# awslabs/flowgger

Measured on AMD Instinct MI355X. Metric: log lines/sec (RFC5424, 256B avg) at 1/2/4/8 MI355X; achieved HBM GB/s, higher is better.
Workload: dtype u8; 1 GPU; BASELINE configs[1]: RFC5424 no structured data, 100000000 lines/GPU @ 254 B avg (1000000-line tile x100 resident in HBM), 1% invalid lines; lines_per_gpu=100000000, bytes_per_gpu=25376525600, parallelism=lines sharded 1-way, no data-path collective, ok_lines_per_tile=990000

## Files before the change

flowgger_amd/_lib.py:

```python
from __future__ import annotations

import ctypes as C
from pathlib import Path

import os

_HERE = Path(__file__).resolve().parent
_ALT = os.environ.get("FLOWGGER_AMD_LIB") or ""
if _ALT and (Path(_ALT).name != _ALT or not _ALT.startswith("libfg_hip") or not _ALT.endswith(".so")):
    raise RuntimeError(f"FLOWGGER_AMD_LIB={_ALT!r}: only a bare libfg_hip*.so file name beside flowgger_amd/_lib.py is accepted")
LIB_PATH = _HERE / (_ALT or ("libfg_hip_prof.so" if os.environ.get("FLOWGGER_AMD_PROF_LIB") else "libfg_hip.so"))

FG_ABI_VERSION = 4
FG_RFC5424, FG_LTSV, FG_GELF, FG_RFC3164, FG_CAPNP = 0, 1, 2, 3, 4
FG_EF_VAL_ESC, FG_EF_NAME_ESC, FG_EF_SUFFIX, FG_EF_NAME_VERBATIM = 1, 2, 4, 8
FG_FRAME_NONE, FG_FRAME_LINE, FG_FRAME_NUL, FG_FRAME_SYSLEN, FG_FRAME_CAPNP = 0, 1, 2, 3, 4
FG_CAPNP_CLEAN, FG_CAPNP_TAIL, FG_CAPNP_TOO_MANY_SEGMENTS, FG_CAPNP_TOO_LARGE = 0, 1, 2, 3
FG_CAPNP_FRAME_MAX_BYTES = 0xFFFF0000
FG_SYSLEN_CLEAN, FG_SYSLEN_TAIL, FG_SYSLEN_BAD_LEN, FG_SYSLEN_LONG_PREFIX = 0, 1, 2, 3
FG_SYSLEN_MAX_PREFIX = 24
FG_UDP_RAW, FG_UDP_ZLIB, FG_UDP_GZIP, FG_UDP_BAD_ZLIB, FG_UDP_BAD_GZIP, FG_UDP_BAD_UTF8, FG_UDP_TOO_LARGE = range(7)
FG_UDP_DEFAULT_MAX_INFLATED = 65_527 * 5
FG_ST_OVERFLOW, FG_ST_BAD_UTF8 = 0xFE, 0xFD
FG_F_LTSV_NOVALUE = 128
FG_OK, FG_ERR_ARG, FG_ERR_HIP, FG_ERR_NO_DEVICE, FG_ERR_ENT_OVERFLOW, FG_ERR_UNSUPPORTED, FG_ERR_NOMEM = 0, -1, -2, -3, -4, -5, -6
FG_YEAR_NOW = -2147483648
FG_NONE = 0xFFFFFFFF
FG_T_STRING, FG_T_BOOL, FG_T_F64, FG_T_I64, FG_T_U64, FG_T_NULL, FG_T_SDID = range(7)
FG_TABLE_ARRAYS = 15
_ERRNAMES = {-1: "FG_ERR_ARG", -2: "FG_ERR_HIP", -3: "FG_ERR_NO_DEVICE (no gfx950 GPU; there is no CPU fallback)",
             -4: "FG_ERR_ENT_OVERFLOW", -5: "FG_ERR_UNSUPPORTED", -6: "FG_ERR_NOMEM"}


class FgError(RuntimeError):
    def __init__(self, code: int, what: str = ""):
        self.code = code
        super().__init__(f"{what}: {_ERRNAMES.get(code, code)}")


class fg_span(C.Structure):
    _fields_ = [("off", C.c_uint32), ("len", C.c_uint32)]


class fg_tables(C.Structure):
    _fields_ = [
        ("n", C.c_uint64), ("ent_cap", C.c_uint64),
        ("meta", C.c_void_p), ("ts", C.c_void_p),
        ("hostname", C.c_void_p), ("appname", C.c_void_p), ("procid", C.c_void_p),
        ("msgid", C.c_void_p), ("msg", C.c_void_p), ("full_msg", C.c_void_p),
        ("ent_first", C.c_void_p), ("ent_count", C.c_void_p),
        ("ent_name", C.c_void_p), ("ent_val", C.c_void_p),
        ("ent_type", C.c_void_p), ("ent_flags", C.c_void_p), ("ent_used", C.c_void_p),
    ]


TABLE_FIELDS = ["meta", "ts", "hostname", "appname", "procid", "msgid", "msg", "full_msg", "ent_first",
                "ent_count", "ent_name", "ent_val", "ent_type", "ent_flags", "ent_used"]


class fg_gelf_extra(C.Structure):
    _fields_ = [("n", C.c_uint32), ("keys", C.POINTER(C.c_char_p)), ("values", C.POINTER(C.c_char_p))]


FG_ENC_GELF, FG_ENC_LTSV, FG_ENC_RFC5424, FG_ENC_RFC3164, FG_ENC_PASSTHROUGH, FG_ENC_CAPNP = range(6)
FG_MERGE_NONE, FG_MERGE_LINE, FG_MERGE_NUL, FG_MERGE_SYSLEN = range(4)


class fg_encode_cfg(C.Structure):
    _fields_ = [("encoder", C.c_int), ("merger", C.c_int), ("n_extra", C.c_uint32), ("extra_keys", C.POINTER(C.c_char_p)),
                ("extra_values", C.POINTER(C.c_char_p)), ("prepend", C.c_char_p), ("now_ts", C.c_double)]


class fg_launch_opts(C.Structure):
    _fields_ = [("lines_per_group", C.c_uint32), ("tile_cap", C.c_uint32), ("waves_per_cu", C.c_uint32),
                ("gelf_lds_budget", C.c_uint32), ("gelf_window_kib", C.c_uint32), ("flags", C.c_uint32), ("chunk_lines", C.c_uint32), ("ent_chunk", C.c_uint32), ("fused_look", C.c_uint32), ("fused_ext", C.c_uint32)]


FG_LO_GELF_GENERIC, FG_LO_TRANSCODE_ONE_PIECE, FG_LO_NO_HEAD, FG_LO_FORCE_HEAD, FG_LO_SD_WALK, FG_LO_SD_PAIRS, FG_LO_NO_ZERO_COPY, FG_LO_FRAME_KERNEL_UPLOAD = 1, 2, 4, 8, 16, 32, 64, 128
FG_LO_FRAME_CLASSIC = 256
FG_LO_STATIC_CHUNKS = 512
FG_LO_FRAME_SELFTEST_STALL = 1024
FG_LO_NO_TAPER = 2048
FG_LO_TAPER_1 = 4096
FG_LO_TAPER_2 = 8192
FG_LO_NO_FUSED_FRAMING = 16384
FG_LO_RFC3164_REGROUP, FG_LO_RFC3164_NO_REGROUP = 32768, 65536
FG_PATH_DECODE_ZERO_COPY, FG_PATH_DECODE_SLICED, FG_PATH_FRAME_FUSED, FG_PATH_FRAME_SLICED, FG_PATH_FRAME_ONE_PIECE = 1, 2, 3, 4, 5
FG_PATH_FRAME_SYSLEN_DEVICE, FG_PATH_FRAME_SYSLEN_HOST = 6, 7
FG_PATH_FRAME_CAPNP_DEVICE, FG_PATH_FRAME_CAPNP_HOST = 8, 9
FG_PATH_FRAME_MULTI = 10
FG_PATH_FRAME_SYSLEN_MULTI_DEVICE, FG_PATH_FRAME_SYSLEN_MULTI_HOST = 11, 12
FG_PATH_FRAME_CAPNP_MULTI_DEVICE, FG_PATH_FRAME_CAPNP_MULTI_HOST = 13, 14
FG_SLOT_FRAME, FG_SLOT_BAD_UTF8, FG_SLOT_CARRY = 0, 1, 2
FG_LO_RESERVED = 0x40000000


class fg_transcoded(C.Structure):
    _fields_ = [("out", C.c_void_p), ("out_bytes", C.c_uint64), ("out_offsets", C.c_void_p), ("meta", C.c_void_p),
                ("enc_status", C.c_void_p), ("frame_offsets", C.c_void_p), ("n", C.c_uint64), ("consumed", C.c_uint64)]


class fg_tz_table(C.Structure):
    _fields_ = [("n_zones", C.c_uint32), ("names", C.POINTER(C.c_char_p)), ("zone_first", C.c_void_p), ("utc_start", C.c_void_p),
                ("utc_offset", C.c_void_p)]


class fg_rfc3164_cfg(C.Structure):
    _fields_ = [("current_year", C.c_int32), ("tz", C.POINTER(fg_tz_table))]


class fg_cfg(C.Structure):
    _fields_ = [
        ("n_schema", C.c_uint32),
        ("schema_names", C.POINTER(C.c_char_p)),
        ("schema_types", C.POINTER(C.c_uint8)),
        ("suffix_bool", C.c_char_p), ("suffix_f64", C.c_char_p),
        ("suffix_i64", C.c_char_p), ("suffix_u64", C.c_char_p),
    ]


_lib = None


def lib() -> C.CDLL:
    global _lib
    if _lib is not None:
        return _lib
    if not LIB_PATH.exists():
        raise RuntimeError(
            f"{LIB_PATH} is missing: build it with `python -m flowgger_amd.build` "
            "(hipcc --offload-arch=gfx950). The decoders have no CPU fallback.")
    try:
        import torch
    except Exception:
        pass
    L = C.CDLL(str(LIB_PATH))
    vp, u64, u32 = C.c_void_p, C.c_uint64, C.c_uint32
    L.fg_abi_version.restype = C.c_int
    L.fg_create.argtypes = [C.c_int, C.POINTER(fg_cfg), C.POINTER(vp)]
    L.fg_clone.argtypes = [vp, C.POINTER(vp)]
    L.fg_destroy.argtypes = [vp]
    L.fg_destroy.restype = None
    L.fg_last_hip_error.argtypes = [vp]
    L.fg_set_launch_opts.argtypes = [vp, C.POINTER(fg_launch_opts)]
    L.fg_tables_layout.argtypes = [u64, u64, C.POINTER(u64)]
    L.fg_decode_batch_device.argtypes = [vp, C.c_int, vp, u64, vp, u64, C.POINTER(fg_tables), vp]
    L.fg_decode_batch.argtypes = [vp, C.c_int, vp, u64, vp, u64, C.POINTER(fg_tables)]
    L.fg_error_string.argtypes = [C.c_int, C.c_uint8]
    L.fg_error_string.restype = C.c_char_p
    L.fg_tables_serialize.argtypes = [C.c_int, C.POINTER(fg_cfg), vp, vp, C.POINTER(fg_tables), u64, u64, vp, u64, vp]
    L.fg_tables_serialize.restype = C.c_int64
    L.fg_tables_stdout.argtypes = [C.c_int, C.c_int, vp, vp, C.POINTER(fg_tables), u64, u64, vp, u64]
    L.fg_tables_stdout.restype = C.c_int64
    L.fg_shard_plan.argtypes = [vp, u64, u32, vp]
    L.fg_gather_size.argtypes = [C.POINTER(fg_tables), u32, C.POINTER(u64), C.POINTER(u64)]
    L.fg_gather_tables.argtypes = [C.POINTER(fg_tables), u32, C.POINTER(fg_tables)]
    L.fg_merge_tables.argtypes = [C.POINTER(fg_tables), u32, C.POINTER(vp), C.POINTER(fg_tables), vp]
    L.fg_merge_tables_device.argtypes = [vp, C.POINTER(fg_tables), u32, C.POINTER(vp), C.POINTER(fg_tables), vp, vp]
    L.fg_ordered_merge.argtypes = [u32, vp, C.POINTER(vp), C.POINTER(vp), C.POINTER(vp), vp, u64, vp]
    L.fg_ordered_merge.restype = C.c_int64
    L.fg_ticket_ring_check.argtypes = [vp]
    L.fg_set_pinned_limits.argtypes = [u64, u64]
    L.fg_pinned_stats.argtypes = [C.POINTER(u64), C.POINTER(u64), C.POINTER(u64)]
    L.fg_set_timing.argtypes = [vp, C.c_int]
    L.fg_last_kernel_ms.argtypes = [vp, C.POINTER(C.c_float)]
    L.fg_frame_decode_batch.argtypes = [vp, C.c_int, C.c_int, vp, u64, C.c_int, C.POINTER(fg_tables), C.POINTER(vp),
                                        C.POINTER(u64), C.POINTER(u64)]
    L.fg_encode_gelf_device.argtypes = [vp, C.c_int, vp, u64, vp, u64, C.POINTER(fg_tables), C.POINTER(fg_gelf_extra), vp, u64, vp,
                                        C.POINTER(u64), vp]
    L.fg_encode_device.argtypes = [vp, C.c_int, C.POINTER(fg_encode_cfg), vp, u64, vp, u64, C.POINTER(fg_tables), vp, u64, vp, vp,
                                   C.POINTER(u64), vp]
    L.fg_encode_device_async.argtypes = [vp, C.c_int, C.POINTER(fg_encode_cfg), vp, u64, vp, u64, C.POINTER(fg_tables), vp, u64, vp, vp,
                                         u64, vp]
    L.fg_transcode_batch.argtypes = [vp, C.c_int, C.c_int, C.POINTER(fg_encode_cfg), vp, u64, vp, u64, C.c_int, C.POINTER(fg_transcoded)]
    L.fg_encode_error_string.argtypes = [C.c_uint8]
    L.fg_encode_error_string.restype = C.c_char_p
    L.fg_set_rfc3164.argtypes = [vp, C.POINTER(fg_rfc3164_cfg)]
    L.fg_measure_link.argtypes = [vp, u64, C.POINTER(C.c_double)]
    L.fg_calibrate_device.argtypes = [vp, C.c_int, vp, vp, u64, vp]
    L.fg_alloc_pinned.argtypes = [u64, C.POINTER(vp)]
    L.fg_free_pinned.argtypes = [vp]
    L.fg_free_pinned.restype = None
    L.fg_frame_device.argtypes = [vp, C.c_int, vp, u64, vp, vp, u64, C.POINTER(u64), vp]
    L.fg_decode_frames_device.argtypes = [vp, C.c_int, C.c_int, vp, u64, vp, u64, vp, C.POINTER(fg_tables), vp]
    L.fg_last_host_path.argtypes = [vp]
    L.fg_last_syslen_stop.argtypes = [vp]
    L.fg_last_capnp_stop.argtypes = [vp]
    L.fg_frame_capnp_device.argtypes = [vp, vp, u64, C.c_int, vp, u64, C.POINTER(u64), C.POINTER(u64), C.POINTER(C.c_int), vp]
    L.fg_frame_syslen_device.argtypes = [vp, vp, u64, C.c_int, vp, vp, vp, vp, u64, C.POINTER(u64), C.POINTER(u64), C.POINTER(C.c_int), vp]
    L.fg_udp_error_string.argtypes = [C.c_uint8]
    L.fg_udp_error_string.restype = C.c_char_p
    L.fg_udp_unpack_device.argtypes = [vp, vp, u64, vp, u64, u64, vp, u64, vp, vp, vp, C.POINTER(u64), vp]
    L.fg_udp_decode_batch.argtypes = [vp, C.c_int, vp, u64, vp, u64, u64, C.POINTER(fg_tables), C.POINTER(vp), C.POINTER(vp), C.POINTER(vp)]
    L.fg_frame_decode_device.argtypes = [vp, C.c_int, C.c_int, vp, u64, C.c_int, vp, u64, C.POINTER(fg_tables), u64, vp, vp]
    L.fg_frame_multi_device.argtypes = [vp, C.c_int, vp, u64, vp, vp, u64, vp, vp, u64, vp, vp, C.POINTER(u64), vp]
    L.fg_frame_decode_multi_batch.argtypes = [vp, C.c_int, C.c_int, vp, u64, vp, vp, u64, C.POINTER(fg_tables), C.POINTER(vp), C.POINTER(vp),
                                              C.POINTER(vp), C.POINTER(vp), C.POINTER(u64)]
    L.fg_frame_syslen_multi_device.argtypes = [vp, vp, u64, vp, u64, vp, vp, vp, vp, u64, vp, vp, vp, C.POINTER(u64), C.POINTER(u64), vp]
    L.fg_frame_decode_syslen_multi_batch.argtypes = [vp, C.c_int, vp, u64, vp, u64, C.POINTER(fg_tables), C.POINTER(vp), C.POINTER(vp),
                                                     C.POINTER(vp), C.POINTER(vp), C.POINTER(u64)]
    L.fg_frame_capnp_multi_device.argtypes = [vp, vp, u64, vp, u64, vp, vp, u64, vp, vp, vp, C.POINTER(u64), vp]
    L.fg_frame_decode_capnp_multi_batch.argtypes = [vp, vp, u64, vp, u64, C.POINTER(fg_tables), C.POINTER(vp), C.POINTER(vp), C.POINTER(vp),
                                                    C.POINTER(vp), C.POINTER(vp), C.POINTER(u64)]
    if L.fg_abi_version() != FG_ABI_VERSION:
        raise RuntimeError("libfg_hip.so ABI version mismatch")
    _lib = L
    return L


def check(rc: int, what: str) -> None:
    if rc != 0:
        raise FgError(rc, what)
```

flowgger_amd/csrc/fg_pipeline.hpp:

```cpp
#pragma once
#include "fg_device.hpp"
#include "fg_plan_policy.hpp"
#include "fg_wave.hpp"

namespace fg {

using u32x4 = unsigned int __attribute__((ext_vector_type(4)));

__device__ __forceinline__ uint32_t eq_flags(uint32_t x, uint32_t pat) {
    uint32_t s = ((x & 0x7F7F7F7Fu) ^ pat) + 0x7F7F7F7Fu;
    return ~(s | x) & 0x80808080u;
}
__device__ __forceinline__ uint32_t range_flags(uint32_t x) {
    uint32_t l = x & 0x7F7F7F7Fu;
    uint32_t ge33 = l + 0x5F5F5F5Fu;
    uint32_t le126 = l + 0x01010101u;
    return ge33 & ~le126 & ~x & 0x80808080u;
}
__device__ __forceinline__ uint32_t ctrl_flags(uint32_t x) {
    uint32_t ge32 = (x & 0x7F7F7F7Fu) + 0x60606060u;
    return ~(ge32 | x) & 0x80808080u;
}
__device__ __forceinline__ uint32_t gather16(uint32_t f0, uint32_t f1, uint32_t f2, uint32_t f3) {
    uint32_t lo = __builtin_amdgcn_udot4(f1, 0x80402010u, __builtin_amdgcn_udot4(f0, 0x08040201u, 0u, false), false);
    uint32_t hi = __builtin_amdgcn_udot4(f3, 0x80402010u, __builtin_amdgcn_udot4(f2, 0x08040201u, 0u, false), false);
    return (lo >> 7) | (hi << 1);
}
__device__ __forceinline__ uint32_t mask16_eq(const uint4& v, uint32_t pat) {
    return gather16(eq_flags(v.x, pat), eq_flags(v.y, pat), eq_flags(v.z, pat), eq_flags(v.w, pat));
}

struct Tile {
    const uint32_t* w;
    const uint32_t* bm;
};
__device__ __forceinline__ void load8(const Tile& T, uint32_t a, uint32_t* lo, uint32_t* hi) {
    uint32_t d = a >> 2, s = a & 3u;
    uint32_t w0 = T.w[d], w1 = T.w[d + 1], w2 = T.w[d + 2];
    *lo = __builtin_amdgcn_alignbyte(w1, w0, s);
    *hi = __builtin_amdgcn_alignbyte(w2, w1, s);
}
__device__ __forceinline__ void load16(const Tile& T, uint32_t a, uint32_t w[4]) {
    const uint32_t d = a >> 2, s = a & 3u;
    uint32_t r0 = T.w[d], r1 = T.w[d + 1], r2 = T.w[d + 2], r3 = T.w[d + 3], r4 = T.w[d + 4];
    w[0] = __builtin_amdgcn_alignbyte(r1, r0, s);
    w[1] = __builtin_amdgcn_alignbyte(r2, r1, s);
    w[2] = __builtin_amdgcn_alignbyte(r3, r2, s);
    w[3] = __builtin_amdgcn_alignbyte(r4, r3, s);
}
struct WinReader {
    const Tile& T;
    uint32_t base;
    uint32_t w0 = 0x80000000u;
    uint64_t lo = 0, hi = 0;
    __device__ __forceinline__ WinReader(const Tile& t, uint32_t b) : T(t), base(b) {}
    __device__ __forceinline__ uint32_t byte(uint32_t i) {
        uint32_t off = i - w0;
        if (off >= 16u) {
            uint32_t w[4];
            load16(T, base + i, w);
            lo = (uint64_t)w[0] | ((uint64_t)w[1] << 32);
            hi = (uint64_t)w[2] | ((uint64_t)w[3] << 32);
            w0 = i;
            off = 0;
        }
        const uint64_t v = off < 8u ? lo : hi;
        return (uint32_t)(v >> (8u * (off & 7u))) & 0xFFu;
    }
};

__device__ __forceinline__ uint32_t find_bit(const uint32_t* bm, uint32_t base, uint32_t q, uint32_t len) {
    while (q < len) {
        uint32_t a = base + q;
        uint32_t w = bm[a >> 5] >> (a & 31u);
        if (w) {
            uint32_t r = q + (uint32_t)__builtin_ctz(w);
            return r < len ? r : len;
        }
        q += 32u - (a & 31u);
    }
    return len;
}
__device__ __forceinline__ uint32_t find_bit_long(const uint32_t* bm, uint32_t base, uint32_t q, uint32_t len) {
    if (q >= len) return len;
    {
        const uint32_t a = base + q;
        const uint32_t w = bm[a >> 5] >> (a & 31u);
        if (w) {
            const uint32_t r = q + (uint32_t)__builtin_ctz(w);
            return r < len ? r : len;
        }
        q += 32u - (a & 31u);
    }
    while (q + 256u <= len) {
        const uint32_t i = (base + q) >> 5;
        uint32_t w[8];
#pragma unroll
        for (int k = 0; k < 8; ++k) w[k] = bm[i + k];
        if ((w[0] | w[1] | w[2] | w[3] | w[4] | w[5] | w[6] | w[7]) != 0u) {
            uint32_t r = len;
#pragma unroll
            for (int k = 7; k >= 0; --k)
                if (w[k]) r = q + 32u * k + (uint32_t)__builtin_ctz(w[k]);
            return r < len ? r : len;
        }
        q += 256u;
    }
    while (q < len) {
        const uint32_t w = bm[(base + q) >> 5];
        if (w) {
            const uint32_t r = q + (uint32_t)__builtin_ctz(w);
            return r < len ? r : len;
        }
        q += 32u;
    }
    return len;
}
template <class M>
__device__ __forceinline__ void rebuild_bitmap(const uint8_t* smem, uint16_t* bm16, uint32_t nchunk) {
    const uint4* src = reinterpret_cast<const uint4*>(smem);
    for (uint32_t c = threadIdx.x; c < nchunk; c += kWave) bm16[c] = (uint16_t)M::mask16(src[c]);
}

struct RowOut {
    uint32_t meta;
    double ts;
    fg_span span[6];
    uint32_t first, count;
    bool skip = false;
};
__device__ __forceinline__ void store_row(const DevTables& t, uint64_t li, const RowOut& o) {
    if (o.skip) return;
    gstore(t.meta, li, o.meta);
    gstore(t.ts, li, o.ts);
#pragma unroll
    for (int k = 0; k < 6; ++k) gstore(t.span[k], li, o.span[k]);
    gstore(t.ent_first, li, o.first);
    gstore(t.ent_count, li, o.count);
}
constexpr uint32_t kStashEntries = 48;
constexpr uint32_t kStashWords = 2;

struct EntAlloc {
    uint32_t ex = 0;
    uint32_t total = 0;
    wv::Slots s{};
    bool overflow = false;
};
__device__ __forceinline__ EntAlloc alloc_entries_ex(const DevTables& t, uint32_t n_ent, uint32_t* ent_state) {
    EntAlloc a;
    if (!__any(n_ent != 0u)) return a;
    a.ex = wv::excl_sum(n_ent, &a.total);
    const uint32_t left = wv::wave_left(ent_state);
    const unsigned long long nofit = __ballot(n_ent != 0u && a.ex + n_ent > left);
    const uint32_t cut = nofit ? (uint32_t)__shfl((int)a.ex, (int)__builtin_ctzll(nofit), kWave) : a.total;
    a.s = wv::wave_alloc(t.ent_used, t.ent_cap, ent_state, a.total, cut, t.alloc_chunk);
    a.overflow = a.s.overflow && n_ent != 0u && a.ex >= a.s.cut;
    return a;
}
__device__ __forceinline__ uint32_t alloc_entries(const DevTables& t, uint32_t n_ent, bool* overflow, uint32_t* ent_state) {
    const EntAlloc a = alloc_entries_ex(t, n_ent, ent_state);
    *overflow = a.overflow;
    return (a.overflow || a.total == 0u) ? 0u : a.s.at(a.ex);
}

struct GroupCtx {
    const uint8_t* bytes;
    const uint8_t* smem;
    uint16_t* bm16;
    uint64_t o0, o1;
    uint64_t a0;
    uint32_t span;
    bool valid;
    uint64_t li;
    uint64_t* stash;
    uint32_t ablate;
    uint32_t* ent_state;
    unsigned long long* phase;
    uint32_t tbase = 0;
    uint32_t tlen = 0;
    uint32_t last2 = 0;
    uint32_t tile_cap = 0;
};

template <uint32_t WORDS, class Unpack>
__device__ __forceinline__ bool stash_to_table(const GroupCtx& c, const DevTables& t, const EntAlloc& a, uint32_t n_ent, bool mine,
                                               Unpack un) {
    const uint32_t lane = threadIdx.x;
    const uint32_t cap = (c.span / 18u) & ~3u;
    if (a.total == 0u || a.total > cap || a.s.overflow || c.stash == nullptr || __any(n_ent != 0u && !mine)) return false;
    uint64_t* s_name = reinterpret_cast<uint64_t*>(const_cast<uint8_t*>(c.smem));
    uint64_t* s_val = s_name + cap;
    uint16_t* s_tf = reinterpret_cast<uint16_t*>(s_val + cap);
    __syncthreads();
    for (uint32_t k0 = 0; k0 < n_ent; k0 += 4u) {
        uint64_t w0[4], w1[4];
#pragma unroll
        for (uint32_t j = 0; j < 4u; ++j) {
            const uint32_t k = k0 + j < n_ent ? k0 + j : n_ent - 1u;
            w0[j] = c.stash[(k * WORDS) * kWave + lane];
            w1[j] = WORDS > 1u ? c.stash[(k * WORDS + 1u) * kWave + lane] : 0ull;
        }
#pragma unroll
        for (uint32_t j = 0; j < 4u; ++j) {
            if (k0 + j < n_ent) {
                uint64_t name, val;
                uint32_t tf;
                un(w0[j], w1[j], &name, &val, &tf);
                const uint32_t idx = a.ex + k0 + j;
                s_name[idx] = name;
                s_val[idx] = val;
                s_tf[idx] = (uint16_t)tf;
            }
        }
    }
    __syncthreads();
    for (uint32_t idx = lane; idx < a.total; idx += kWave) {
        const uint32_t slot = a.s.at(idx);
        const uint64_t name = s_name[idx];
        const uint32_t tf = s_tf[idx];
        t.ent_name[slot] = fg_span{(uint32_t)name, (uint32_t)(name >> 32)};
        t.ent_val[slot] = s_val[idx];
        t.ent_type[slot] = (uint8_t)(tf & 0xFFu);
        t.ent_flags[slot] = (uint8_t)(tf >> 8);
    }
    return true;
}


struct FrameArgs {
    uint32_t strip;
    const uint8_t* line_bad;
    uint32_t* ticket = nullptr;
    uint32_t ticket_base = 0;
    uint32_t taper0 = kNoTaper, taper1 = kNoTaper, taper2 = kNoTaper;
};

#define FG_STREAM_AUX 2
__device__ __forceinline__ uint4 stream_load(const uint4* p) {
    typedef uint32_t nt4 __attribute__((ext_vector_type(4)));
    const nt4 v = __builtin_nontemporal_load(reinterpret_cast<const nt4*>(p));
    return make_uint4(v.x, v.y, v.z, v.w);
}

template <class F, class = void>
struct tail_batch { static constexpr int value = 4; };
template <class F>
struct tail_batch<F, decltype((void)F::kTailBatch)> { static constexpr int value = F::kTailBatch; };

template <class F, class = void>
struct defer_row_store { static constexpr bool value = true; };
template <class F>
struct defer_row_store<F, decltype((void)F::kDeferRowStore)> { static constexpr bool value = F::kDeferRowStore; };

constexpr uint32_t kHeadCap = 1024;
template <class F, class = void>
struct head_cap { static constexpr uint32_t value = kHeadCap; };
template <class F>
struct head_cap<F, decltype((void)F::kHeadBytes)> { static constexpr uint32_t value = F::kHeadBytes; };

template <int NB, bool PROF, class F, bool HEAD = false>
__device__ __forceinline__ void persistent_loop(const uint8_t* __restrict__ bytes, const uint64_t* __restrict__ offsets,
                                                uint64_t n, const DevTables& t, uint32_t tile_cap, uint32_t L, uint64_t chunk_lines,
                                                unsigned long long* prof, uint64_t* stash_base, F& fmt, FrameArgs fr) {
    static_assert(!HEAD || F::kClasses <= 1, "HEAD staging classifies one stage-A byte class at most");
    const uint64_t kChunkLines = chunk_lines;
    extern __shared__ __attribute__((aligned(16))) uint8_t smem[];
    uint16_t* bm16 = reinterpret_cast<uint16_t*>(smem + tile_cap + 64u);
    const uint32_t bm_stride = tile_cap / 16u + 16u;
    uint4* dst = reinterpret_cast<uint4*>(smem);
    const uint32_t lane = threadIdx.x;
    const uint64_t G = gridDim.x;
    uint64_t* stash = stash_base ? stash_base + (uint64_t)blockIdx.x * (kStashEntries * kStashWords * kWave) : nullptr;

    const bool dyn = fr.ticket != nullptr;
    uint32_t tk_raw = 0;
    bool tk_pending = false;
    auto draw_ticket = [&]() {
        if (lane == 0u) tk_raw = __hip_atomic_fetch_add(fr.ticket, 1u, __ATOMIC_RELAXED, __HIP_MEMORY_SCOPE_AGENT);
        tk_pending = true;
    };
    uint64_t chunk = blockIdx.x;
    uint64_t p, hi_line;
    chunk_range(chunk, kChunkLines, fr.taper0, fr.taper1, fr.taper2, n, &p, &hi_line);
    if (dyn && p < n) draw_ticket();

    auto load_offsets = [&](uint64_t q, uint64_t* o0, uint64_t* o1) {
        const uint64_t li = q + lane;
        const bool in = lane < L && li < hi_line;
        *o0 = offsets[in ? li : hi_line];
        *o1 = offsets[in ? li + 1 : hi_line];
    };
    auto geometry = [&](uint64_t q, uint64_t o0, uint64_t o1, uint32_t* nl, uint64_t* a0, uint32_t* span) {
        const uint64_t left = hi_line - q;
        const uint32_t avail = left < (uint64_t)L ? (uint32_t)left : L;
        const uint32_t lo_l = (uint32_t)__builtin_amdgcn_readfirstlane((int)(uint32_t)o0);
        const uint32_t lo_h = (uint32_t)__builtin_amdgcn_readfirstlane((int)(uint32_t)(o0 >> 32));
        const uint64_t lo = (uint64_t)lo_l | ((uint64_t)lo_h << 32);
        *a0 = lo & ~15ull;
        const unsigned long long fit = __ballot(lane < avail && (o1 - *a0) <= (uint64_t)tile_cap);
        uint32_t cnt = fit == ~0ull ? 64u : (uint32_t)__builtin_ctzll(~fit);
        if (cnt == 0u) cnt = 1u;
        *nl = cnt;
        const uint32_t last = cnt - 1u;
        const uint32_t hi_l = (uint32_t)__builtin_amdgcn_readlane((int)(uint32_t)o1, (int)last);
        const uint32_t hi_h = (uint32_t)__builtin_amdgcn_readlane((int)(uint32_t)(o1 >> 32), (int)last);
        const uint64_t hi = (uint64_t)hi_l | ((uint64_t)hi_h << 32);
        const uint64_t want = hi - *a0;
        *span = want > tile_cap ? tile_cap : (uint32_t)((want + 15ull) & ~15ull);
    };
    auto load_window = [&](uint64_t a0, uint32_t span, u32x4* v) {
        __amdgpu_buffer_rsrc_t rsrc =
            __builtin_amdgcn_make_buffer_rsrc(const_cast<uint8_t*>(bytes + a0), (short)0, (int)span, 0x00020000);
#pragma unroll
        for (int k = 0; k < NB; ++k) v[k] = __builtin_amdgcn_raw_buffer_load_b128(rsrc, (int)(lane * 16u + k * 1024u), 0, FG_STREAM_AUX);
    };
    auto geometry_head = [&](uint64_t q, uint64_t o0, uint64_t o1, uint32_t* nl, uint32_t* span, uint32_t* st_out, uint32_t* tb_out) {
        const uint64_t left = hi_line - q;
        const uint32_t avail = left < (uint64_t)L ? (uint32_t)left : L;
        const uint64_t want = (o1 - o0) + (o0 & 15ull);
        uint32_t st = want >= head_cap<F>::value ? head_cap<F>::value : (uint32_t)((want + 15ull) & ~15ull);
        if (lane >= avail) st = 0u;
        uint32_t total;
        const uint32_t tb = wv::excl_sum(st, &total);
        const unsigned long long fit = __ballot(lane < avail && tb + st <= tile_cap);
        uint32_t cnt = fit == ~0ull ? 64u : (uint32_t)__builtin_ctzll(~fit);
        if (cnt == 0u) cnt = 1u;
        *nl = cnt;
        const uint32_t last = cnt - 1u;
        *span = (uint32_t)__builtin_amdgcn_readlane((int)tb, (int)last) + (uint32_t)__builtin_amdgcn_readlane((int)st, (int)last);
        *st_out = lane < cnt ? st : 0u;
        *tb_out = tb;
    };
    auto load_window_head = [&](uint64_t o0, uint32_t st, u32x4* v) {
#pragma unroll
        for (int k = 0; k < NB; ++k) {
            const uint32_t lo = (uint32_t)__builtin_amdgcn_readlane((int)(uint32_t)o0, k);
            const uint32_t hi = (uint32_t)__builtin_amdgcn_readlane((int)(uint32_t)(o0 >> 32), k);
            const uint32_t sk = (uint32_t)__builtin_amdgcn_readlane((int)st, k);
            const uint64_t b = ((uint64_t)lo | ((uint64_t)hi << 32)) & ~15ull;
            __amdgpu_buffer_rsrc_t rsrc = __builtin_amdgcn_make_buffer_rsrc(const_cast<uint8_t*>(bytes + b), (short)0, (int)sk, 0x00020000);
            v[k] = __builtin_amdgcn_raw_buffer_load_b128(rsrc, (int)(lane * 16u), 0, FG_STREAM_AUX);
        }
    };
    auto load_last2 = [&](uint64_t o0, uint64_t o1) -> uint32_t {
        const uint64_t len = o1 - o0;
        uint32_t r = 0;
        if (len >= 1u) r = bytes[o1 - 1u];
        if (len >= 2u) r |= (uint32_t)bytes[o1 - 2u] << 8;
        return r;
    };

    uint32_t* ent_state = reinterpret_cast<uint32_t*>(smem + tile_cap + 56u);
    if (lane < 2u) ent_state[lane] = 0u;
    if (p >= hi_line) return;
    uint64_t o0, o1, a0 = 0;
    uint32_t span, nl, st = 0, tb = 0, last2 = 0;
    load_offsets(p, &o0, &o1);
    u32x4 v[NB];
    if constexpr (HEAD) {
        geometry_head(p, o0, o1, &nl, &span, &st, &tb);
        load_window_head(o0, st, v);
        last2 = load_last2(o0, o1);
    } else {
        geometry(p, o0, o1, &nl, &a0, &span);
        load_window(a0, span, v);
    }
    RowOut pend{};
    uint64_t pend_li = 0;
    bool pend_valid = false;
    uint64_t acc0 = 0, acc1 = 0, acc2 = 0, acc3 = 0, iters = 0, tm0 = 0, tm1 = 0, tm2 = 0, tm3 = 0;
    const uint32_t ablate = PROF ? (uint32_t)prof[5] : 0u;
    const uint32_t term4 = fr.strip == FG_FRAME_LINE ? 0x0A0A0A0Au : fr.strip == FG_FRAME_NUL ? 0u : wv::kNoTerm;

    for (;;) {
        uint64_t pn = p + nl;
        if (pn >= hi_line) {
            if (dyn) {
                if (!tk_pending) draw_ticket();
                const uint32_t tk = (uint32_t)__builtin_amdgcn_readfirstlane((int)tk_raw);
                chunk = (uint64_t)(uint32_t)(tk - fr.ticket_base) + G;
                tk_pending = false;
                chunk_range(chunk, kChunkLines, fr.taper0, fr.taper1, fr.taper2, n, &pn, &hi_line);
                if (pn < n) draw_ticket();
            } else {
                chunk += G;
                chunk_range(chunk, kChunkLines, kNoTaper, kNoTaper, kNoTaper, n, &pn, &hi_line);
            }
        }
        const bool more = pn < n;
        uint64_t no0 = 0, no1 = 0;
        if (more) load_offsets(pn, &no0, &no1);
        if (PROF) {
            tm0 = __builtin_amdgcn_s_memtime();
            __builtin_amdgcn_s_waitcnt(0x0F70);
            tm1 = __builtin_amdgcn_s_memtime();
        }
        FG_MARK(A);
        const uint32_t nchunk = span >> 4;
        const uint32_t nrow = HEAD ? nl : (nchunk + kWave - 1u) / kWave;
        if constexpr (HEAD) {
#pragma unroll
            for (int k = 0; k < NB; ++k) {
                if ((uint32_t)k < nl) {
                    const uint32_t tk = (uint32_t)__builtin_amdgcn_readlane((int)tb, k), sk = (uint32_t)__builtin_amdgcn_readlane((int)st, k);
                    if (lane * 16u < sk) {
                        const uint4 q = make_uint4(v[k][0], v[k][1], v[k][2], v[k][3]);
                        dst[(tk >> 4) + lane] = q;
                        if constexpr (F::kClasses != 0) F::classify_store(q, bm16, (tk >> 4) + lane, bm_stride, term4);
                    }
                }
            }
            constexpr uint32_t HB = tail_batch<F>::value >= 8 ? 8u : 4u;
            for (uint32_t r0 = NB; r0 < nl; r0 += HB) {
                uint4 w[HB];
                uint32_t tk[HB], sk[HB];
#pragma unroll
                for (uint32_t j = 0; j < HB; ++j) {
                    const uint32_t r = r0 + j < nl ? r0 + j : nl - 1u;
                    const uint32_t lo = (uint32_t)__builtin_amdgcn_readlane((int)(uint32_t)o0, (int)r);
                    const uint32_t hi = (uint32_t)__builtin_amdgcn_readlane((int)(uint32_t)(o0 >> 32), (int)r);
                    tk[j] = (uint32_t)__builtin_amdgcn_readlane((int)tb, (int)r);
                    sk[j] = (uint32_t)__builtin_amdgcn_readlane((int)st, (int)r);
                    const uint64_t b = ((uint64_t)lo | ((uint64_t)hi << 32)) & ~15ull;
                    __amdgpu_buffer_rsrc_t rsrc = __builtin_amdgcn_make_buffer_rsrc(const_cast<uint8_t*>(bytes + b), (short)0, (int)sk[j], 0x00020000);
                    const u32x4 x = __builtin_amdgcn_raw_buffer_load_b128(rsrc, (int)(lane * 16u), 0, FG_STREAM_AUX);
                    w[j] = make_uint4(x[0], x[1], x[2], x[3]);
                }
#pragma unroll
                for (uint32_t j = 0; j < HB; ++j)
                    if (lane * 16u < sk[j]) {
                        dst[(tk[j] >> 4) + lane] = w[j];
                        if constexpr (F::kClasses != 0) F::classify_store(w[j], bm16, (tk[j] >> 4) + lane, bm_stride, term4);
                    }
            }
        } else {
#pragma unroll
        for (int k = 0; k < NB; ++k) {
            if ((uint32_t)k < nrow) {
                uint32_t idx = k * kWave + lane;
                uint4 q = make_uint4(v[k][0], v[k][1], v[k][2], v[k][3]);
                dst[idx] = q;
                F::classify_store(q, bm16, idx, bm_stride, idx < nchunk ? term4 : wv::kPastSpan);
            }
        }
        }
        if (!HEAD && nrow > (uint32_t)NB) {
            const uint4* __restrict__ src = reinterpret_cast<const uint4*>(bytes + a0);
            const uint32_t last = nchunk - 1u;
            constexpr int TB = tail_batch<F>::value;
            for (uint32_t c0 = NB * kWave; c0 < nchunk; c0 += kWave * TB) {
                uint4 w[TB];
#pragma unroll
                for (int k = 0; k < TB; ++k) {
                    const uint32_t idx = c0 + k * kWave + lane;
                    w[k] = stream_load(src + (idx < last ? idx : last));
                }
#pragma unroll
                for (int k = 0; k < TB; ++k) {
                    if (k == 0 || c0 + k * kWave < nchunk) {
                        const uint32_t idx = c0 + k * kWave + lane, ci = idx < last ? idx : last;
                        dst[ci] = w[k];
                        F::classify_store(w[k], bm16, ci, bm_stride, term4);
                    }
                }
            }
        }
        __builtin_amdgcn_sched_barrier(0);
        FG_MARK(S);
        if (PROF) {
            __builtin_amdgcn_s_waitcnt(0xC07F);
            tm2 = __builtin_amdgcn_s_memtime();
        }
        uint64_t pa0 = 0;
        uint32_t pspan = 0, pnl = 0, pst = 0, ptb = 0, plast2 = 0;
        if (more) {
            if constexpr (HEAD) geometry_head(pn, no0, no1, &pnl, &pspan, &pst, &ptb);
            else geometry(pn, no0, no1, &pnl, &pa0, &pspan);
        }
        FG_MARK(ST);
        if (pend_valid && !(ablate & 1u)) store_row(t, pend_li, pend);
        FG_MARK(W0);
        if (more) {
            if constexpr (HEAD) {
                load_window_head(no0, pst, v);
                plast2 = load_last2(no0, no1);
            } else {
                load_window(pa0, pspan, v);
            }
        }
        __builtin_amdgcn_sched_barrier(0);
        FG_MARK(W1);
        FG_MARK(B);
        if (PROF) tm3 = __builtin_amdgcn_s_memtime();
        __syncthreads();
        if (!(ablate & 2u)) {
            const uint64_t li = p + lane;
            const bool valid = lane < nl;
            uint64_t e1 = o1;
            uint32_t l2 = last2;
            if (fr.strip != FG_FRAME_NONE) {
                uint32_t b1 = last2 & 0xFFu, b2 = (last2 >> 8) & 0xFFu;
                if constexpr (!HEAD) {
                    const uint64_t len = o1 - o0;
                    const bool over = nl == 1u && __builtin_amdgcn_readfirstlane((int)((o1 - a0) > (uint64_t)span)) != 0;
                    if (over) {
                        FG_RARE_BEGIN();
                        if (valid && len >= 1u) b1 = bytes[o1 - 1u];
                        if (valid && len >= 2u) b2 = bytes[o1 - 2u];
                        FG_RARE_END();
                    } else if (valid) {
                        const uint32_t q = (uint32_t)(o1 - a0);
                        if (len >= 1u) b1 = smem[q - 1u];
                        if (len >= 2u) b2 = smem[q - 2u];
                    }
                }
                if (valid && e1 > o0) {
                    if (fr.strip == FG_FRAME_LINE) {
                        if (b1 == '\n') {
                            --e1;
                            if (e1 > o0 && b2 == '\r') --e1;
                        }
                    } else if (b1 == 0u) {
                        --e1;
                    }
                    if (HEAD && e1 != o1) {
                        l2 = 0u;
                        if (e1 - o0 >= 1u) l2 = bytes[e1 - 1];
                        if (e1 - o0 >= 2u) l2 |= (uint32_t)bytes[e1 - 2] << 8;
                    }
                }
            }
            GroupCtx c{bytes, smem, bm16, o0, e1, a0, span, valid, li, (ablate & 8u) ? nullptr : stash, ablate, ent_state, PROF ? prof + 6 : nullptr};
            c.tile_cap = tile_cap;
            if constexpr (HEAD) {
                const uint32_t al = (uint32_t)(o0 & 15ull), len = (uint32_t)(e1 - o0);
                c.tbase = tb + al;
                c.tlen = st == 0u ? 0u : (st - al < len ? st - al : len);
                c.last2 = l2;
            }
            pend = fmt.decode(c, t);
            if (fr.line_bad && valid && fr.line_bad[li]) {
                pend.meta = FG_ST_BAD_UTF8 | (0xFFu << 8) | (0xFFu << 16);
                pend.ts = 0.0;
#pragma unroll
                for (int k = 0; k < 6; ++k) pend.span[k] = fg_span{0, FG_NONE};
                pend.count = 0;
            }
            pend_li = li;
            pend_valid = valid;
            if (!defer_row_store<F>::value) {
                if (pend_valid && !(ablate & 1u)) store_row(t, pend_li, pend);
                pend_valid = false;
            }
        }
        if (PROF) {
            __builtin_amdgcn_sched_barrier(0);
            __builtin_amdgcn_s_waitcnt(0xC07F);
            uint64_t tm4 = __builtin_amdgcn_s_memtime();
            acc0 += tm1 - tm0;
            acc1 += tm2 - tm1;
            acc2 += tm3 - tm2;
            acc3 += tm4 - tm3;
            iters += 1;
        }
        FG_MARK(Z);
        if (!more) break;
        __syncthreads();
        p = pn;
        nl = pnl;
        o0 = no0;
        o1 = no1;
        a0 = pa0;
        span = pspan;
        if constexpr (HEAD) {
            st = pst;
            tb = ptb;
            last2 = plast2;
        }
    }
    if (pend_valid && !(ablate & 1u)) store_row(t, pend_li, pend);
    if (PROF && lane == 0) {
        atomicAdd(&prof[0], (unsigned long long)acc0);
        atomicAdd(&prof[1], (unsigned long long)acc1);
        atomicAdd(&prof[2], (unsigned long long)acc2);
        atomicAdd(&prof[3], (unsigned long long)acc3);
        atomicAdd(&prof[4], (unsigned long long)iters);
    }
}

}

#include <cstdio>
#include <cstdlib>

#include "fg_cus.hpp"

namespace fg {
constexpr int kComputeBoundWindow = 2;

inline void take_tickets(FrameArgs* fr, TicketSlot* tk, const LaunchPlan& p) {
    if (!tk || !tk->d_word || !tk->h_val || p.chunks + p.blocks >= 0xFFFFFFFFull || p.blocks > p.chunks) return;
    if (!p.tickets) return;
    fr->ticket = tk->d_word;
    fr->ticket_base = *tk->h_val;
    fr->taper0 = p.taper[0], fr->taper1 = p.taper[1], fr->taper2 = p.taper[2];
    *tk->h_val += (uint32_t)p.chunks;
}

template <class K>
inline int plan_launch(K kernel, uint64_t n, uint64_t avg_len, uint32_t extra_lds, uint32_t max_tile, uint32_t stash_blocks, LaunchPlan* p,
                       const fg_launch_opts& lo, const PlanFormat& pf = PlanFormat()) {
    static_cast<LaunchGeometry&>(*p) = launch_geometry(n, avg_len, extra_lds, max_tile, lo, pf);
    const int cus = device_cus();
    if (cus < 1) return -1;
    int per_cu = 0;
    if (hipOccupancyMaxActiveBlocksPerMultiprocessor(&per_cu, kernel, kWave, p->lds) != hipSuccess || per_cu < 1) per_cu = 1;
    if (lo.waves_per_cu > 0 && per_cu > (int)lo.waves_per_cu) per_cu = (int)lo.waves_per_cu;
    uint64_t blocks = (uint64_t)per_cu * (uint64_t)cus;
    if (blocks > p->groups) blocks = p->groups;
    if (stash_blocks && blocks > stash_blocks) blocks = stash_blocks;
    const ChunkPlan cp = plan_chunks(n, blocks, p->L, p->g, p->full, pf.ticket_from, lo, pf.taper);
    p->chunk = cp.chunk;
    p->chunks = cp.chunks;
    p->tickets = cp.tickets;
    for (int j = 0; j < 3; ++j) p->taper[j] = cp.taper[j];
    p->blocks = cp.blocks;
    return 0;
}

#if defined(FG_PROF_BUILD)
inline bool prof_requested() { return getenv("FG_PROF") != nullptr; }
#define FG_PROF_TWIN(...) (__VA_ARGS__)
#else
constexpr bool prof_requested() { return false; }
#define FG_PROF_TWIN(...) nullptr
#endif
struct ProfRun {
    unsigned long long* d = nullptr;
    unsigned long long h[16] = {0, 0, 0, 0, 0, 0, 0, 0, 0, 0, 0, 0, 0, 0, 0, 0};
    bool begin(hipStream_t stream) {
#if defined(FG_PROF_BUILD)
        if (const char* e = getenv("FG_ABLATE")) h[5] = (unsigned long long)atoi(e);
#endif
        if (hipMalloc((void**)&d, sizeof(h)) != hipSuccess) return false;
        (void)hipMemcpyAsync(d, h, sizeof(h), hipMemcpyHostToDevice, stream);
        return true;
    }
    void end(hipStream_t stream, const char* name, const LaunchPlan& p) {
        (void)hipStreamSynchronize(stream);
        (void)hipMemcpy(h, d, sizeof(h), hipMemcpyDeviceToHost);
        (void)hipFree(d);
        const double it = h[4] ? (double)h[4] : 1.0;
        fprintf(stderr,
                "[fg prof] %s: grid %u x64, L %u, tile %u, iters/wave %.1f | cycles per iteration: wait %.0f, stageA %.0f, "
                "stores+prefetch-issue %.0f, stageB %.0f\n",
                name, p.blocks, p.L, p.tile, it / (double)(p.blocks ? p.blocks : 1), h[0] / it, h[1] / it, h[2] / it, h[3] / it);
        bool any_phase = false;
        for (int k = 6; k < 16; ++k) any_phase = any_phase || h[k] != 0;
        if (any_phase) {
            fprintf(stderr, "[fg prof] %s stage-B phases (cycles per iteration):", name);
            for (int k = 6; k < 16; ++k) fprintf(stderr, " %.0f", h[k] / it);
            fprintf(stderr, "\n");
        }
    }
};

template <class K>
struct Kernels {
    K run, prof;
    const char* name;
};
template <class K>
inline Kernels<K> kernels(K run, typename SameAs<K>::type prof, const char* name) { return Kernels<K>{run, prof, name}; }

struct DecodeCall {
    uint64_t n;
    const DevTables* t;
    hipStream_t stream;
    FrameArgs fr;
    const fg_launch_opts* lo;
    TicketSlot* tk;
};
template <class K, class Go>
inline int launch_planned(const Kernels<K>& k, const LaunchPlan& p, const DecodeCall& c, Go go, bool prof_tickets = true) {
    const bool prof = k.prof != nullptr && prof_requested();
    FrameArgs fr = c.fr;
    if (!prof || prof_tickets) take_tickets(&fr, c.tk, p);
    DevTables tt = *c.t;
    tt.alloc_chunk = entry_chunk(tt.ent_cap, p.blocks, c.n, *c.lo, tt.shares);
    if (prof) {
        ProfRun pr;
        if (!pr.begin(c.stream)) return -1;
        go(k.prof, p, tt, fr, pr.d);
        pr.end(c.stream, k.name, p);
    } else {
        go(k.run, p, tt, fr, (unsigned long long*)nullptr);
    }
    return (int)hipGetLastError();
}
template <class K, class Go>
inline int plan_and_launch(const Kernels<K>& k, const DecodeCall& c, uint64_t avg_len, uint32_t extra_lds, uint32_t max_tile, uint32_t stash_blocks,
                           const PlanFormat& pf, Go go) {
    LaunchPlan p;
    if (plan_launch(k.run, c.n, avg_len, extra_lds, max_tile, stash_blocks, &p, *c.lo, pf)) return -1;
    return launch_planned(k, p, c, go);
}
}
```

flowgger_amd/csrc/fg_plan_policy.hpp:

```cpp
#pragma once
#include <stdint.h>

#include "../../include/fg_hip.h"

#if defined(__HIPCC__)
#define FG_POLICY_HD __host__ __device__
#else
#define FG_POLICY_HD
#endif

namespace fg {

constexpr uint32_t kNoTaper = 0xFFFFFFFFu;

FG_POLICY_HD inline void chunk_range(uint64_t c, uint64_t chunk, uint32_t t0, uint32_t t1, uint32_t t2, uint64_t n, uint64_t* lo,
                                     uint64_t* hi) {
    uint64_t base = 0, first = 0, sz = chunk;
    if (c >= t0) {
        base = (uint64_t)t0 * sz, first = t0, sz >>= 1;
        if (c >= t1) {
            base += (uint64_t)(t1 - t0) * sz, first = t1, sz >>= 1;
            if (c >= t2) base += (uint64_t)(t2 - t1) * sz, first = t2, sz >>= 1;
        }
    }
    const uint64_t l = base + (c - first) * sz;
    *lo = l < n ? l : n;
    *hi = l + sz < n ? l + sz : n;
}

inline uint64_t count_chunks(uint64_t chunk, const uint32_t t[3], uint64_t n) {
    uint64_t base = 0, first = 0, sz = chunk;
    for (int j = 0; j < 3; ++j) {
        if (t[j] == kNoTaper) break;
        const uint64_t upto = base + (uint64_t)(t[j] - first) * sz;
        if (upto >= n) break;
        base = upto, first = t[j], sz >>= 1;
    }
    return first + (n - base + sz - 1) / sz;
}

struct ChunkPlan {
    uint64_t chunk = 1;
    uint64_t chunks = 0;
    uint32_t blocks = 0;
    bool tickets = false;
    uint32_t taper[3] = {kNoTaper, kNoTaper, kNoTaper};
};

inline ChunkPlan plan_chunks(uint64_t n, uint64_t blocks, uint32_t L, uint64_t g, uint64_t full, uint32_t ticket_from, const fg_launch_opts& lo,
                             uint32_t taper = 1) {
    ChunkPlan p;
    if (blocks < 1u) blocks = 1u;
    if (g < 1u) g = 1u;
    if (g > L) g = L;
    if (full < 1u) full = 1u;
    const bool dynamic = !(lo.flags & FG_LO_STATIC_CHUNKS);
    const bool named = lo.chunk_lines >= (dynamic ? 1u : L) && lo.chunk_lines <= 65536u;
    const uint64_t per_wave = (n + blocks - 1) / blocks;
    uint64_t chunk;
    bool tickets = false;
    if (named) {
        chunk = lo.chunk_lines;
        if (n < blocks * 2u * chunk) {
            chunk = per_wave;
            if (chunk < (dynamic ? g : (uint64_t)L)) chunk = dynamic ? g : (uint64_t)L;
        }
        tickets = dynamic;
    } else if (dynamic && per_wave >= (uint64_t)ticket_from * full) {
        chunk = full;
        tickets = true;
    } else if (dynamic) {
        chunk = per_wave;
        const uint64_t unit = g >= L ? g : (g * 15u / 16u ? g * 15u / 16u : 1u);
        if (chunk < unit) chunk = unit;
    } else {
        const uint64_t k = (per_wave + full - 1) / full;
        chunk = (per_wave + (k ? k : 1) - 1) / (k ? k : 1);
        if (chunk < L) chunk = L;
    }
    if (chunk < 1u) chunk = 1u;
    p.chunk = chunk;
    p.chunks = (n + chunk - 1) / chunk;
    if (lo.flags & (FG_LO_TAPER_1 | FG_LO_TAPER_2)) taper = ((lo.flags & FG_LO_TAPER_1) ? 1u : 0u) + ((lo.flags & FG_LO_TAPER_2) ? 2u : 0u);
    if (taper > 3u) taper = 3u;
    if (tickets && taper && !(lo.flags & FG_LO_NO_TAPER)) {
        uint64_t m = n / (2u * chunk);
        if (m > blocks) m = blocks;
        uint32_t levels = 0;
        while (levels < taper && (chunk >> (levels + 1u)) >= g) ++levels;
        if (m >= 1u && levels >= 1u && p.chunks + 4u * m < 0xFFFFFFF0ull) {
            const uint64_t t0 = (n - m * chunk) / chunk;
            p.taper[0] = (uint32_t)t0;
            if (levels >= 2u) p.taper[1] = (uint32_t)(t0 + m);
            if (levels >= 3u) p.taper[2] = (uint32_t)(t0 + 2u * m);
            p.chunks = count_chunks(chunk, p.taper, n);
        }
    }
    p.blocks = (uint32_t)(blocks > p.chunks ? p.chunks : blocks);
    p.tickets = tickets;
    return p;
}

constexpr int kWindowKiB = 20;
constexpr uint32_t kMaxTile = 57344;

constexpr uint32_t tile_lds(uint32_t tile, uint32_t classes = 1) { return tile + 64u + (tile / 16u + 16u) * 2u * classes; }

constexpr uint32_t kShortLineTile = 17408;
static_assert(tile_lds(kShortLineTile) <= 160u * 1024u / 8u, "eight waves per CU");
static_assert(tile_lds(kShortLineTile + 1024u) > 160u * 1024u / 8u, "the largest such tile");

constexpr uint64_t kHeadFromLen = 768, kPairsFromLen = 320;
struct Variant { bool head, pairs; };
inline Variant pick_variant(uint64_t avg_len, uint32_t flags) {
    return Variant{(flags & FG_LO_FORCE_HEAD) || (avg_len >= kHeadFromLen && !(flags & FG_LO_NO_HEAD)),
                   (flags & FG_LO_SD_PAIRS) || (avg_len >= kPairsFromLen && !(flags & FG_LO_SD_WALK))};
}
inline bool gelf_group_fits_3k(uint64_t avg_len) { return 8u * avg_len * 17u / 16u + 256u <= 3072u; }
inline bool gelf_const_3k(uint64_t avg_len, const fg_launch_opts& lo) {
    return gelf_group_fits_3k(avg_len) && !lo.tile_cap && !(lo.flags & FG_LO_GELF_GENERIC);
}

struct PlanFormat {
    uint32_t max_lines = 64;
    uint32_t n_classes = 1;
    uint32_t (*extra_for)(uint32_t tile, uint32_t lines) = nullptr;
    uint32_t (*extra_tile)(uint32_t tile) = nullptr;
    uint32_t default_tile = 0;
    uint32_t default_chunk = 0;
    uint32_t ticket_from = 2;
    uint32_t taper = 1;
    PlanFormat& lines(uint32_t v) { max_lines = v; return *this; }
    PlanFormat& classes(uint32_t v) { n_classes = v; return *this; }
    PlanFormat& lds_for(uint32_t (*f)(uint32_t, uint32_t)) { extra_for = f; return *this; }
    PlanFormat& lds_tile(uint32_t (*f)(uint32_t)) { extra_tile = f; return *this; }
    PlanFormat& tile(uint32_t v) { default_tile = v; return *this; }
    PlanFormat& chunk(uint32_t v) { default_chunk = v; return *this; }
    PlanFormat& tickets_from(uint32_t v) { ticket_from = v; return *this; }
    PlanFormat& taper_levels(uint32_t v) { taper = v; return *this; }
};
inline PlanFormat rfc5424_walk_format(uint64_t avg_len) {
    return PlanFormat().tickets_from(20u).taper_levels(0u).tile(avg_len < kPairsFromLen ? kShortLineTile : 0u);
}

struct LaunchGeometry {
    uint32_t L = 64;
    uint32_t tile = 0;
    uint32_t lds = 0;
    uint64_t groups = 0;
    uint64_t full = 256;
    uint64_t g = 64;
};
struct LaunchPlan : LaunchGeometry {
    uint64_t chunk = 256;
    uint64_t chunks = 0;
    bool tickets = false;
    uint32_t taper[3] = {kNoTaper, kNoTaper, kNoTaper};
    uint32_t blocks = 0;
};

inline LaunchGeometry launch_geometry(uint64_t n, uint64_t avg_len, uint32_t extra_lds, uint32_t max_tile, const fg_launch_opts& lo,
                                      const PlanFormat& pf = PlanFormat()) {
    const uint64_t window = (uint64_t)kWindowKiB * 1024u;
    auto tile_for = [&](uint32_t l) { return (((uint64_t)l * avg_len * 17u / 16u + 256u) + 1023u) / 1024u * 1024u; };
    auto clamp = [&](uint64_t v) { return (uint32_t)(v < 4096u ? 4096u : v > max_tile ? max_tile : v); };
    const bool named_lines = lo.lines_per_group >= 1 && lo.lines_per_group <= pf.max_lines;
    const bool named_tile = lo.tile_cap >= 1024 && lo.tile_cap <= max_tile;
    LaunchGeometry p;
    uint32_t L = pf.max_lines;
    while (L > 1 && tile_for(L) > window + 2048u) L >>= 1;
    if (named_lines) L = lo.lines_per_group;
    uint32_t tile = clamp(tile_for(L));
    if (pf.default_tile && tile > pf.default_tile && !named_lines) tile = pf.default_tile;
    if (named_tile) tile = (lo.tile_cap + 1023u) / 1024u * 1024u;
    if (!pf.extra_for && !named_lines) {
        if (L <= 16u && !named_tile && tile < 18432u && max_tile >= 18432u && !pf.default_tile) tile = 18432u;
        L = pf.max_lines;
    }
    p.L = L;
    p.tile = tile;
    p.lds = tile_lds(tile, pf.n_classes ? pf.n_classes : 1u) + extra_lds + (pf.extra_for ? pf.extra_for(tile, L) : 0u) +
            (pf.extra_tile ? pf.extra_tile(tile) : 0u);
    {
        const uint64_t by_lines = (n + L - 1) / L, by_bytes = (n * avg_len + tile - 1) / tile;
        p.groups = by_lines > by_bytes ? by_lines : by_bytes;
    }
    p.full = pf.default_chunk ? pf.default_chunk : (avg_len ? (uint64_t)tile / avg_len : L) >= L ? 256u : 512u;
    p.g = avg_len ? ((uint64_t)tile * 16u) / (avg_len * 17u) : L;
    return p;
}

inline uint32_t entry_chunk(uint64_t ent_cap, uint32_t blocks, uint64_t n, const fg_launch_opts& lo, uint32_t shares = 1) {
    if (lo.ent_chunk == 1u) return 0u;
    if (lo.ent_chunk >= 2u) return lo.ent_chunk;
    const uint64_t waves = blocks ? blocks : 1u;
    const uint64_t budget = ent_cap / (shares ? shares : 1u);
    uint64_t c = budget / (16ull * waves);
    if (c > 4096u) c = 4096u;
    if (budget / (4ull * waves) < 256u) return 0u;
    if (c < 256u) c = 256u;
    const uint64_t per_wave = (n + waves - 1u) / waves * 8ull;
    if (c > per_wave) c = per_wave;
    if (c < 256u) c = 256u;
    return (uint32_t)c;
}

}
```

flowgger_amd/csrc/fg_rfc5424.hip:

```cpp
#include <cstdio>
#include <cstdlib>

#include "fg_fused.hpp"
#include "fg_sd2.hpp"
#include "fg_tsfast.hpp"

namespace fg {

enum : uint32_t {
    E_OK = 0,
    E_BOM = 1,
    E_BRACKETS = 2,
    E_INVPRI = 3,
    E_NOVER = 4,
    E_BADVER = 5,
    E_NOTS = 6,
    E_BADTS = 7,
    E_NOHOST = 8,
    E_NOAPP = 9,
    E_NOPROC = 10,
    E_NOMSGID = 11,
    E_NODATA = 12,
    E_NOMSG = 13,
    E_MALFORMED = 14,
    E_NOSD = 15,
    E_SDFMT = 16,
    E_NOBRACKET = 17
};

struct Row {
    uint32_t status = E_OK;
    uint32_t facility = 0xFF, severity = 0xFF, flags = 0;
    double ts = 0.0;
    uint32_t off[6];
    uint32_t len[6];
    uint32_t data0 = 0;
    uint32_t n_ent = 0;
};


template <class R>
__device__ __forceinline__ uint32_t find_space(R& rd, uint32_t q, uint32_t len) {
    while (q < len && rd.byte(q) != ' ') ++q;
    return q;
}

template <bool EMIT, class R>
__device__ __forceinline__ uint32_t sd_walk(R& rd, uint32_t pos, uint32_t len, uint32_t* msg_at, uint32_t* n_ent,
                            const DevTables& t, uint32_t slot) {
    uint32_t cnt = 0;
    for (;;) {
        uint32_t s = pos + 1;
        uint32_t sp = find_space(rd, s, len);
        if (sp >= len) return E_NOSD;
        if (EMIT) {
            t.ent_name[slot + cnt] = fg_span{s, sp - s};
            t.ent_val[slot + cnt] = 0;
            t.ent_type[slot + cnt] = FG_T_SDID;
            t.ent_flags[slot + cnt] = 0;
        }
        ++cnt;
        uint32_t st = 0, name_s = 0, name_e = 0, val_s = 0, esc_seen = 0;
        uint32_t i = sp + 1;
        uint32_t after = 0;
        for (; i < len; ++i) {
            uint32_t c = rd.byte(i);
            if (st == 3) {
                if (c == '\\') {
                    st = 4;
                    esc_seen = 1;
                } else if (c == '"') {
                    if (EMIT) {
                        t.ent_name[slot + cnt] = fg_span{name_s, name_e - name_s};
                        t.ent_val[slot + cnt] = (uint64_t)val_s | ((uint64_t)(i - val_s) << 32);
                        t.ent_type[slot + cnt] = FG_T_STRING;
                        t.ent_flags[slot + cnt] = esc_seen ? FG_EF_VAL_ESC : 0;
                    }
                    ++cnt;
                    st = 0;
                }
            } else if (st == 4) {
                st = 3;
            } else {
                bool is_name = (c - 33u) <= 93u && c != '"' && c != '=' && c != ']';
                if (st == 0) {
                    if (c == ' ' || c == '"') {
                    } else if (c == ']') {
                        after = i + 1;
                        break;
                    } else if (is_name) {
                        st = 1;
                        name_s = i;
                    } else {
                        return E_SDFMT;
                    }
                } else if (st == 1) {
                    if (is_name) {
                    } else if (c == '=') {
                        name_e = i;
                        st = 2;
                    } else {
                        return E_SDFMT;
                    }
                } else {
                    if (c != '"') return E_SDFMT;
                    st = 3;
                    val_s = i + 1;
                    esc_seen = 0;
                }
            }
        }
        if (after == 0) return E_NOBRACKET;
        if (after >= len) return E_NOMSG;
        uint32_t c = rd.byte(after);
        if (c == '[') {
            pos = after;
            continue;
        }
        if (c != ' ') return E_MALFORMED;
        *msg_at = after;
        *n_ent = cnt;
        return E_OK;
    }
}

template <class R>
__device__ __forceinline__ void parse_tail(R& rd, uint32_t q, uint32_t line0, uint32_t len, Row& r, const DevTables& t) {
    if (q >= len) {
        r.status = E_NOMSG;
        return;
    }
    r.data0 = q;
    uint32_t c = rd.byte(q);
    uint32_t msg_at;
    if (c == '-') {
        msg_at = q + 1;
    } else if (c == '[') {
        uint32_t st = sd_walk<false>(rd, q, len, &msg_at, &r.n_ent, t, 0);
        if (st != E_OK) {
            r.status = st;
            r.n_ent = 0;
            return;
        }
    } else {
        r.status = E_MALFORMED;
        return;
    }
    uint32_t e = trim_end(rd, line0, len);
    r.off[S_FULL] = line0;
    r.len[S_FULL] = e - line0;
    uint32_t s = trim_start(rd, msg_at, len);
    if (e > s) {
        r.off[S_MSG] = s;
        r.len[S_MSG] = e - s;
    }
}

template <class R>
__device__ __forceinline__ void parse_line_generic(R& rd, uint32_t len, Row& r, const DevTables& t) {
    uint32_t p = 0;
    if (len >= 3 && rd.byte(0) == 0xEFu && rd.byte(1) == 0xBBu && rd.byte(2) == 0xBFu) {
        p = 3;
        r.flags |= FG_F_BOM;
    } else if (len == 0 || rd.byte(0) != '<') {
        r.status = E_BOM;
        return;
    }
    const uint32_t line0 = p;
    if (p >= len || rd.byte(p) != '<') {
        r.status = E_BRACKETS;
        return;
    }
    uint32_t q = p + 1;
    {
        uint32_t v = 0, nd = 0;
        bool ok = true;
        if (q < len && rd.byte(q) == '+') ++q;
        while (q < len) {
            uint32_t c = rd.byte(q);
            if (c == '>' || c == ' ') break;
            uint32_t d = c - '0';
            if (d <= 9u) {
                v = v * 10u + d;
                if (v > 255u) {
                    v = 256u;
                    ok = false;
                }
                ++nd;
            } else {
                ok = false;
            }
            ++q;
        }
        if (!ok || nd == 0) {
            r.status = E_INVPRI;
            return;
        }
        if (q >= len || rd.byte(q) != '>') {
            r.status = E_NOVER;
            return;
        }
        ++q;
        if (!(q < len && rd.byte(q) == '1' && (q + 1 == len || rd.byte(q + 1) == ' '))) {
            r.status = E_BADVER;
            return;
        }
        ++q;
        r.facility = v >> 3;
        r.severity = v & 7u;
    }
    if (q >= len) {
        r.status = E_NOTS;
        return;
    }
    ++q;
    {
        uint32_t e = find_space(rd, q, len);
        if (!parse_rfc3339(rd, q, e, &r.ts)) {
            r.status = E_BADTS;
            return;
        }
        q = e;
    }
#pragma unroll
    for (int k = 0; k < 4; ++k) {
        if (q >= len) {
            r.status = E_NOHOST + k;
            return;
        }
        ++q;
        uint32_t e = find_space(rd, q, len);
        r.off[k] = q;
        r.len[k] = e - q;
        q = e;
    }
    if (q >= len) {
        r.status = E_NODATA;
        return;
    }
    ++q;
    parse_tail(rd, q, line0, len, r, t);
}


enum : uint32_t {
    R_GENERIC = 1,
    R_TS_SLOW = 2,
    R_TAIL = 4,
    R_TRIM = 8
};

struct Fast {
    uint32_t route;
    uint32_t no_ts;
    uint32_t ts_ok;
    uint32_t rest;
    uint32_t t0, te;
    uint32_t d0;
    uint32_t c7;
    uint32_t e, s;
};

__device__ __forceinline__ uint32_t fast_rfc3339(const Tile& T, uint32_t base, const uint32_t* hdr, uint32_t t0, uint32_t L,
                                                 double* out) {
    const uint32_t a = base + t0;
    const uint32_t s = t0 - 4u;
    uint32_t r[9];
#pragma unroll
    for (int k = 0; k < 9; ++k) r[k] = __builtin_amdgcn_alignbyte(hdr[k + 2], hdr[k + 1], s);
    return fast_rfc3339_core(r, L, [&](uint32_t pos, uint32_t* z0, uint32_t* z1) { load8(T, a + pos, z0, z1); }, out);
}

__device__ __forceinline__ uint32_t take_space(uint64_t& lo, uint64_t& hi, uint32_t none, uint32_t& found) {
    const bool in_lo = lo != 0, in_hi = hi != 0;
    const uint32_t p = in_lo ? (uint32_t)__builtin_ctzll(lo) : in_hi ? 64u + (uint32_t)__builtin_ctzll(hi) : none;
    const uint64_t lo2 = lo & (lo - 1ull), hi2 = hi & (hi - 1ull);
    hi = in_lo ? hi : hi2;
    lo = lo2;
    found += (in_lo || in_hi) ? 1u : 0u;
    return p;
}

constexpr uint32_t kNoLastByte = 0xFFFFFFFFu;
__device__ __forceinline__ Fast parse_line_fast(const Tile& T, uint32_t base, uint32_t len, Row& r, uint32_t last_byte = kNoLastByte) {
    Fast f;
    uint32_t l0 = last_byte, l1;
    if (last_byte == kNoLastByte) load8(T, base + (len ? len - 1u : 0u), &l0, &l1);
    uint32_t hdr[33];
    {
        const uint32_t d = base >> 2, sft = base & 3u;
        uint32_t raw[34];
#pragma unroll
        for (int k = 0; k < 34; ++k) raw[k] = T.w[d + k];
#pragma unroll
        for (int k = 0; k < 33; ++k) hdr[k] = __builtin_amdgcn_alignbyte(raw[k + 1], raw[k], sft);
    }
    const uint32_t h0 = hdr[0], h1 = hdr[1];

    const uint32_t c1 = ((h0 >> 8) & 0xFFu) - '0', c2 = ((h0 >> 16) & 0xFFu) - '0', c3 = (h0 >> 24) - '0';
    const bool d2 = c2 <= 9u, d3 = d2 && c3 <= 9u;
    const uint32_t nd = 1u + (d2 ? 1u : 0u) + (d3 ? 1u : 0u);
    uint32_t pri = c1;
    pri = d2 ? pri * 10u + c2 : pri;
    pri = d3 ? pri * 10u + c3 : pri;
    const uint64_t hh = (((uint64_t)h1 << 32) | h0) >> (8u * (1u + nd));
    const uint32_t sp0 = 3u + nd;
    const bool shape = (h0 & 0xFFu) == '<' && c1 <= 9u && pri <= 255u && (uint32_t)(hh & 0xFFFFu) == (('1' << 8) | '>') &&
                       sp0 <= len;
    f.no_ts = sp0 == len ? 1u : 0u;
    f.route = (!shape || (sp0 < len && (uint32_t)((hh >> 16) & 0xFFu) != ' ')) ? R_GENERIC : 0u;
    r.facility = pri >> 3;
    r.severity = pri & 7u;

    uint64_t lo, hi;
    {
        uint32_t m[8];
#pragma unroll
        for (int k = 0; k < 8; ++k)
            m[k] = gather16(eq_flags(hdr[4 * k], 0x20202020u), eq_flags(hdr[4 * k + 1], 0x20202020u),
                            eq_flags(hdr[4 * k + 2], 0x20202020u), eq_flags(hdr[4 * k + 3], 0x20202020u));
        lo = (uint64_t)(m[0] | (m[1] << 16)) | ((uint64_t)(m[2] | (m[3] << 16)) << 32);
        hi = (uint64_t)(m[4] | (m[5] << 16)) | ((uint64_t)(m[6] | (m[7] << 16)) << 32);
    }
    {
        const uint64_t lo_keep = len < 64u ? (1ull << (len & 63u)) - 1ull : ~0ull;
        const uint64_t hi_keep = len < 64u ? 0ull : len < 128u ? (1ull << ((len - 64u) & 63u)) - 1ull : ~0ull;
        lo &= lo_keep & ~((2ull << sp0) - 1ull);
        hi &= hi_keep;
    }
    uint32_t found = 0;
    const uint32_t s1 = take_space(lo, hi, len, found);
    const uint32_t s2 = take_space(lo, hi, len, found);
    const uint32_t s3 = take_space(lo, hi, len, found);
    const uint32_t s4 = take_space(lo, hi, len, found);
    const uint32_t s5 = take_space(lo, hi, len, found);
    f.route |= (found < 5u && len > 128u) ? R_GENERIC : 0u;

    f.t0 = sp0 + 1u;
    f.te = s1;
    {
        const uint32_t ok = fast_rfc3339(T, base, hdr, f.t0, s1 - f.t0, &r.ts);
        f.ts_ok = ok == 1u ? 1u : 0u;
        f.route |= ok == 2u ? R_TS_SLOW : 0u;
    }
    r.off[S_HOST] = s1 + 1u;
    r.len[S_HOST] = s2 - s1 - 1u;
    r.off[S_APP] = s2 + 1u;
    r.len[S_APP] = s3 - s2 - 1u;
    r.off[S_PROC] = s3 + 1u;
    r.len[S_PROC] = s4 - s3 - 1u;
    r.off[S_MSGID] = s4 + 1u;
    r.len[S_MSGID] = s5 - s4 - 1u;
    const uint32_t d0 = s5 + 1u;
    f.d0 = d0;
    f.rest = found < 5u ? E_NOHOST + found : d0 >= len ? E_NOMSG : E_OK;

    uint32_t m0, m1;
    load8(T, base + (d0 < len ? d0 : 0u), &m0, &m1);
    const uint32_t c = m0 & 0xFFu;
    f.c7 = c;
    const bool live = !f.no_ts && f.rest == E_OK;
    f.route |= (live && c != '-') ? R_TAIL : 0u;
    const uint32_t last = l0 & 0xFFu;
    const bool end_plain = last > 0x20u && last < 0x80u;
    f.e = len;
    const uint32_t cA = (m0 >> 8) & 0xFFu, cB = (m0 >> 16) & 0xFFu;
    const uint32_t s = d0 + 1u;
    const bool one_sp = s + 1u < len && cA == ' ' && cB > 0x20u && cB < 0x80u;
    const bool no_sp = s < len && cA > 0x20u && cA < 0x80u;
    f.s = one_sp ? s + 1u : s;
    f.route |= (live && c == '-' && !(end_plain && (one_sp || no_sp))) ? R_TRIM : 0u;
    return f;
}

struct QuoteClass {
    static __device__ __forceinline__ uint32_t mask16(const uint4& v) {
        const uint32_t Q = 0x22222222u, B = 0x5C5C5C5Cu;
        return gather16(eq_flags(v.x, Q) | eq_flags(v.x, B), eq_flags(v.y, Q) | eq_flags(v.y, B),
                        eq_flags(v.z, Q) | eq_flags(v.z, B), eq_flags(v.w, Q) | eq_flags(v.w, B));
    }
};
__device__ __forceinline__ bool is_sd_name_char(uint32_t c) {
    return (c - 33u) <= 93u && c != '"' && c != '=' && c != ']';
}
struct WinMasks {
    uint32_t space;
    uint32_t skip;
    uint32_t name;
    uint32_t eq, quote, rb;
};
__device__ __forceinline__ WinMasks window_masks(const uint32_t w[4]) {
    uint32_t sp[4], qu[4], eq[4], rb[4], rg[4];
#pragma unroll
    for (int k = 0; k < 4; ++k) {
        sp[k] = eq_flags(w[k], 0x20202020u);
        qu[k] = eq_flags(w[k], 0x22222222u);
        eq[k] = eq_flags(w[k], 0x3D3D3D3Du);
        rb[k] = eq_flags(w[k], 0x5D5D5D5Du);
        rg[k] = range_flags(w[k]);
    }
    WinMasks m;
    m.quote = gather16(qu[0], qu[1], qu[2], qu[3]);
    m.eq = gather16(eq[0], eq[1], eq[2], eq[3]);
    m.rb = gather16(rb[0], rb[1], rb[2], rb[3]);
    m.space = gather16(sp[0], sp[1], sp[2], sp[3]);
    m.skip = m.space | m.quote;
    m.name = gather16(rg[0], rg[1], rg[2], rg[3]) & ~(m.quote | m.eq | m.rb);
    return m;
}

enum { SD_COUNT = 0, SD_EMIT = 1, SD_STASH = 2 };
__device__ __forceinline__ uint64_t stash_pack(uint32_t name_s, uint32_t name_len, uint32_t val_len, uint32_t esc, uint32_t sdid) {
    return (uint64_t)name_s | ((uint64_t)name_len << 16) | ((uint64_t)val_len << 32) | ((uint64_t)esc << 48) | ((uint64_t)sdid << 49);
}
template <int MODE>
__device__ __forceinline__ uint32_t sd_walk_tile(const Tile& T, uint32_t base, uint32_t pos, uint32_t len, uint32_t* msg_at,
                                                 uint32_t* n_ent, const DevTables& t, uint32_t slot, uint32_t* tile_w = nullptr,
                                                 bool* rec_ok_out = nullptr) {
    constexpr bool EMIT = MODE == SD_EMIT;
    LdsReader rd(T.w, base);
    uint32_t cnt = 0;
    uint32_t wpos = (base + 3u) & ~3u;
    bool rec_ok = true;
    auto record = [&](uint64_t rec, uint32_t consumed) {
        if (rec_ok) {
            if (wpos + 8u <= base + consumed) {
                tile_w[wpos >> 2] = (uint32_t)rec;
                tile_w[(wpos >> 2) + 1u] = (uint32_t)(rec >> 32);
                wpos += 8u;
            } else {
                rec_ok = false;
            }
        }
    };
    for (;;) {
        const uint32_t s = pos + 1;
        uint32_t sp = s;
        for (;;) {
            if (sp >= len) return E_NOSD;
            uint32_t w[4];
            load16(T, base + sp, w);
            const uint32_t avail = len - sp < 16u ? len - sp : 16u;
            const uint32_t hit = gather16(eq_flags(w[0], 0x20202020u), eq_flags(w[1], 0x20202020u), eq_flags(w[2], 0x20202020u),
                                          eq_flags(w[3], 0x20202020u)) & ((1u << avail) - 1u);
            if (hit) {
                sp += (uint32_t)__builtin_ctz(hit);
                break;
            }
            sp += avail;
        }
        if (EMIT) {
            t.ent_name[slot + cnt] = fg_span{s, sp - s};
            t.ent_val[slot + cnt] = 0;
            t.ent_type[slot + cnt] = FG_T_SDID;
            t.ent_flags[slot + cnt] = 0;
        }
        if (MODE == SD_STASH) record(stash_pack(s, sp - s, 0, 0, 1), sp + 1u);
        ++cnt;
        uint32_t status = E_OK;
        uint32_t i = sp + 1;
        bool in_value = false;
        uint32_t name_s = 0, name_e = 0, val_s = 0, cur = 0, esc_seen = 0;
        uint32_t close_at = 0;
        for (;;) {
            uint32_t w0 = i, start = 0;
            if (in_value) {
                const uint32_t p = find_bit(T.bm, base, cur, len);
                if (p >= len) {
                    status = E_NOBRACKET;
                    break;
                }
                w0 = p;
                start = 1;
            } else if (i >= len) {
                status = E_NOBRACKET;
                break;
            }
            uint32_t w[4];
            load16(T, base + w0, w);
            if (in_value) {
                if ((w[0] & 0xFFu) == '\\') {
                    esc_seen = 1;
                    cur = w0 + 2;
                    continue;
                }
                if (EMIT) {
                    t.ent_name[slot + cnt] = fg_span{name_s, name_e - name_s};
                    t.ent_val[slot + cnt] = (uint64_t)val_s | ((uint64_t)(w0 - val_s) << 32);
                    t.ent_type[slot + cnt] = FG_T_STRING;
                    t.ent_flags[slot + cnt] = esc_seen ? FG_EF_VAL_ESC : 0;
                }
                if (MODE == SD_STASH) record(stash_pack(name_s, name_e - name_s, w0 - val_s, esc_seen, 0), w0 + 1u);
                ++cnt;
                in_value = false;
            }
            const uint32_t avail = len - w0 < 16u ? len - w0 : 16u;
            const uint32_t inside = (1u << avail) - 1u;
            const WinMasks m = window_masks(w);
            const uint32_t from = ~((1u << start) - 1u);
            const uint32_t stop = ~m.skip & from & inside;
            if (stop == 0) {
                i = w0 + avail;
                continue;
            }
            const uint32_t i0 = (uint32_t)__builtin_ctz(stop);
            if ((m.rb >> i0) & 1u) {
                close_at = w0 + i0;
                break;
            }
            if (!((m.name >> i0) & 1u)) {
                status = E_SDFMT;
                break;
            }
            const uint32_t after_name = ~m.name & ~((1u << i0) - 1u) & 0xFFFFu;
            const uint32_t e0 = after_name ? (uint32_t)__builtin_ctz(after_name) : 16u;
            if (e0 + 1u < avail) {
                if (!((m.eq >> e0) & 1u) || !((m.quote >> (e0 + 1u)) & 1u)) {
                    status = E_SDFMT;
                    break;
                }
                name_s = w0 + i0;
                name_e = w0 + e0;
                val_s = name_e + 2u;
            } else if (i0 != 0) {
                i = w0 + i0;
                continue;
            } else {
                uint32_t q = w0, c = 0;
                do {
                    ++q;
                    c = q < len ? rd.byte(q) : 0x100u;
                } while (is_sd_name_char(c));
                if (q >= len || q + 1u >= len) {
                    status = (q < len && c != '=') ? E_SDFMT : E_NOBRACKET;
                    break;
                }
                if (c != '=' || rd.byte(q + 1u) != '"') {
                    status = E_SDFMT;
                    break;
                }
                name_s = w0;
                name_e = q;
                val_s = q + 2u;
            }
            in_value = true;
            esc_seen = 0;
            cur = val_s;
        }
        if (status != E_OK) return status;
        const uint32_t after = close_at + 1;
        if (after >= len) return E_NOMSG;
        const uint32_t c = rd.byte(after);
        if (c == '[') {
            pos = after;
            continue;
        }
        if (c != ' ') return E_MALFORMED;
        *msg_at = after;
        *n_ent = cnt;
        if (rec_ok_out) *rec_ok_out = rec_ok;
        return E_OK;
    }
}
__device__ __forceinline__ bool finish_sd_tail(const Tile& T, uint32_t base, uint32_t len, uint32_t walk_len, uint32_t last2, uint32_t msg_at, Row& r,
                                               const uint8_t* gbytes, uint64_t o0) {
    LdsReader rd(T.w, base);
    if (walk_len < len) {
        const uint32_t s = trim_start(rd, msg_at, walk_len - 8u);
        if (s + 8u >= walk_len) return false;
        const uint32_t last = last2 & 0xFFu;
        uint32_t e = len;
        if (!(last > 0x20u && last < 0x80u)) {
            GlobalReader grd(reinterpret_cast<const uint32_t*>(gbytes), o0);
            e = trim_end(grd, 0u, len);
        }
        r.off[S_FULL] = 0;
        r.len[S_FULL] = e;
        if (e > s) {
            r.off[S_MSG] = s;
            r.len[S_MSG] = e - s;
        }
        return true;
    }
    uint32_t e = trim_end(rd, 0u, len);
    r.off[S_FULL] = 0;
    r.len[S_FULL] = e;
    uint32_t s = trim_start(rd, msg_at, len);
    if (e > s) {
        r.off[S_MSG] = s;
        r.len[S_MSG] = e - s;
    }
    return true;
}
__device__ __forceinline__ bool parse_tail_sd_tile(const Tile& T, uint32_t base, uint32_t q, uint32_t len, uint32_t walk_len, uint32_t last2, Row& r,
                                                   const DevTables& t, uint32_t* tile_w, bool* rec_ok, const uint8_t* gbytes, uint64_t o0) {
    r.data0 = q;
    uint32_t msg_at = 0;
    uint32_t st = tile_w ? sd_walk_tile<SD_STASH>(T, base, q, walk_len, &msg_at, &r.n_ent, t, 0, tile_w, rec_ok)
                         : sd_walk_tile<SD_COUNT>(T, base, q, walk_len, &msg_at, &r.n_ent, t, 0);
    if (st != E_OK) {
        r.n_ent = 0;
        if (walk_len < len) return false;
        r.status = st;
        return true;
    }
    if (!finish_sd_tail(T, base, len, walk_len, last2, msg_at, r, gbytes, o0)) {
        r.n_ent = 0;
        return false;
    }
    return true;
}

constexpr uint32_t kShortSdTail = 64;

template <bool HEAD, bool SDX = false, bool PROF = false>
struct Rfc5424FormatT {
    static constexpr uint32_t kClasses = 0;
    static __device__ __forceinline__ void classify_store(const uint4&, uint16_t*, uint32_t, uint32_t, uint32_t) {}
    unsigned long long* pacc = nullptr;

    __device__ __forceinline__ RowOut decode(const GroupCtx& c, const DevTables& t) const {
    const uint8_t* __restrict__ bytes = c.bytes;
    const uint8_t* smem = c.smem;
    uint16_t* bm16 = c.bm16;
    const uint64_t o0 = c.o0, o1 = c.o1, a0 = c.a0;
    const uint32_t span = c.span, ablate = c.ablate;
    const bool valid = c.valid;
    uint64_t* stash = c.stash;
    const uint32_t lane = threadIdx.x;
    Row r;
#pragma unroll
    for (int k = 0; k < 6; ++k) {
        r.off[k] = 0;
        r.len[k] = FG_NONE;
    }
    const uint32_t len = (uint32_t)(o1 - o0);
    const bool in_tile = HEAD ? c.tlen == len : (o1 - a0) <= (uint64_t)span;
    const bool head_only = HEAD && !in_tile && c.tlen >= 512u;
    const uint32_t walk_len = HEAD ? c.tlen : len;
    const uint32_t base = HEAD ? c.tbase : (uint32_t)(o0 - a0);
    bool from_global = false;
    uint32_t* tile_w = reinterpret_cast<uint32_t*>(const_cast<uint8_t*>(smem));
    bool rec_ok = false;
    Tile T{reinterpret_cast<const uint32_t*>(smem), reinterpret_cast<const uint32_t*>(bm16)};
    uint64_t pc[10] = {0, 0, 0, 0, 0, 0, 0, 0, 0, 0}, tk = PROF ? wv::clock() : 0;
    auto tick = [&](int k) {
        if (PROF) {
            const uint64_t now = wv::clock();
            pc[k] += now - tk;
            tk = now;
        }
    };
    uint32_t route = 0;
    Fast f{};
    if (valid) {
        route = R_GENERIC;
        if (in_tile || head_only) {
            f = parse_line_fast(T, base, len, r, HEAD ? (len ? (c.last2 & 0xFFu) : 0u) : kNoLastByte);
            route = f.route;
            if (!(route & R_GENERIC)) {
                if (route & R_TS_SLOW) {
                    LdsReader rd(T.w, base);
                    bool ok = parse_rfc3339(rd, f.t0, f.te, &r.ts);
                    r.status = f.no_ts ? E_NOTS : ok ? f.rest : E_BADTS;
                } else {
                    r.status = f.no_ts ? E_NOTS : f.ts_ok ? f.rest : E_BADTS;
                }
            }
        }
    }
    const bool sd_any = valid && !(route & R_GENERIC) && (route & R_TAIL) && r.status == E_OK && f.c7 == '[';
    const uint64_t sd_ballot = __ballot(sd_any);
    const bool group_has_sd = __any(sd_any && len - f.d0 > kShortSdTail) || __popcll(sd_ballot) > 4;
    const bool sd_lane = sd_any && group_has_sd;
    FG_MARK(F);
    tick(0);
    sd2::Lds SL{};
    sd2::LineIn sin{false, 0u, 0u, 0u, false};
    sd2::LineOut slo{false, 0u, false, E_OK, 0u, 0u, 0u};
    bool sd2_ran = false;
    if constexpr (SDX) {
        if (group_has_sd) {
            const uint32_t stride16 = c.tile_cap / 16u + 16u;
            SL = sd2::carve(smem, bm16, c.tile_cap, reinterpret_cast<uint8_t*>(bm16 + 2u * stride16));
            __syncthreads();
            const bool chain = sd2::classify_tile(SL, span);
            __syncthreads();
            tick(1);
            sin = sd2::LineIn{sd_lane && (in_tile || head_only), base, f.d0, walk_len, in_tile};
            if (!chain) {
                slo = sd2::group_walk<PROF>(SL, span, sin, pc);
                sd2_ran = true;
            }
            tk = PROF ? wv::clock() : 0;
        }
    } else if (group_has_sd) {
        __syncthreads();
        rebuild_bitmap<QuoteClass>(smem, bm16, span >> 4);
        __syncthreads();
    }
    bool redo = false;
    bool coop = false;
    if (valid) {
        if (!(route & R_GENERIC)) {
            if (r.status == E_OK) {
                if (SDX && sd_lane) {
                    redo = !slo.handled;
                    if (slo.handled) {
                        r.data0 = f.d0;
                        if (slo.status != E_OK) {
                            r.status = slo.status;
                        } else {
                            r.n_ent = slo.n_ent;
                            redo = !finish_sd_tail(T, base, len, walk_len, c.last2, slo.msg_at, r, bytes, o0);
                        }
                    }
                } else if (sd_lane) {
                    redo = !parse_tail_sd_tile(T, base, f.d0, len, walk_len, c.last2, r, t, stash ? tile_w : nullptr, &rec_ok, bytes, o0);
                } else if (head_only && (route & R_TAIL)) {
                    redo = true;
                } else if (route & R_TAIL) {
                    LdsReader rd(T.w, base);
                    parse_tail(rd, f.d0, 0u, len, r, t);
                } else {
                    uint32_t e = f.e, s0 = f.s;
                    if (route & R_TRIM) {
                        LdsReader rd(T.w, base);
                        if (head_only) {
                            s0 = trim_start(rd, f.d0 + 1u, walk_len - 8u);
                            GlobalReader grd(reinterpret_cast<const uint32_t*>(bytes), o0);
                            e = trim_end(grd, 0u, len);
                            redo = s0 + 8u >= walk_len;
                        } else {
                            e = trim_end(rd, 0u, len);
                            s0 = trim_start(rd, f.d0 + 1u, len);
                        }
                    }
                    r.data0 = f.d0;
                    r.off[S_FULL] = 0;
                    r.len[S_FULL] = e;
                    r.off[S_MSG] = e > s0 ? s0 : 0u;
                    r.len[S_MSG] = e > s0 ? e - s0 : FG_NONE;
                }
            }
        } else {
            redo = !in_tile;
            if (in_tile) {
                r = Row();
#pragma unroll
                for (int k = 0; k < 6; ++k) {
                    r.off[k] = 0;
                    r.len[k] = FG_NONE;
                }
                LdsReader rd(T.w, base);
                parse_line_generic(rd, len, r, t);
            }
        }
        if (HEAD && redo && (o1 - (o0 & ~15ull)) <= (uint64_t)c.tile_cap) {
            coop = true;
            redo = false;
            slo.handled = false;
            r = Row();
#pragma unroll
            for (int k = 0; k < 6; ++k) {
                r.off[k] = 0;
                r.len[k] = FG_NONE;
            }
        }
        if (redo) {
            slo.handled = false;
            from_global = true;
            r = Row();
#pragma unroll
            for (int k = 0; k < 6; ++k) {
                r.off[k] = 0;
                r.len[k] = FG_NONE;
            }
            FG_RARE_BEGIN();
            GlobalReader rd(reinterpret_cast<const uint32_t*>(bytes), o0);
            parse_line_generic(rd, len, r, t);
            FG_RARE_END();
        }
    }

    tick(6);
    uint32_t first = 0;
    {
        const EntAlloc ea = alloc_entries_ex(t, r.n_ent, c.ent_state);
        tick(7);
        const uint32_t mine = (ea.overflow || ea.total == 0u) ? 0u : ea.s.at(ea.ex);
        if (ea.overflow) {
            r.status = FG_ST_OVERFLOW;
            r.n_ent = 0;
        }
        first = r.n_ent != 0 ? mine : 0u;
        const bool by_pairs = SDX && sd_lane && slo.handled && !from_global;
        if constexpr (SDX) {
            if (sd2_ran) sd2::group_emit(SL, t, sin, slo, by_pairs && !ea.overflow && !(ablate & 4u), first);
        }
        if (r.n_ent != 0 && !(ablate & 4u) && !by_pairs) {
            uint32_t msg_at, cnt;
            if (sd_lane && !from_global && stash && rec_ok) {
                const uint32_t* rec32 = tile_w + (((base + 3u) & ~3u) >> 2);
                for (uint32_t k0 = 0; k0 < r.n_ent; k0 += 4u) {
                    uint32_t lo[4], hi[4];
#pragma unroll
                    for (uint32_t j = 0; j < 4u; ++j) {
                        const uint32_t k = k0 + j < r.n_ent ? k0 + j : r.n_ent - 1u;
                        lo[j] = rec32[k * 2u];
                        hi[j] = rec32[k * 2u + 1u];
                    }
#pragma unroll
                    for (uint32_t j = 0; j < 4u; ++j) {
                        const uint32_t k = k0 + j;
                        if (k < r.n_ent) {
                            const uint32_t name_s = lo[j] & 0xFFFFu, name_len = lo[j] >> 16, val_len = hi[j] & 0xFFFFu;
                            const bool sdid = (hi[j] >> 17) & 1u;
                            t.ent_name[first + k] = fg_span{name_s, name_len};
                            t.ent_val[first + k] = sdid ? 0ull : ((uint64_t)(name_s + name_len + 2u) | ((uint64_t)val_len << 32));
                            t.ent_type[first + k] = sdid ? FG_T_SDID : FG_T_STRING;
                            t.ent_flags[first + k] = ((hi[j] >> 16) & 1u) ? FG_EF_VAL_ESC : 0;
                        }
                    }
                }
            } else if (from_global || (sd_lane && stash)) {
                FG_RARE_BEGIN();
                GlobalReader rd(reinterpret_cast<const uint32_t*>(bytes), o0);
                sd_walk<true>(rd, r.data0, len, &msg_at, &cnt, t, first);
                FG_RARE_END();
            } else if (sd_lane) {
                sd_walk_tile<SD_EMIT>(T, base, r.data0, walk_len, &msg_at, &cnt, t, first);
            } else if (in_tile) {
                LdsReader rd(T.w, base);
                sd_walk<true>(rd, r.data0, len, &msg_at, &cnt, t, first);
            } else {
                FG_RARE_BEGIN();
                GlobalReader rd(reinterpret_cast<const uint32_t*>(bytes), o0);
                sd_walk<true>(rd, r.data0, len, &msg_at, &cnt, t, first);
                FG_RARE_END();
            }
        }
    }

    tick(8);
    RowOut o;
    const bool ok = r.status == E_OK;
    o.meta = r.status | (r.facility << 8) | (r.severity << 16) | (r.flags << 24);
    o.ts = ok ? r.ts : 0.0;
#pragma unroll
    for (int k = 0; k < 6; ++k) o.span[k] = ok ? fg_span{r.off[k], r.len[k]} : fg_span{0, FG_NONE};
    o.first = first;
    o.count = r.n_ent;
    if constexpr (HEAD) {
        unsigned long long todo = __ballot(coop);
        while (todo) {
            const int src = (int)__builtin_ctzll(todo);
            todo &= todo - 1ull;
            auto rl64 = [&](uint64_t x) -> uint64_t {
                return (uint64_t)(uint32_t)__builtin_amdgcn_readlane((int)(uint32_t)x, src) |
                       ((uint64_t)(uint32_t)__builtin_amdgcn_readlane((int)(uint32_t)(x >> 32), src) << 32);
            };
            const uint64_t ro0 = rl64(o0), ro1 = rl64(o1), rli = rl64(c.li);
            const uint64_t ra0 = ro0 & ~15ull;
            const uint32_t rspan = (uint32_t)((ro1 - ra0 + 15ull) & ~15ull);
            __syncthreads();
            {
                __amdgpu_buffer_rsrc_t rsrc = __builtin_amdgcn_make_buffer_rsrc(const_cast<uint8_t*>(bytes + ra0), (short)0, (int)rspan, 0x00020000);
                uint4* dst = reinterpret_cast<uint4*>(const_cast<uint8_t*>(smem));
                const uint32_t nrow = (rspan + 1023u) >> 10;
                for (uint32_t r0 = 0; r0 < nrow; r0 += 4u) {
                    u32x4 w[4];
#pragma unroll
                    for (uint32_t j = 0; j < 4u; ++j) w[j] = __builtin_amdgcn_raw_buffer_load_b128(rsrc, (int)(lane * 16u + (r0 + j) * 1024u), 0, FG_STREAM_AUX);
#pragma unroll
                    for (uint32_t j = 0; j < 4u; ++j)
                        if (r0 + j < nrow) dst[(r0 + j) * kWave + lane] = make_uint4(w[j][0], w[j][1], w[j][2], w[j][3]);
                }
            }
            __syncthreads();
            GroupCtx c2{bytes, smem, bm16, ro0, ro1, ra0, rspan, lane == 0u, rli, c.stash, ablate, c.ent_state, nullptr};
            c2.tile_cap = c.tile_cap;
            Rfc5424FormatT<false, SDX, false> whole;
            const RowOut w = whole.decode(c2, t);
            auto b32 = [&](uint32_t x) -> uint32_t { return (uint32_t)__builtin_amdgcn_readfirstlane((int)x); };
            const uint32_t g_meta = b32(w.meta), g_first = b32(w.first), g_count = b32(w.count);
            const uint64_t tsb = (uint64_t)__builtin_bit_cast(unsigned long long, w.ts);
            const uint32_t g_ts0 = b32((uint32_t)tsb), g_ts1 = b32((uint32_t)(tsb >> 32));
            uint32_t g_off[6], g_len[6];
#pragma unroll
            for (int k = 0; k < 6; ++k) {
                g_off[k] = b32(w.span[k].off);
                g_len[k] = b32(w.span[k].len);
            }
            if ((int)lane == src) {
                o.meta = g_meta;
                o.ts = __builtin_bit_cast(double, (unsigned long long)((uint64_t)g_ts0 | ((uint64_t)g_ts1 << 32)));
#pragma unroll
                for (int k = 0; k < 6; ++k) o.span[k] = fg_span{g_off[k], g_len[k]};
                o.first = g_first;
                o.count = g_count;
            }
        }
    }
    tick(9);
    if (PROF && pacc && lane == 0)
        for (int k = 0; k < 10; ++k) pacc[k] += (unsigned long long)pc[k];
    return o;
    }
};

using Rfc5424Format = Rfc5424FormatT<false>;

template <int NB, bool PROF, bool HEAD = false, bool SDX = false>
__global__ __launch_bounds__(kWave, 2) void k_rfc5424(const uint8_t* __restrict__ bytes,
                                                     const uint64_t* __restrict__ offsets, uint64_t n, DevTables t,
                                                     uint32_t tile_cap, uint32_t L, uint64_t groups,
                                                     unsigned long long* prof, uint64_t* stash_base, FrameArgs fr) {
    Rfc5424FormatT<HEAD, SDX, PROF> fmt;
    if constexpr (PROF) {
        __shared__ unsigned long long pacc[10];
        if (threadIdx.x < 10) pacc[threadIdx.x] = 0ull;
        fmt.pacc = pacc;
        __syncthreads();
        persistent_loop<NB, PROF, Rfc5424FormatT<HEAD, SDX, PROF>, HEAD>(bytes, offsets, n, t, tile_cap, L, groups, prof, stash_base, fmt, fr);
        __syncthreads();
        if (prof && threadIdx.x < 10) atomicAdd(&prof[6 + threadIdx.x], pacc[threadIdx.x]);
    } else if constexpr (SDX) {
        __shared__ DevTables t_lds;
        if (threadIdx.x == 0) t_lds = t;
        __syncthreads();
        persistent_loop<NB, PROF, Rfc5424FormatT<HEAD, SDX, PROF>, HEAD>(bytes, offsets, n, t_lds, tile_cap, L, groups, prof, stash_base, fmt, fr);
    } else {
        persistent_loop<NB, PROF, Rfc5424FormatT<HEAD, SDX, PROF>, HEAD>(bytes, offsets, n, t, tile_cap, L, groups, prof, stash_base, fmt, fr);
    }
}

template <int NB, bool SDX>
__global__ __launch_bounds__(kWave, 2) void k_rfc5424_fused(const uint8_t* __restrict__ bytes, DevTables t, uint32_t tile_cap, uint32_t L,
                                                           uint64_t* stash_base, FusedArgs fa, uint32_t strip) {
    Rfc5424FormatT<false, SDX, false> fmt;
    __shared__ DevTables t_lds;
    __shared__ FusedArgs fa_lds;
    if (threadIdx.x == 0) {
        t_lds = t;
        fa_lds = fa;
    }
    __syncthreads();
    fused_loop<NB>(bytes, t_lds, tile_cap, L, fmt, fa_lds, strip, stash_base);
}

}

extern "C" uint64_t fg_stash_bytes(uint32_t blocks) {
    return (uint64_t)blocks * fg::kStashEntries * fg::kStashWords * fg::kWave * sizeof(uint64_t);
}

namespace {
template <bool HEAD, bool SDX>
auto rfc5424_kernels(const char* name) {
    return fg::kernels(fg::k_rfc5424<fg::kWindowKiB, false, HEAD, SDX>, FG_PROF_TWIN(fg::k_rfc5424<fg::kWindowKiB, true, HEAD, SDX>), name);
}
}

extern "C" int fg_launch_rfc5424(const uint8_t* d_bytes, const uint64_t* d_offsets, uint64_t n, const fg::DevTables* t,
                                 uint64_t avg_len, hipStream_t stream, uint64_t* stash, uint32_t stash_blocks, uint32_t strip,
                                 const uint8_t* line_bad, const fg_launch_opts* lo, fg::TicketSlot* tk) {
    if (n == 0) return 0;
    const fg::Variant v = fg::pick_variant(avg_len, lo->flags);
    const auto ks = v.pairs ? (v.head ? rfc5424_kernels<true, true>("rfc5424 (head, pairs)") : rfc5424_kernels<false, true>("rfc5424 (pairs)"))
                            : (v.head ? rfc5424_kernels<true, false>("rfc5424 (head)") : rfc5424_kernels<false, false>("rfc5424"));
    const fg::PlanFormat pf = v.pairs ? fg::PlanFormat().classes(2u).lds_tile(fg::sd2::extra_bytes).tile(12288u).chunk(128u).tickets_from(4u)
                              : v.head ? fg::PlanFormat()
                                       : fg::rfc5424_walk_format(avg_len);
    const uint32_t max_tile = v.pairs ? 36864u : fg::kMaxTile;
    const uint64_t plan_len = v.head ? (avg_len < fg::kHeadCap ? avg_len : fg::kHeadCap) : avg_len;
    const uint32_t sb = stash ? stash_blocks : 0u;
    if (stash_blocks == 0) stash = nullptr;
    return fg::plan_and_launch(ks, fg::DecodeCall{n, t, stream, fg::FrameArgs{strip, line_bad}, lo, tk}, plan_len, 0u, max_tile, sb, pf,
                               [&](auto k, const fg::LaunchPlan& p, const fg::DevTables& tt, const fg::FrameArgs& fr, unsigned long long* prof) {
                                   hipLaunchKernelGGL(k, dim3(p.blocks), dim3(fg::kWave), p.lds, stream, d_bytes, d_offsets, n, tt, p.tile, p.L, p.chunk,
                                                      prof, stash, fr);
                               });
}

extern "C" int fg_launch_rfc5424_fused(const uint8_t* d_bytes, uint64_t nbytes, const fg::DevTables* t, const fg::FusedGeom* g, hipStream_t stream,
                                       uint64_t* stash, uint32_t stash_blocks, uint32_t strip, int final_, uint64_t* d_offsets, uint64_t cap,
                                       uint8_t* scratch, const fg_launch_opts* lo, unsigned long long** d_total) {
    const bool sdx = g->variant == 1u;
    const auto kernel = sdx ? fg::k_rfc5424_fused<12, true> : fg::k_rfc5424_fused<16, false>;
    const uint32_t base_lds = fg::tile_lds(g->tile, sdx ? 2u : 1u) + (sdx ? fg::sd2::extra_bytes(g->tile) : 0u);
    if (stash_blocks == 0) stash = nullptr;
    return fg::launch_fused(kernel, fg::FusedCall{nbytes, t, g, stream, strip, final_, d_offsets, cap, scratch, lo, d_total}, base_lds, stash ? stash_blocks : 0u,
                            [&](auto k, uint32_t blocks, uint32_t lds, const fg::DevTables& tt, const fg::FusedArgs& fa) {
                                hipLaunchKernelGGL(k, dim3(blocks), dim3(fg::kWave), lds, stream, d_bytes, tt, g->tile, g->L, stash, fa, strip);
                            });
}
```

flowgger_amd/decoder.py:

```python
from __future__ import annotations

import ctypes as C
from typing import Iterable, List, Optional, Sequence, Tuple, Union

import numpy as np

from . import _lib as L
from .record import DecodeError, Record, parse_canonical
from .tables import DeviceTables, HostTables

_TYPE_IDS = {"string": L.FG_T_STRING, "bool": L.FG_T_BOOL, "f64": L.FG_T_F64, "i64": L.FG_T_I64, "u64": L.FG_T_U64}


def pack_lines(lines: Iterable[Union[str, bytes]]) -> Tuple[np.ndarray, np.ndarray]:
    bl = [ln.encode("utf-8", "surrogateescape") if isinstance(ln, str) else bytes(ln) for ln in lines]
    offsets = np.zeros(len(bl) + 1, np.uint64)
    if bl:
        offsets[1:] = np.cumsum([len(b) for b in bl], dtype=np.uint64)
    data = np.frombuffer(b"".join(bl), np.uint8).copy() if bl else np.zeros(0, np.uint8)
    return data, offsets


class Decoder:

    fmt: int = -1

    def __init__(self, config: Optional[dict] = None, device: int = 0):
        self._cfg = self._make_cfg(config)
        self._ctx = C.c_void_p()
        self.device = device
        L.check(L.lib().fg_create(device, C.byref(self._cfg) if self._cfg is not None else None,
                                  C.byref(self._ctx)), "fg_create")

    def _make_cfg(self, config: Optional[dict]):
        return None

    def clone_boxed(self) -> "Decoder":
        other = object.__new__(type(self))
        other._cfg = self._cfg
        other._keep = getattr(self, "_keep", None)
        other.device = self.device
        other._ctx = C.c_void_p()
        L.check(L.lib().fg_clone(self._ctx, C.byref(other._ctx)), "fg_clone")
        return other

    def set_launch_opts(self, lines_per_group: int = 0, tile_cap: int = 0, waves_per_cu: int = 0, gelf_lds_budget: int = 0,
                        gelf_window_kib: int = 0, gelf_generic: bool = False, transcode_one_piece: bool = False, chunk_lines: int = 0,
                        no_head: bool = False, force_head: bool = False, sd_walk: bool = False, sd_pairs: bool = False, no_zero_copy: bool = False, frame_kernel_upload: bool = False, frame_classic: bool = False, static_chunks: bool = False, frame_selftest_stall: bool = False, ent_chunk: int = 0, no_taper: bool = False, taper_levels: int = 0, no_fused_framing: bool = False, fused_look: int = 0, fused_ext: int = 0, rfc3164_regroup: int = 0) -> None:
        lo = L.fg_launch_opts(lines_per_group, tile_cap, waves_per_cu, gelf_lds_budget, gelf_window_kib,
                              (L.FG_LO_GELF_GENERIC if gelf_generic else 0) | (L.FG_LO_TRANSCODE_ONE_PIECE if transcode_one_piece else 0) |
                              (L.FG_LO_NO_HEAD if no_head else 0) | (L.FG_LO_FORCE_HEAD if force_head else 0) |
                              (L.FG_LO_SD_WALK if sd_walk else 0) | (L.FG_LO_SD_PAIRS if sd_pairs else 0) | (L.FG_LO_NO_ZERO_COPY if no_zero_copy else 0) | (L.FG_LO_FRAME_KERNEL_UPLOAD if frame_kernel_upload else 0) | (L.FG_LO_FRAME_CLASSIC if frame_classic else 0) | (L.FG_LO_STATIC_CHUNKS if static_chunks else 0) | (L.FG_LO_FRAME_SELFTEST_STALL if frame_selftest_stall else 0) | (L.FG_LO_NO_TAPER if no_taper else 0) | (L.FG_LO_TAPER_1 if taper_levels & 1 else 0) | (L.FG_LO_TAPER_2 if taper_levels & 2 else 0) | (L.FG_LO_NO_FUSED_FRAMING if no_fused_framing else 0) | (L.FG_LO_RFC3164_REGROUP if rfc3164_regroup == 1 else L.FG_LO_RFC3164_NO_REGROUP if rfc3164_regroup == 2 else 0),
                              chunk_lines, ent_chunk, fused_look, fused_ext)
        L.check(L.lib().fg_set_launch_opts(self._ctx, C.byref(lo)), "fg_set_launch_opts")

    def close(self) -> None:
        if getattr(self, "_ctx", None) is not None and self._ctx.value:
            L.lib().fg_destroy(self._ctx)
            self._ctx = C.c_void_p()

    def __del__(self):
        try:
            self.close()
        except Exception:
            pass

    def decode(self, line: Union[str, bytes]) -> Record:
        res = self.decode_batch([line])[0]
        if isinstance(res, DecodeError):
            raise res
        return res

    def decode_packed(self, data: np.ndarray, offsets: np.ndarray) -> HostTables:
        data = np.ascontiguousarray(data, np.uint8)
        offsets = np.ascontiguousarray(offsets, np.uint64)
        n = len(offsets) - 1
        st = L.fg_tables()
        L.check(L.lib().fg_decode_batch(self._ctx, self.fmt, data.ctypes.data, data.size,
                                        offsets.ctypes.data, n, C.byref(st)), "fg_decode_batch")
        return HostTables.from_struct(st)

    def decode_batch(self, lines: Sequence[Union[str, bytes]]) -> List[Union[Record, DecodeError]]:
        data, offsets = pack_lines(lines)
        tab = self.decode_packed(data, offsets)
        n_rows = len(offsets) - 1
        if self.fmt == L.FG_LTSV:
            import sys

            from .tables import tables_stdout

            if n_rows and bool(((tab.a["meta"][:n_rows] >> 24) & L.FG_F_LTSV_NOVALUE).any()):
                text = tables_stdout(tab, self.fmt, data, offsets)
                if text:
                    sys.stdout.write(text.decode("utf-8", "replace"))
        blob, offs = tab.serialize(self.fmt, data, offsets, cfg=self._cfg)
        raw = blob.tobytes()
        return [parse_canonical(raw[int(offs[i]):int(offs[i + 1])]) for i in range(len(lines))]

    def decode_device(self, d_bytes, d_offsets, tables: DeviceTables, stream=None) -> None:
        import torch

        if stream is None:
            stream = torch.cuda.current_stream(d_bytes.device)
        n = d_offsets.numel() - 1
        L.check(L.lib().fg_decode_batch_device(self._ctx, self.fmt, d_bytes.data_ptr(), d_bytes.numel(),
                                               d_offsets.data_ptr(), n, C.byref(tables.struct),
                                               C.c_void_p(stream.cuda_stream)), "fg_decode_batch_device")

    def frame_device(self, d_bytes, framing: int, cap_frames: Optional[int] = None, stream=None):
        import torch

        if stream is None:
            stream = torch.cuda.current_stream(d_bytes.device)
        nbytes = d_bytes.numel()
        cap = cap_frames if cap_frames is not None else nbytes // 16 + 16
        while True:
            d_offsets = torch.empty(cap + 2, dtype=torch.int64, device=d_bytes.device)
            d_bad = torch.empty(cap + 1, dtype=torch.uint8, device=d_bytes.device)
            n = C.c_uint64()
            rc = L.lib().fg_frame_device(self._ctx, framing, d_bytes.data_ptr(), nbytes, d_offsets.data_ptr(),
                                         d_bad.data_ptr(), cap, C.byref(n), C.c_void_p(stream.cuda_stream))
            if rc == L.FG_ERR_ENT_OVERFLOW:
                cap = int(n.value) + 16
                continue
            L.check(rc, "fg_frame_device")
            return d_offsets, d_bad, int(n.value)

    def frame_syslen_device(self, d_bytes, final: bool = True, cap_frames: Optional[int] = None, stream=None):
        import torch

        if stream is None:
            stream = torch.cuda.current_stream(d_bytes.device)
        nbytes = d_bytes.numel()
        cap = cap_frames if cap_frames is not None else nbytes // 32 + 16
        d_packed = torch.empty((nbytes + 15) // 16 * 16 + 16, dtype=torch.uint8, device=d_bytes.device)
        while True:
            d_offsets = torch.empty(cap + 1, dtype=torch.int64, device=d_bytes.device)
            d_starts = torch.empty(cap + 1, dtype=torch.int64, device=d_bytes.device)
            d_bad = torch.empty(max(cap, 1), dtype=torch.uint8, device=d_bytes.device)
            n, consumed, stop = C.c_uint64(), C.c_uint64(), C.c_int()
            rc = L.lib().fg_frame_syslen_device(self._ctx, d_bytes.data_ptr(), nbytes, int(final), d_packed.data_ptr(), d_offsets.data_ptr(),
                                                d_starts.data_ptr(), d_bad.data_ptr(), cap, C.byref(n), C.byref(consumed), C.byref(stop),
                                                C.c_void_p(stream.cuda_stream))
            if rc == L.FG_ERR_ENT_OVERFLOW:
                cap = int(n.value) + 16
                continue
            L.check(rc, "fg_frame_syslen_device")
            k = int(n.value)
            return d_packed, d_offsets[:k + 1], d_starts[:k + 1], d_bad[:k], k, int(consumed.value), int(stop.value)

    def frame_capnp_device(self, d_bytes, final: bool = True, cap_frames: Optional[int] = None, stream=None):
        import torch

        if stream is None:
            stream = torch.cuda.current_stream(d_bytes.device)
        nbytes = d_bytes.numel()
        cap = cap_frames if cap_frames is not None else nbytes // 64 + 16
        while True:
            d_offsets = torch.empty(cap + 1, dtype=torch.int64, device=d_bytes.device)
            n, consumed, stop = C.c_uint64(), C.c_uint64(), C.c_int()
            rc = L.lib().fg_frame_capnp_device(self._ctx, d_bytes.data_ptr(), nbytes, int(final), d_offsets.data_ptr(), cap, C.byref(n),
                                               C.byref(consumed), C.byref(stop), C.c_void_p(stream.cuda_stream))
            if rc == L.FG_ERR_ENT_OVERFLOW and cap_frames is None:
                cap = int(n.value) + 16
                continue
            L.check(rc, "fg_frame_capnp_device")
            k = int(n.value)
            return d_offsets[:k + 1], k, int(consumed.value), int(stop.value)

    def last_capnp_stop(self) -> int:
        return int(L.lib().fg_last_capnp_stop(self._ctx))

    def last_host_path(self) -> int:
        return int(L.lib().fg_last_host_path(self._ctx))

    def last_syslen_stop(self) -> int:
        return int(L.lib().fg_last_syslen_stop(self._ctx))

    def decode_frames_device(self, d_bytes, d_offsets, n: int, tables: DeviceTables, framing: int, d_bad=None,
                             stream=None) -> None:
        import torch

        if stream is None:
            stream = torch.cuda.current_stream(d_bytes.device)
        L.check(L.lib().fg_decode_frames_device(self._ctx, self.fmt, framing, d_bytes.data_ptr(), d_bytes.numel(),
                                                d_offsets.data_ptr(), n, d_bad.data_ptr() if d_bad is not None else None,
                                                C.byref(tables.struct), C.c_void_p(stream.cuda_stream)),
                "fg_decode_frames_device")

    def frame_decode_device(self, d_bytes, framing: int, tables: DeviceTables, cap_frames: int, final: bool = True, avg_line: int = 0,
                            stream=None):
        import torch

        if stream is None:
            stream = torch.cuda.current_stream(d_bytes.device)
        d_offsets = torch.empty(cap_frames + 2, dtype=torch.int64, device=d_bytes.device)
        d_result = torch.zeros(2, dtype=torch.int64, device=d_bytes.device)
        L.check(L.lib().fg_frame_decode_device(self._ctx, self.fmt, framing, d_bytes.data_ptr(), d_bytes.numel(), int(final),
                                               d_offsets.data_ptr(), cap_frames, C.byref(tables.struct), avg_line, d_result.data_ptr(),
                                               C.c_void_p(stream.cuda_stream)), "fg_frame_decode_device")
        return d_offsets, d_result

    def frame_decode_batch(self, raw: Union[bytes, np.ndarray], framing: int, final: bool = True):
        buf = np.frombuffer(raw, np.uint8) if not isinstance(raw, np.ndarray) else np.ascontiguousarray(raw, np.uint8)
        padded = np.zeros(buf.size + 16, np.uint8)
        padded[:buf.size] = buf
        st = L.fg_tables()
        off = C.c_void_p()
        n, used = C.c_uint64(), C.c_uint64()
        L.check(L.lib().fg_frame_decode_batch(self._ctx, self.fmt, framing, padded.ctypes.data, buf.size, int(final),
                                              C.byref(st), C.byref(off), C.byref(n), C.byref(used)), "fg_frame_decode_batch")
        nf = int(n.value)
        if nf == 0:
            return None, np.zeros(1, np.uint64), int(used.value)
        offsets = np.ctypeslib.as_array(C.cast(off, C.POINTER(C.c_uint64)), (nf + 1,)).copy()
        return HostTables.from_struct(st), offsets, int(used.value)

    def frame_multi_device(self, d_bytes, d_seg_starts, d_seg_final, framing: int, cap_slots: Optional[int] = None, stream=None):
        import torch

        if stream is None:
            stream = torch.cuda.current_stream(d_bytes.device)
        nbytes, K = d_bytes.numel(), d_seg_starts.numel() - 1
        cap = cap_slots if cap_slots is not None else nbytes // 16 + K + 16
        d_first = torch.empty(K + 1, dtype=torch.int64, device=d_bytes.device)
        d_cons = torch.empty(max(K, 1), dtype=torch.int64, device=d_bytes.device)
        while True:
            d_offsets = torch.empty(cap + 1, dtype=torch.int64, device=d_bytes.device)
            d_kind = torch.empty(max(cap, 1), dtype=torch.uint8, device=d_bytes.device)
            n = C.c_uint64()
            rc = L.lib().fg_frame_multi_device(self._ctx, framing, d_bytes.data_ptr(), nbytes, d_seg_starts.data_ptr(),
                                               d_seg_final.data_ptr() if d_seg_final is not None else None, K, d_offsets.data_ptr(),
                                               d_kind.data_ptr(), cap, d_first.data_ptr(), d_cons.data_ptr(), C.byref(n),
                                               C.c_void_p(stream.cuda_stream))
            if rc == L.FG_ERR_ENT_OVERFLOW and cap_slots is None:
                cap = int(n.value)
                continue
            L.check(rc, "fg_frame_multi_device")
            return d_offsets, d_kind, int(n.value), d_first, d_cons[:K]

    def frame_decode_multi(self, raw: Union[bytes, np.ndarray], seg_starts, seg_final, framing: int):
        buf = np.frombuffer(raw, np.uint8) if not isinstance(raw, np.ndarray) else np.ascontiguousarray(raw, np.uint8)
        starts = np.ascontiguousarray(seg_starts, np.uint64)
        K = len(starts) - 1
        final = None if seg_final is None else np.ascontiguousarray(seg_final, np.uint8)
        st = L.fg_tables()
        off, kind, first, cons = C.c_void_p(), C.c_void_p(), C.c_void_p(), C.c_void_p()
        n = C.c_uint64()
        L.check(L.lib().fg_frame_decode_multi_batch(self._ctx, self.fmt, framing, buf.ctypes.data if buf.size else None, buf.size,
                                                    starts.ctypes.data, final.ctypes.data if final is not None and K else None, K,
                                                    C.byref(st), C.byref(off), C.byref(kind), C.byref(first), C.byref(cons), C.byref(n)),
                "fg_frame_decode_multi_batch")
        ns = int(n.value)
        u64p, u8p = C.POINTER(C.c_uint64), C.POINTER(C.c_uint8)
        offsets = np.ctypeslib.as_array(C.cast(off, u64p), (ns + 1,)).copy()
        kinds = np.ctypeslib.as_array(C.cast(kind, u8p), (ns,)).copy() if ns else np.zeros(0, np.uint8)
        seg_first = np.ctypeslib.as_array(C.cast(first, u64p), (K + 1,)).copy()
        seg_cons = np.ctypeslib.as_array(C.cast(cons, u64p), (K,)).copy() if K else np.zeros(0, np.uint64)
        return (HostTables.from_struct(st) if ns else None), offsets, kinds, seg_first, seg_cons

    def frame_syslen_multi_device(self, d_bytes, d_seg_starts, cap_frames: Optional[int] = None, stream=None):
        import torch

        if stream is None:
            stream = torch.cuda.current_stream(d_bytes.device)
        dev = d_bytes.device
        nbytes, K = d_bytes.numel(), d_seg_starts.numel() - 1
        cap = cap_frames if cap_frames is not None else nbytes // 32 + 16
        d_packed = torch.empty((nbytes + 15) // 16 * 16 + 16, dtype=torch.uint8, device=dev)
        d_first = torch.empty(K + 1, dtype=torch.int64, device=dev)
        d_cons = torch.empty(max(K, 1), dtype=torch.int64, device=dev)
        d_stop = torch.empty(max(K, 1), dtype=torch.uint8, device=dev)
        while True:
            d_offsets = torch.empty(cap + 1, dtype=torch.int64, device=dev)
            d_starts = torch.empty(max(cap, 1), dtype=torch.int64, device=dev)
            d_bad = torch.empty(max(cap, 1), dtype=torch.uint8, device=dev)
            n, payload = C.c_uint64(), C.c_uint64()
            rc = L.lib().fg_frame_syslen_multi_device(self._ctx, d_bytes.data_ptr(), nbytes, d_seg_starts.data_ptr(), K, d_packed.data_ptr(),
                                                      d_offsets.data_ptr(), d_starts.data_ptr(), d_bad.data_ptr(), cap, d_first.data_ptr(),
                                                      d_cons.data_ptr(), d_stop.data_ptr(), C.byref(n), C.byref(payload),
                                                      C.c_void_p(stream.cuda_stream))
            if rc == L.FG_ERR_ENT_OVERFLOW and cap_frames is None:
                cap = int(n.value) + 16
                continue
            L.check(rc, "fg_frame_syslen_multi_device")
            k = int(n.value)
            return d_packed, d_offsets[:k + 1], d_starts[:k], d_bad[:k], k, d_first, d_cons[:K], d_stop[:K], int(payload.value)

    def frame_decode_syslen_multi(self, raw: Union[bytes, np.ndarray], seg_starts):
        buf = np.frombuffer(raw, np.uint8) if not isinstance(raw, np.ndarray) else np.ascontiguousarray(raw, np.uint8)
        starts = np.ascontiguousarray(seg_starts, np.uint64)
        K = len(starts) - 1
        st = L.fg_tables()
        fs, first, cons, stop = C.c_void_p(), C.c_void_p(), C.c_void_p(), C.c_void_p()
        n = C.c_uint64()
        L.check(L.lib().fg_frame_decode_syslen_multi_batch(self._ctx, self.fmt, buf.ctypes.data if buf.size else None, buf.size,
                                                           starts.ctypes.data, K, C.byref(st), C.byref(fs), C.byref(first), C.byref(cons),
                                                           C.byref(stop), C.byref(n)), "fg_frame_decode_syslen_multi_batch")
        nf = int(n.value)
        u64p, u8p = C.POINTER(C.c_uint64), C.POINTER(C.c_uint8)
        frame_starts = np.ctypeslib.as_array(C.cast(fs, u64p), (nf,)).copy() if nf else np.zeros(0, np.uint64)
        seg_first = np.ctypeslib.as_array(C.cast(first, u64p), (K + 1,)).copy()
        seg_cons = np.ctypeslib.as_array(C.cast(cons, u64p), (K,)).copy() if K else np.zeros(0, np.uint64)
        seg_stop = np.ctypeslib.as_array(C.cast(stop, u8p), (K,)).copy() if K else np.zeros(0, np.uint8)
        return (HostTables.from_struct(st) if nf else None), frame_starts, seg_first, seg_cons, seg_stop

    def frame_capnp_multi_device(self, d_bytes, d_seg_starts, cap_slots: Optional[int] = None, stream=None):
        import torch

        if stream is None:
            stream = torch.cuda.current_stream(d_bytes.device)
        dev = d_bytes.device
        nbytes, K = d_bytes.numel(), d_seg_starts.numel() - 1
        cap = cap_slots if cap_slots is not None else nbytes // 64 + K + 16
        d_first = torch.empty(K + 1, dtype=torch.int64, device=dev)
        d_cons = torch.empty(max(K, 1), dtype=torch.int64, device=dev)
        d_stop = torch.empty(max(K, 1), dtype=torch.uint8, device=dev)
        while True:
            d_offsets = torch.empty(cap + 1, dtype=torch.int64, device=dev)
            d_kind = torch.empty(max(cap, 1), dtype=torch.uint8, device=dev)
            n = C.c_uint64()
            rc = L.lib().fg_frame_capnp_multi_device(self._ctx, d_bytes.data_ptr(), nbytes, d_seg_starts.data_ptr(), K, d_offsets.data_ptr(),
                                                     d_kind.data_ptr(), cap, d_first.data_ptr(), d_cons.data_ptr(), d_stop.data_ptr(),
                                                     C.byref(n), C.c_void_p(stream.cuda_stream))
            if rc == L.FG_ERR_ENT_OVERFLOW and cap_slots is None:
                cap = int(n.value) + 16
                continue
            L.check(rc, "fg_frame_capnp_multi_device")
            k = int(n.value)
            return d_offsets[:k + 1], d_kind[:k], k, d_first, d_cons[:K], d_stop[:K]

    def frame_decode_capnp_multi(self, raw: Union[bytes, np.ndarray], seg_starts):
        buf = np.frombuffer(raw, np.uint8) if not isinstance(raw, np.ndarray) else np.ascontiguousarray(raw, np.uint8)
        starts = np.ascontiguousarray(seg_starts, np.uint64)
        K = len(starts) - 1
        st = L.fg_tables()
        off, kind, first, cons, stop = C.c_void_p(), C.c_void_p(), C.c_void_p(), C.c_void_p(), C.c_void_p()
        n = C.c_uint64()
        L.check(L.lib().fg_frame_decode_capnp_multi_batch(self._ctx, buf.ctypes.data if buf.size else None, buf.size, starts.ctypes.data, K,
                                                          C.byref(st), C.byref(off), C.byref(kind), C.byref(first), C.byref(cons),
                                                          C.byref(stop), C.byref(n)), "fg_frame_decode_capnp_multi_batch")
        ns = int(n.value)
        u64p, u8p = C.POINTER(C.c_uint64), C.POINTER(C.c_uint8)
        offsets = np.ctypeslib.as_array(C.cast(off, u64p), (ns + 1,)).copy()
        kinds = np.ctypeslib.as_array(C.cast(kind, u8p), (ns,)).copy() if ns else np.zeros(0, np.uint8)
        seg_first = np.ctypeslib.as_array(C.cast(first, u64p), (K + 1,)).copy()
        seg_cons = np.ctypeslib.as_array(C.cast(cons, u64p), (K,)).copy() if K else np.zeros(0, np.uint64)
        seg_stop = np.ctypeslib.as_array(C.cast(stop, u8p), (K,)).copy() if K else np.zeros(0, np.uint8)
        return (HostTables.from_struct(st) if ns else None), offsets, kinds, seg_first, seg_cons, seg_stop

    def udp_decode_packed(self, data: np.ndarray, offsets: np.ndarray, max_inflated: Optional[int] = None):
        data = np.ascontiguousarray(data, np.uint8)
        offsets = np.ascontiguousarray(offsets, np.uint64)
        n = len(offsets) - 1
        st = L.fg_tables()
        lines, offs, ust = C.c_void_p(), C.c_void_p(), C.c_void_p()
        L.check(L.lib().fg_udp_decode_batch(self._ctx, self.fmt, data.ctypes.data, data.size, offsets.ctypes.data, n, int(max_inflated or 0),
                                            C.byref(st), C.byref(lines), C.byref(offs), C.byref(ust)), "fg_udp_decode_batch")
        if n == 0:
            return None, np.zeros(0, np.uint8), np.zeros(1, np.uint64), np.zeros(0, np.uint8)
        line_offsets = np.ctypeslib.as_array(C.cast(offs, C.POINTER(C.c_uint64)), (n + 1,)).copy()
        total = int(line_offsets[n])
        out = np.zeros(total + 16, np.uint8)
        if total:
            out[:total] = np.ctypeslib.as_array(C.cast(lines, C.POINTER(C.c_uint8)), (total,))
        status = np.ctypeslib.as_array(C.cast(ust, C.POINTER(C.c_uint8)), (n,)).copy()
        return HostTables.from_struct(st), out[:total], line_offsets, status

    def decode_datagrams(self, datagrams: Sequence[bytes], max_inflated: Optional[int] = None) -> List[Union[Record, DecodeError]]:
        data, offsets = pack_lines(datagrams)
        if len(datagrams) == 0:
            return []
        tab, lines, line_offsets, ust = self.udp_decode_packed(data, offsets, max_inflated)
        blob, offs = tab.serialize(self.fmt, lines, line_offsets, cfg=self._cfg)
        raw = blob.tobytes()
        out: List[Union[Record, DecodeError]] = []
        for i in range(len(datagrams)):
            if ust[i] > L.FG_UDP_GZIP:
                out.append(DecodeError(L.lib().fg_udp_error_string(int(ust[i])).decode()))
            else:
                out.append(parse_canonical(raw[int(offs[i]):int(offs[i + 1])]))
        return out

    def encode_gelf_device(self, d_bytes, d_offsets, n: int, tables: DeviceTables, extra: Optional[dict] = None, stream=None):
        import torch

        if stream is None:
            stream = torch.cuda.current_stream(d_bytes.device)
        items = list((extra or {}).items())
        ks = (C.c_char_p * max(len(items), 1))(*[k.encode() for k, _ in items])
        vs = (C.c_char_p * max(len(items), 1))(*[v.encode() for _, v in items])
        ex = L.fg_gelf_extra(len(items), C.cast(ks, C.POINTER(C.c_char_p)), C.cast(vs, C.POINTER(C.c_char_p)))
        d_off = torch.empty(n + 1, dtype=torch.int64, device=d_bytes.device)
        total = C.c_uint64()
        args = (self._ctx, self.fmt, d_bytes.data_ptr(), d_bytes.numel(), d_offsets.data_ptr(), n, C.byref(tables.struct), C.byref(ex))
        L.check(L.lib().fg_encode_gelf_device(*args, None, 0, d_off.data_ptr(), C.byref(total), C.c_void_p(stream.cuda_stream)),
                "fg_encode_gelf_device (size)")
        d_out = torch.empty(max(int(total.value), 1), dtype=torch.uint8, device=d_bytes.device)
        L.check(L.lib().fg_encode_gelf_device(*args, d_out.data_ptr(), d_out.numel(), d_off.data_ptr(), C.byref(total),
                                              C.c_void_p(stream.cuda_stream)), "fg_encode_gelf_device")
        return d_out[:int(total.value)], d_off

    def set_timing(self, enabled: bool = True) -> None:
        L.check(L.lib().fg_set_timing(self._ctx, int(enabled)), "fg_set_timing")

    def last_kernel_ms(self) -> float:
        ms = C.c_float()
        L.check(L.lib().fg_last_kernel_ms(self._ctx, C.byref(ms)), "fg_last_kernel_ms")
        return float(ms.value)

    def error_string(self, status: int) -> Optional[str]:
        s = L.lib().fg_error_string(self.fmt, status)
        return None if s is None else s.decode()


class UdpUnpacker:

    def __init__(self, decoder: Decoder, max_inflated: Optional[int] = None):
        self.decoder = decoder
        self.max_inflated = int(max_inflated or 0)

    def unpack(self, d_bytes, d_offsets, stream=None):
        import torch

        if stream is None:
            stream = torch.cuda.current_stream(d_bytes.device)
        n = d_offsets.numel() - 1
        dev = d_bytes.device
        d_off = torch.zeros(n + 1, dtype=torch.int64, device=dev)
        d_drop = torch.zeros(max(n, 1), dtype=torch.uint8, device=dev)
        d_st = torch.zeros(max(n, 1), dtype=torch.uint8, device=dev)
        total = C.c_uint64()
        args = (self.decoder._ctx, d_bytes.data_ptr(), d_bytes.numel(), d_offsets.data_ptr(), n, self.max_inflated)
        tail = (d_off.data_ptr(), d_drop.data_ptr(), d_st.data_ptr(), C.byref(total), C.c_void_p(stream.cuda_stream))
        L.check(L.lib().fg_udp_unpack_device(*args, None, 0, *tail), "fg_udp_unpack_device (size)")
        cap = int(total.value)
        d_out = torch.zeros((cap + 15) // 16 * 16 + 16, dtype=torch.uint8, device=dev)
        L.check(L.lib().fg_udp_unpack_device(*args, d_out.data_ptr(), cap, *tail), "fg_udp_unpack_device")
        return d_out[:cap], d_off, d_drop[:n], d_st[:n]


class FlushPolicy:

    def __init__(self, max_bytes: int = 8 << 20, max_latency_ms: float = 5.0):
        self.max_bytes, self.max_latency_ms = max_bytes, max_latency_ms


_RUST_WS = "\t\n\x0b\x0c\r \x85\xa0\u1680\u2000\u2001\u2002\u2003\u2004\u2005\u2006\u2007\u2008\u2009\u200a\u2028\u2029\u202f\u205f\u3000"


class MultiStreamSplitter:

    def __init__(self, decoder: Decoder, framing: int, policy: Optional[FlushPolicy] = None):
        if framing not in (L.FG_FRAME_LINE, L.FG_FRAME_NUL):
            raise ValueError("MultiStreamSplitter frames FG_FRAME_LINE or FG_FRAME_NUL streams")
        self.decoder, self.framing, self.policy = decoder, framing, policy or FlushPolicy()
        self._carry: dict = {}
        self._pending: dict = {}
        self._closed: set = set()
        self._bytes = 0
        self._first_at: Optional[float] = None

    def push(self, conn_id, chunk: bytes) -> list:
        import time

        if conn_id in self._closed:
            raise ValueError("push after close")
        if chunk:
            self._pending.setdefault(conn_id, []).append(bytes(chunk))
            self._bytes += len(chunk)
            if self._first_at is None:
                self._first_at = time.monotonic()
        due = self._bytes >= self.policy.max_bytes or (
            self._first_at is not None and (time.monotonic() - self._first_at) * 1e3 >= self.policy.max_latency_ms)
        return self.flush() if due else []

    def close(self, conn_id) -> None:
        self._closed.add(conn_id)
        self._pending.setdefault(conn_id, [])

    def pending_bytes(self) -> int:
        return self._bytes

    def flush(self) -> list:
        conns = list(self._pending)
        segs = [self._carry.pop(c, b"") + b"".join(self._pending[c]) for c in conns]
        final = [1 if c in self._closed else 0 for c in conns]
        self._pending, self._bytes, self._first_at = {}, 0, None
        for c in conns:
            self._closed.discard(c)
        if not conns:
            return []
        raw = b"".join(segs)
        starts = np.zeros(len(segs) + 1, np.uint64)
        starts[1:] = np.cumsum([len(s) for s in segs], dtype=np.uint64)
        tab, offsets, kind, first, _ = self.decoder.frame_decode_multi(raw, starts, final, self.framing)
        fmt, out = self.decoder.fmt, []
        can, coffs = b"", None
        if tab is not None:
            data = np.frombuffer(raw + b"\0" * 32, np.uint8)
            if fmt == L.FG_LTSV and bool(((tab.a["meta"][:tab.n] >> 24) & L.FG_F_LTSV_NOVALUE).any()):
                import sys

                from .tables import tables_stdout

                text = tables_stdout(tab, fmt, data, offsets, self.framing)
                if text:
                    sys.stdout.write(text.decode("utf-8", "replace"))
            blob, coffs = tab.serialize(fmt, data, offsets, cfg=self.decoder._cfg)
            can = blob.tobytes()
        for k, c in enumerate(conns):
            res: list = []
            for i in range(int(first[k]), int(first[k + 1])):
                a, b = int(offsets[i]), int(offsets[i + 1])
                if kind[i] == L.FG_SLOT_CARRY:
                    self._carry[c] = raw[a:b]
                elif kind[i] == L.FG_SLOT_BAD_UTF8:
                    res.append(DecodeError("Invalid UTF-8 input"))
                else:
                    r = parse_canonical(can[int(coffs[i]):int(coffs[i + 1])])
                    if isinstance(r, DecodeError):
                        line = raw[a:b]
                        if self.framing == L.FG_FRAME_LINE:
                            line = line[:-2] if line.endswith(b"\r\n") else line[:-1] if line.endswith(b"\n") else line
                        elif line.endswith(b"\0"):
                            line = line[:-1]
                        text = line.decode("utf-8").strip(_RUST_WS)
                        if self.framing == L.FG_FRAME_NUL and not text:
                            continue
                        r = DecodeError(f"{r}: [{text}]")
                    res.append(r)
            out.append((c, res))
        return out


SYSLEN_BAD_LENGTH = "Can't read message's length"
SYSLEN_SHORT_READ = "failed to fill whole buffer"
SYSLEN_PANIC = "thread panicked: called `Result::unwrap()` on an `Err` value: FromUtf8Error (syslen_splitter.rs:32)"


class MultiSyslenSplitter:

    def __init__(self, decoder: Decoder, policy: Optional[FlushPolicy] = None):
        self.decoder, self.policy = decoder, policy or FlushPolicy()
        self._carry: dict = {}
        self._pending: dict = {}
        self._closed: set = set()
        self._over: set = set()
        self._bytes = 0
        self._first_at: Optional[float] = None

    def push(self, conn_id, chunk: bytes) -> list:
        import time

        if conn_id in self._closed or conn_id in self._over:
            raise ValueError("push after the connection ended")
        if chunk:
            self._pending.setdefault(conn_id, []).append(bytes(chunk))
            self._bytes += len(chunk)
            if self._first_at is None:
                self._first_at = time.monotonic()
        due = self._bytes >= self.policy.max_bytes or (
            self._first_at is not None and (time.monotonic() - self._first_at) * 1e3 >= self.policy.max_latency_ms)
        return self.flush() if due else []

    def close(self, conn_id) -> None:
        if conn_id not in self._over:
            self._closed.add(conn_id)
            self._pending.setdefault(conn_id, [])

    def pending_bytes(self) -> int:
        return self._bytes

    def _decode_error(self, r: DecodeError, payload: bytes) -> DecodeError:
        return DecodeError(f"{r}: [{payload.decode('utf-8').strip(_RUST_WS)}]")

    def _eof(self, tail: bytes) -> list:
        sp = tail.find(b" ")
        if sp >= 0:
            return [DecodeError(SYSLEN_SHORT_READ)]
        num = tail[:-1]
        body = num[1:] if num[:1] == b"+" else num
        if len(tail) <= 1 or not body or not body.isdigit() or int(body) >= 1 << 64:
            return [DecodeError(SYSLEN_BAD_LENGTH)]
        if int(body) != 0:
            return [DecodeError(SYSLEN_SHORT_READ)]
        r = self.decoder.decode_batch([b""])[0]
        return [self._decode_error(r, b"") if isinstance(r, DecodeError) else r, DecodeError(SYSLEN_BAD_LENGTH)]

    def flush(self) -> list:
        conns = list(self._pending)
        segs = [self._carry.pop(c, b"") + b"".join(self._pending[c]) for c in conns]
        self._pending, self._bytes, self._first_at = {}, 0, None
        if not conns:
            return []
        raw = b"".join(segs)
        starts = np.zeros(len(segs) + 1, np.uint64)
        starts[1:] = np.cumsum([len(s) for s in segs], dtype=np.uint64)
        tab, fstart, first, cons, stop = self.decoder.frame_decode_syslen_multi(raw, starts)
        fmt = self.decoder.fmt
        payloads = []
        for a in fstart:
            sp = raw.index(b" ", int(a))
            payloads.append(raw[sp + 1:sp + 1 + int(raw[int(a):sp])])
        can, coffs = b"", None
        if tab is not None:
            data, offsets = pack_lines(payloads)
            data = np.concatenate([data, np.zeros(32, np.uint8)])
            if fmt == L.FG_LTSV and bool(((tab.a["meta"][:tab.n] >> 24) & L.FG_F_LTSV_NOVALUE).any()):
                import sys

                from .tables import tables_stdout

                text = tables_stdout(tab, fmt, data, offsets)
                if text:
                    sys.stdout.write(text.decode("utf-8", "replace"))
            blob, coffs = tab.serialize(fmt, data, offsets, cfg=self.decoder._cfg)
            can = blob.tobytes()
            status = tab.a["meta"][:tab.n] & 0xFF
        out = []
        for k, c in enumerate(conns):
            res: list = []
            over = False
            for i in range(int(first[k]), int(first[k + 1])):
                if status[i] == L.FG_ST_BAD_UTF8:
                    res.append(DecodeError(SYSLEN_PANIC))
                    over = True
                    break
                r = parse_canonical(can[int(coffs[i]):int(coffs[i + 1])])
                res.append(self._decode_error(r, payloads[i]) if isinstance(r, DecodeError) else r)
            if not over and stop[k] == L.FG_SYSLEN_BAD_LEN:
                res.append(DecodeError(SYSLEN_BAD_LENGTH))
                over = True
            tail = segs[k][int(cons[k]):]
            if not over and c in self._closed:
                res += self._eof(tail) if tail else [DecodeError(SYSLEN_BAD_LENGTH)]
                over = True
            self._closed.discard(c)
            if over:
                self._over.add(c)
            elif tail:
                self._carry[c] = tail
            out.append((c, res))
        return out


class RFC5424Decoder(Decoder):
    fmt = L.FG_RFC5424


class GelfDecoder(Decoder):
    fmt = L.FG_GELF


def pack_messages(messages: Iterable[bytes]) -> Tuple[np.ndarray, np.ndarray]:
    bl = [bytes(m) for m in messages]
    for i, b in enumerate(bl):
        if len(b) & 7:
            raise ValueError(f"message {i}: {len(b)} bytes is not a whole number of 8-byte words")
    offsets = np.zeros(len(bl) + 1, np.uint64)
    if bl:
        offsets[1:] = np.cumsum([len(b) for b in bl], dtype=np.uint64)
    data = np.frombuffer(b"".join(bl), np.uint8).copy() if bl else np.zeros(0, np.uint8)
    return data, offsets


class CapnpStreamError(Exception):

    def __init__(self, text: str, offsets=None, consumed: int = 0):
        super().__init__(text)
        self.offsets = np.zeros(1, np.uint64) if offsets is None else offsets
        self.consumed = consumed


class CapnpFramer:

    MAX_SEGMENTS = 512
    MAX_WORDS = 8 << 20

    def __init__(self):
        self._carry = b""
        self._ended = None

    @classmethod
    def frame(cls, buf: Union[bytes, memoryview]) -> Tuple[np.ndarray, int]:
        import struct

        mv = memoryview(buf)
        offs, p, n_buf = [0], 0, len(mv)
        while n_buf - p >= 8:
            n = struct.unpack_from("<I", mv, p)[0] + 1
            if n >= cls.MAX_SEGMENTS:
                raise CapnpStreamError(f"Too many segments: {n}", np.array(offs, np.uint64), p)
            table = (4 + 4 * n + 7) // 8 * 8
            if n_buf - p < table:
                break
            words = sum(struct.unpack_from(f"<{n}I", mv, p + 4))
            if words > cls.MAX_WORDS:
                raise CapnpStreamError(f"Message has {words} words, which is too large", np.array(offs, np.uint64), p)
            if n_buf - p < table + 8 * words:
                break
            p += table + 8 * words
            offs.append(p)
        return np.array(offs, np.uint64), p

    def feed(self, chunk: bytes) -> Tuple[np.ndarray, np.ndarray]:
        if self._ended is not None:
            raise self._ended
        buf = self._carry + bytes(chunk)
        try:
            offsets, consumed = self.frame(buf)
        except CapnpStreamError as e:
            self._ended = e
            if len(e.offsets) < 2:
                raise
            offsets, consumed = e.offsets, e.consumed
        self._carry = buf[consumed:]
        return np.frombuffer(buf[:consumed], np.uint8).copy(), offsets

    @property
    def pending(self) -> int:
        return len(self._carry)


class _GpuCapnpCarry:

    def __init__(self):
        self._carry = b""
        self._ended = None

    def begin(self, chunk: bytes) -> bytes:
        if self._ended is not None:
            raise self._ended
        return self._carry + bytes(chunk)

    def end(self, buf: bytes, n: int, consumed: int, stop: int) -> None:
        self._carry = buf[consumed:]
        if stop in (L.FG_CAPNP_TOO_MANY_SEGMENTS, L.FG_CAPNP_TOO_LARGE):
            try:
                CapnpFramer.frame(self._carry)
                raise AssertionError("the device framer stopped at a table the host walk accepts")
            except CapnpStreamError as e:
                self._ended = e
            if n == 0:
                raise self._ended

    @property
    def pending(self) -> int:
        return len(self._carry)


class CapnpDecoder(Decoder):
    fmt = L.FG_CAPNP

    def decode_batch(self, lines: Sequence[bytes]) -> List[Union[Record, DecodeError]]:
        data, offsets = pack_messages(lines)
        tab = self.decode_packed(data, offsets)
        blob, offs = tab.serialize(self.fmt, data, offsets)
        raw = blob.tobytes()
        return [parse_canonical(raw[int(offs[i]):int(offs[i + 1])]) for i in range(len(lines))]


class CapnpSplitter:

    def __init__(self, decoder: Optional[CapnpDecoder] = None, device: int = 0, gpu_framing: bool = False):
        self.decoder = decoder or CapnpDecoder(device=device)
        self.framer = _GpuCapnpCarry() if gpu_framing else CapnpFramer()
        self.gpu_framing = gpu_framing

    def feed(self, chunk: bytes) -> List[Union[Record, DecodeError]]:
        if self.gpu_framing:
            buf = self.framer.begin(chunk)
            tab, offsets, consumed = self.decoder.frame_decode_batch(buf, L.FG_FRAME_CAPNP, final=False)
            n = len(offsets) - 1
            self.framer.end(buf, n, consumed, self.decoder.last_capnp_stop())
            data = np.frombuffer(buf[:consumed], np.uint8)
        else:
            data, offsets = self.framer.feed(chunk)
            n = len(offsets) - 1
            tab = self.decoder.decode_packed(data, offsets) if n else None
        if n == 0:
            return []
        blob, offs = tab.serialize(L.FG_CAPNP, data, offsets)
        raw = blob.tobytes()
        return [parse_canonical(raw[int(offs[i]):int(offs[i + 1])]) for i in range(n)]


class MultiCapnpSplitter:

    def __init__(self, decoder: Optional[CapnpDecoder] = None, policy: Optional[FlushPolicy] = None):
        self.decoder, self.policy = decoder or CapnpDecoder(), policy or FlushPolicy()
        self._carry: dict = {}
        self._pending: dict = {}
        self._closed: set = set()
        self._over: set = set()
        self._bytes = 0
        self._first_at: Optional[float] = None

    def push(self, conn_id, chunk: bytes) -> list:
        import time

        if conn_id in self._closed or conn_id in self._over:
            raise ValueError("push after the connection ended")
        if chunk:
            self._pending.setdefault(conn_id, []).append(bytes(chunk))
            self._bytes += len(chunk)
            if self._first_at is None:
                self._first_at = time.monotonic()
        due = self._bytes >= self.policy.max_bytes or (
            self._first_at is not None and (time.monotonic() - self._first_at) * 1e3 >= self.policy.max_latency_ms)
        return self.flush() if due else []

    def close(self, conn_id) -> None:
        if conn_id not in self._over:
            self._closed.add(conn_id)
            self._pending.setdefault(conn_id, [])

    def pending_bytes(self) -> int:
        return self._bytes

    def flush(self) -> list:
        conns = list(self._pending)
        whole = [self._carry.pop(c, b"") + b"".join(self._pending[c]) for c in conns]
        self._pending, self._bytes, self._first_at = {}, 0, None
        if not conns:
            return []
        segs = [w[:len(w) & ~7] for w in whole]
        raw = b"".join(segs)
        starts = np.zeros(len(segs) + 1, np.uint64)
        starts[1:] = np.cumsum([len(s) for s in segs], dtype=np.uint64)
        tab, offsets, kind, first, cons, stop = self.decoder.frame_decode_capnp_multi(raw, starts)
        can, coffs = b"", None
        if tab is not None:
            blob, coffs = tab.serialize(L.FG_CAPNP, np.frombuffer(raw + b"\0" * 32, np.uint8), offsets)
            can = blob.tobytes()
        out = []
        for k, c in enumerate(conns):
            res: list = [parse_canonical(can[int(coffs[i]):int(coffs[i + 1])]) for i in range(int(first[k]), int(first[k + 1]))
                         if kind[i] == L.FG_SLOT_FRAME]
            tail = whole[k][int(cons[k]):]
            over = c in self._closed
            if stop[k] in (L.FG_CAPNP_TOO_MANY_SEGMENTS, L.FG_CAPNP_TOO_LARGE):
                try:
                    CapnpFramer.frame(tail)
                    raise AssertionError("the framer stopped at a table the host walk accepts")
                except CapnpStreamError as e:
                    res.append(e)
                over = True
            self._closed.discard(c)
            if over:
                self._over.add(c)
            elif tail:
                self._carry[c] = tail
            out.append((c, res))
        return out


class CapnpTranscodingSplitter:

    def __init__(self, encoder, decoder: Optional[CapnpDecoder] = None, device: int = 0, now_ts: float = 0.0, gpu_framing: bool = False):
        from .encoder import Pipeline

        self.decoder = decoder or CapnpDecoder(device=device)
        self.pipeline = Pipeline(self.decoder, encoder)
        self.framer = _GpuCapnpCarry() if gpu_framing else CapnpFramer()
        self.gpu_framing = gpu_framing
        self.now_ts = now_ts

    def feed(self, chunk: bytes):
        from .encoder import Transcoded

        if self.gpu_framing:
            buf = self.framer.begin(chunk)
            res = self.pipeline.run_stream(buf, L.FG_FRAME_CAPNP, final=False, now_ts=self.now_ts)
            self.framer.end(buf, len(res.out_offsets) - 1, res.consumed, self.decoder.last_capnp_stop())
            return res
        data, offsets = self.framer.feed(chunk)
        if len(offsets) < 2:
            return Transcoded(np.zeros(0, np.uint8), np.zeros(1, np.uint64), np.zeros(0, np.uint32), np.zeros(0, np.uint8), None, 0)
        return self.pipeline.run_packed(data, offsets, now_ts=self.now_ts)


class RFC3164Decoder(Decoder):
    fmt = L.FG_RFC3164

    def __init__(self, config: Optional[dict] = None, device: int = 0):
        super().__init__(config, device)
        from . import tzdb

        opt = (config or {}).get("rfc3164", {})
        self.current_year = int(opt.get("current_year", L.FG_YEAR_NOW))
        zones = opt.get("zones", "all")
        self.tz_table = tzdb.default_table() if zones == "all" else (tzdb.build_table(zones) if zones else None)
        self._apply()

    def _apply(self):
        cfg = L.fg_rfc3164_cfg(self.current_year, None)
        t = self.tz_table
        if t is not None and len(t.names):
            names = (C.c_char_p * len(t.names))(*[n.encode() for n in t.names])
            zf = np.ascontiguousarray(t.zone_first, np.uint32)
            us = np.ascontiguousarray(t.utc_start, np.int64)
            uo = np.ascontiguousarray(t.utc_offset, np.int32)
            tab = L.fg_tz_table(len(t.names), C.cast(names, C.POINTER(C.c_char_p)), zf.ctypes.data, us.ctypes.data, uo.ctypes.data)
            cfg.tz = C.pointer(tab)
            self._keep3164 = (names, zf, us, uo, tab)
        L.check(L.lib().fg_set_rfc3164(self._ctx, C.byref(cfg)), "fg_set_rfc3164")

    def clone_boxed(self) -> "Decoder":
        other = super().clone_boxed()
        other.current_year, other.tz_table = self.current_year, self.tz_table
        return other


class LTSVDecoder(Decoder):
    fmt = L.FG_LTSV

    def _make_cfg(self, config: Optional[dict]):
        inp = (config or {}).get("input", {})
        schema = inp.get("ltsv_schema")
        suffixes = inp.get("ltsv_suffixes")
        cfg = L.fg_cfg()
        keep = []
        names, types = [], []
        if schema is not None:
            if not isinstance(schema, dict):
                raise ValueError("input.ltsv_schema must be a list of key/type pairs")
            for name, sdtype in schema.items():
                if not isinstance(sdtype, str):
                    raise ValueError("input.ltsv_schema types must be strings")
                t = _TYPE_IDS.get(sdtype.lower())
                if t is None:
                    raise ValueError(f"Unsupported type in input.ltsv_schema for name [{name}]")
                names.append(name.encode())
                types.append(t)
        cfg.n_schema = len(names)
        arr_n = (C.c_char_p * max(len(names), 1))(*names)
        arr_t = (C.c_uint8 * max(len(types), 1))(*types)
        cfg.schema_names = C.cast(arr_n, C.POINTER(C.c_char_p))
        cfg.schema_types = C.cast(arr_t, C.POINTER(C.c_uint8))
        keep += [arr_n, arr_t, names]
        if suffixes is not None:
            if not isinstance(suffixes, dict):
                raise ValueError("input.ltsv_suffixes must be a list of type/suffixes pairs")
            for sdtype, suffix in suffixes.items():
                if not isinstance(suffix, str):
                    raise ValueError("input.ltsv_suffixes suffixes must be strings")
                t = sdtype.lower()
                if t == "string":
                    raise ValueError("Strings cannot be suffixed")
                if t not in ("bool", "f64", "i64", "u64"):
                    raise ValueError(f"Unsupported type in input.ltsv_suffixes for type [{sdtype}]")
                setattr(cfg, "suffix_" + t, suffix.encode())
        self._keep = keep
        return cfg
```

include/fg_hip.h:

```cpp
#ifndef FG_HIP_H
#define FG_HIP_H
#include <stdint.h>

#ifdef __cplusplus
extern "C" {
#endif

#define FG_ABI_VERSION 4

typedef enum fg_format { FG_RFC5424 = 0, FG_LTSV = 1, FG_GELF = 2, FG_RFC3164 = 3, FG_CAPNP = 4 } fg_format;

enum {
    FG_OK = 0,
    FG_ERR_ARG = -1,
    FG_ERR_HIP = -2,
    FG_ERR_NO_DEVICE = -3,
    FG_ERR_ENT_OVERFLOW = -4,
    FG_ERR_UNSUPPORTED = -5,
    FG_ERR_NOMEM = -6
};

enum {
    FG_T_STRING = 0, FG_T_BOOL = 1, FG_T_F64 = 2, FG_T_I64 = 3, FG_T_U64 = 4, FG_T_NULL = 5,
    FG_T_SDID = 6
};

#define FG_NONE 0xFFFFFFFFu
typedef struct fg_span { uint32_t off; uint32_t len; } fg_span;

#define FG_META_STATUS(m)   ((uint8_t)((m) & 0xFF))
#define FG_META_FACILITY(m) ((uint8_t)(((m) >> 8) & 0xFF))
#define FG_META_SEVERITY(m) ((uint8_t)(((m) >> 16) & 0xFF))
#define FG_META_FLAGS(m)    ((uint8_t)(((m) >> 24) & 0xFF))
enum {
    FG_F_TS_NOW = 1,
    FG_F_HOST_ESC = 2,
    FG_F_MSG_ESC = 4,
    FG_F_FULLMSG_ESC = 8,
    FG_F_BOM = 16,
    FG_F_GELF_RETRY = 32,
    FG_F_MSG_JOIN = 64,
    FG_F_LTSV_NOVALUE = 128
};
#define FG_ST_OVERFLOW 0xFE
#define FG_ST_BAD_UTF8 0xFD

typedef enum fg_framing {
    FG_FRAME_NONE = 0,
    FG_FRAME_LINE = 1,
    FG_FRAME_NUL = 2,
    FG_FRAME_SYSLEN = 3,
    FG_FRAME_CAPNP = 4
} fg_framing;

typedef enum fg_capnp_stop {
    FG_CAPNP_CLEAN = 0,
    FG_CAPNP_TAIL = 1,
    FG_CAPNP_TOO_MANY_SEGMENTS = 2,
    FG_CAPNP_TOO_LARGE = 3
} fg_capnp_stop;

typedef enum fg_syslen_stop {
    FG_SYSLEN_CLEAN = 0,
    FG_SYSLEN_TAIL = 1,
    FG_SYSLEN_BAD_LEN = 2,
    FG_SYSLEN_LONG_PREFIX = 3
} fg_syslen_stop;
#define FG_SYSLEN_MAX_PREFIX 24u

static inline uint32_t FG_SYSLEN_PREFIX_LEN(const uint8_t* frame, uint64_t frame_len) {
    uint32_t k = 0;
    while (k < frame_len && frame[k] != (uint8_t)' ') ++k;
    return k < frame_len ? k + 1u : (uint32_t)frame_len;
}

enum {
    FG_EF_VAL_ESC = 1,
    FG_EF_NAME_ESC = 2,
    FG_EF_SUFFIX = 4,
    FG_EF_NAME_VERBATIM = 8
};

typedef struct fg_tables {
    uint64_t n;
    uint64_t ent_cap;
    uint32_t* meta;
    double*   ts;
    fg_span*  hostname;
    fg_span*  appname;
    fg_span*  procid;
    fg_span*  msgid;
    fg_span*  msg;
    fg_span*  full_msg;
    uint32_t* ent_first;
    uint32_t* ent_count;
    fg_span*  ent_name;
    uint64_t* ent_val;
    uint8_t*  ent_type;
    uint8_t*  ent_flags;
    uint64_t* ent_used;
} fg_tables;

#define FG_ROW_BYTES 68u
#define FG_ENT_BYTES 18u

typedef struct fg_cfg {
    uint32_t n_schema;
    const char* const* schema_names;
    const uint8_t* schema_types;
    const char* suffix_bool;
    const char* suffix_f64;
    const char* suffix_i64;
    const char* suffix_u64;
} fg_cfg;

typedef struct fg_tz_table {
    uint32_t n_zones;
    const char* const* names;
    const uint32_t* zone_first;
    const int64_t* utc_start;
    const int32_t* utc_offset;
} fg_tz_table;
#define FG_YEAR_NOW (-2147483647 - 1)
typedef struct fg_rfc3164_cfg {
    int32_t current_year;
    const fg_tz_table* tz;
} fg_rfc3164_cfg;

typedef struct fg_ctx fg_ctx;
#define FG_STREAM_OWN ((void*)(intptr_t)-1)

int fg_abi_version(void);

typedef struct fg_launch_opts {
    uint32_t lines_per_group;
    uint32_t tile_cap;
    uint32_t waves_per_cu;
    uint32_t gelf_lds_budget;
    uint32_t gelf_window_kib;
    uint32_t flags;
    uint32_t chunk_lines;
    uint32_t ent_chunk;
    uint32_t fused_look;
    uint32_t fused_ext;
} fg_launch_opts;
enum {
    FG_LO_GELF_GENERIC = 1,
    FG_LO_TRANSCODE_ONE_PIECE = 2,
    FG_LO_NO_HEAD = 4,
    FG_LO_FORCE_HEAD = 8,
    FG_LO_SD_WALK = 16,
    FG_LO_SD_PAIRS = 32,
    FG_LO_NO_ZERO_COPY = 64,
    FG_LO_FRAME_KERNEL_UPLOAD = 128,
    FG_LO_FRAME_CLASSIC = 256,
    FG_LO_STATIC_CHUNKS = 512,
    FG_LO_FRAME_SELFTEST_STALL = 1024,
    FG_LO_NO_TAPER = 2048,
    FG_LO_TAPER_1 = 4096,
    FG_LO_TAPER_2 = 8192,
    FG_LO_NO_FUSED_FRAMING = 16384,
    FG_LO_RFC3164_REGROUP = 32768,
    FG_LO_RFC3164_NO_REGROUP = 65536,
    FG_LO_RESERVED = 0x40000000
};

int fg_create(int device, const fg_cfg* cfg, fg_ctx** out);
int fg_clone(const fg_ctx* ctx, fg_ctx** out);
void fg_destroy(fg_ctx* ctx);
int fg_last_hip_error(const fg_ctx* ctx);
int fg_set_launch_opts(fg_ctx* ctx, const fg_launch_opts* opts);
int fg_set_rfc3164(fg_ctx* ctx, const fg_rfc3164_cfg* cfg);

#define FG_TABLE_ARRAYS 15
int fg_tables_layout(uint64_t n, uint64_t ent_cap, uint64_t sizes[FG_TABLE_ARRAYS]);

int fg_decode_batch_device(fg_ctx* ctx, fg_format fmt, const uint8_t* d_bytes, uint64_t nbytes,
                           const uint64_t* d_offsets, uint64_t n, const fg_tables* tables,
                           void* stream);

int fg_frame_device(fg_ctx* ctx, fg_framing framing, const uint8_t* d_bytes, uint64_t nbytes,
                    uint64_t* d_offsets, uint8_t* d_bad_utf8, uint64_t cap_frames, uint64_t* n_frames,
                    void* stream);

typedef enum fg_slot_kind { FG_SLOT_FRAME = 0, FG_SLOT_BAD_UTF8 = 1, FG_SLOT_CARRY = 2 } fg_slot_kind;
int fg_frame_multi_device(fg_ctx* ctx, fg_framing framing, const uint8_t* d_bytes, uint64_t nbytes,
                          const uint64_t* d_seg_starts, const uint8_t* d_seg_final, uint64_t n_segs,
                          uint64_t* d_offsets, uint8_t* d_kind, uint64_t cap_slots,
                          uint64_t* d_seg_first, uint64_t* d_seg_consumed, uint64_t* n_slots, void* stream);

int fg_decode_frames_device(fg_ctx* ctx, fg_format fmt, fg_framing framing, const uint8_t* d_bytes,
                            uint64_t nbytes, const uint64_t* d_offsets, uint64_t n,
                            const uint8_t* d_bad_utf8, const fg_tables* tables, void* stream);


int fg_frame_syslen_device(fg_ctx* ctx, const uint8_t* d_bytes, uint64_t nbytes, int final, uint8_t* d_packed, uint64_t* d_offsets,
                           uint64_t* d_frame_starts, uint8_t* d_bad_utf8, uint64_t cap_frames, uint64_t* n_frames, uint64_t* consumed,
                           int* stop_reason, void* stream);
int fg_frame_syslen_multi_device(fg_ctx* ctx, const uint8_t* d_bytes, uint64_t nbytes, const uint64_t* d_seg_starts, uint64_t n_segs,
                                 uint8_t* d_packed, uint64_t* d_offsets, uint64_t* d_frame_starts, uint8_t* d_bad_utf8, uint64_t cap_frames,
                                 uint64_t* d_seg_first, uint64_t* d_seg_consumed, uint8_t* d_seg_stop, uint64_t* n_frames,
                                 uint64_t* payload_bytes, void* stream);
#define FG_CAPNP_FRAME_MAX_BYTES 0xFFFF0000ull
int fg_frame_capnp_device(fg_ctx* ctx, const uint8_t* d_bytes, uint64_t nbytes, int final, uint64_t* d_offsets, uint64_t cap_frames,
                          uint64_t* n_frames, uint64_t* consumed, int* stop_reason, void* stream);
int fg_frame_capnp_multi_device(fg_ctx* ctx, const uint8_t* d_bytes, uint64_t nbytes, const uint64_t* d_seg_starts, uint64_t n_segs,
                                uint64_t* d_offsets, uint8_t* d_kind, uint64_t cap_slots, uint64_t* d_seg_first, uint64_t* d_seg_consumed,
                                uint8_t* d_seg_stop, uint64_t* n_slots, void* stream);
int fg_frame_decode_device(fg_ctx* ctx, fg_format fmt, fg_framing framing, const uint8_t* d_bytes, uint64_t nbytes, int final,
                           uint64_t* d_offsets, uint64_t cap_frames, const fg_tables* tables, uint64_t avg_line_hint,
                           uint64_t* d_result, void* stream);

typedef enum fg_udp_status {
    FG_UDP_RAW = 0,
    FG_UDP_ZLIB = 1,
    FG_UDP_GZIP = 2,
    FG_UDP_BAD_ZLIB = 3,
    FG_UDP_BAD_GZIP = 4,
    FG_UDP_BAD_UTF8 = 5,
    FG_UDP_TOO_LARGE = 6
} fg_udp_status;
#define FG_UDP_DEFAULT_MAX_INFLATED 327635u
#define FG_UDP_MAX_MAX_INFLATED 0x7FFFFFF0u
const char* fg_udp_error_string(uint8_t st);
int fg_udp_unpack_device(fg_ctx* ctx, const uint8_t* d_bytes, uint64_t nbytes, const uint64_t* d_offsets, uint64_t n,
                         uint64_t max_inflated, uint8_t* d_out, uint64_t out_cap, uint64_t* d_out_offsets,
                         uint8_t* d_drop, uint8_t* d_udp_status, uint64_t* total, void* stream);

int fg_decode_batch(fg_ctx* ctx, fg_format fmt, const uint8_t* bytes, uint64_t nbytes,
                    const uint64_t* offsets, uint64_t n, fg_tables* out);

int fg_frame_decode_batch(fg_ctx* ctx, fg_format fmt, fg_framing framing, const uint8_t* bytes,
                          uint64_t nbytes, int final, fg_tables* out, const uint64_t** out_offsets,
                          uint64_t* n_frames, uint64_t* consumed);

int fg_frame_decode_multi_batch(fg_ctx* ctx, fg_format fmt, fg_framing framing, const uint8_t* bytes, uint64_t nbytes,
                                const uint64_t* seg_starts, const uint8_t* seg_final, uint64_t n_segs,
                                fg_tables* out, const uint64_t** out_offsets, const uint8_t** out_kind,
                                const uint64_t** out_seg_first, const uint64_t** out_seg_consumed, uint64_t* n_slots);

int fg_frame_decode_syslen_multi_batch(fg_ctx* ctx, fg_format fmt, const uint8_t* bytes, uint64_t nbytes, const uint64_t* seg_starts,
                                       uint64_t n_segs, fg_tables* out, const uint64_t** out_frame_starts, const uint64_t** out_seg_first,
                                       const uint64_t** out_seg_consumed, const uint8_t** out_seg_stop, uint64_t* n_frames);

int fg_frame_decode_capnp_multi_batch(fg_ctx* ctx, const uint8_t* bytes, uint64_t nbytes, const uint64_t* seg_starts, uint64_t n_segs,
                                      fg_tables* out, const uint64_t** out_offsets, const uint8_t** out_kind, const uint64_t** out_seg_first,
                                      const uint64_t** out_seg_consumed, const uint8_t** out_seg_stop, uint64_t* n_slots);

int fg_udp_decode_batch(fg_ctx* ctx, fg_format fmt, const uint8_t* bytes, uint64_t nbytes, const uint64_t* offsets, uint64_t n,
                        uint64_t max_inflated, fg_tables* out, const uint8_t** out_lines, const uint64_t** out_line_offsets,
                        const uint8_t** udp_status);

enum {
    FG_PATH_DECODE_ZERO_COPY = 1,
    FG_PATH_DECODE_SLICED = 2,
    FG_PATH_FRAME_FUSED = 3,
    FG_PATH_FRAME_SLICED = 4,
    FG_PATH_FRAME_ONE_PIECE = 5,
    FG_PATH_FRAME_SYSLEN_DEVICE = 6,
    FG_PATH_FRAME_SYSLEN_HOST = 7,
    FG_PATH_FRAME_CAPNP_DEVICE = 8,
    FG_PATH_FRAME_CAPNP_HOST = 9,
    FG_PATH_FRAME_MULTI = 10,
    FG_PATH_FRAME_SYSLEN_MULTI_DEVICE = 11,
    FG_PATH_FRAME_SYSLEN_MULTI_HOST = 12,
    FG_PATH_FRAME_CAPNP_MULTI_DEVICE = 13,
    FG_PATH_FRAME_CAPNP_MULTI_HOST = 14
};
int fg_last_host_path(const fg_ctx* ctx);
int fg_last_capnp_stop(const fg_ctx* ctx);
int fg_last_syslen_stop(const fg_ctx* ctx);

typedef struct fg_gelf_extra {
    uint32_t n;
    const char* const* keys;
    const char* const* values;
} fg_gelf_extra;
int fg_encode_gelf_device(fg_ctx* ctx, fg_format src_fmt, const uint8_t* d_bytes, uint64_t nbytes,
                          const uint64_t* d_offsets, uint64_t n, const fg_tables* tables,
                          const fg_gelf_extra* extra, uint8_t* d_out, uint64_t out_cap,
                          uint64_t* d_out_offsets, uint64_t* total, void* stream);

typedef enum fg_encoder { FG_ENC_GELF = 0, FG_ENC_LTSV = 1, FG_ENC_RFC5424 = 2, FG_ENC_RFC3164 = 3, FG_ENC_PASSTHROUGH = 4, FG_ENC_CAPNP = 5 } fg_encoder;
typedef enum fg_merger { FG_MERGE_NONE = 0, FG_MERGE_LINE = 1, FG_MERGE_NUL = 2, FG_MERGE_SYSLEN = 3 } fg_merger;
typedef struct fg_encode_cfg {
    fg_encoder encoder;
    fg_merger merger;
    uint32_t n_extra;
    const char* const* extra_keys;
    const char* const* extra_values;
    const char* prepend;
    double now_ts;
} fg_encode_cfg;
int fg_encode_device(fg_ctx* ctx, fg_format src_fmt, const fg_encode_cfg* cfg, const uint8_t* d_bytes, uint64_t nbytes,
                     const uint64_t* d_offsets, uint64_t n, const fg_tables* tables, uint8_t* d_out, uint64_t out_cap,
                     uint64_t* d_out_offsets, uint8_t* d_enc_status, uint64_t* total, void* stream);

int fg_encode_device_async(fg_ctx* ctx, fg_format src_fmt, const fg_encode_cfg* cfg, const uint8_t* d_bytes, uint64_t nbytes,
                           const uint64_t* d_offsets, uint64_t n, const fg_tables* tables, uint8_t* d_out, uint64_t out_cap,
                           uint64_t* d_out_offsets, uint8_t* d_enc_status, uint64_t ent_hint, void* stream);
const char* fg_encode_error_string(uint8_t enc_status);

typedef struct fg_transcoded {
    const uint8_t* out;
    uint64_t out_bytes;
    const uint64_t* out_offsets;
    const uint32_t* meta;
    const uint8_t* enc_status;
    const uint64_t* frame_offsets;
    uint64_t n;
    uint64_t consumed;
} fg_transcoded;
int fg_transcode_batch(fg_ctx* ctx, fg_format fmt, fg_framing framing, const fg_encode_cfg* cfg, const uint8_t* bytes,
                       uint64_t nbytes, const uint64_t* offsets, uint64_t n, int final, fg_transcoded* out);

int fg_alloc_pinned(uint64_t bytes, void** out);
void fg_free_pinned(void* p);
int fg_set_pinned_limits(uint64_t total_bytes, uint64_t idle_bytes);
int fg_pinned_stats(uint64_t* pinned_bytes, uint64_t* idle_bytes, uint64_t* live_blocks);
int fg_is_pinned(const void* p);

int fg_measure_link(fg_ctx* ctx, uint64_t nbytes, double gbps[3]);

enum { FG_CALIB_COPY = 0, FG_CALIB_READ = 1,
       FG_CALIB_COPY_NT = 2,
       FG_CALIB_COPY_FLAT = 3  };
int fg_calibrate_device(fg_ctx* ctx, int mode, const uint8_t* d_src, uint8_t* d_dst, uint64_t nbytes, void* stream);

const char* fg_error_string(fg_format fmt, uint8_t status);

int64_t fg_tables_serialize(fg_format fmt, const fg_cfg* cfg, const uint8_t* bytes,
                            const uint64_t* offsets, const fg_tables* tables, uint64_t i0,
                            uint64_t i1, uint8_t* out, uint64_t cap, uint64_t* out_offsets);

int64_t fg_tables_stdout(fg_format fmt, fg_framing framing, const uint8_t* bytes, const uint64_t* offsets, const fg_tables* tables,
                         uint64_t i0, uint64_t i1, uint8_t* out, uint64_t cap);

int fg_shard_plan(const uint64_t* offsets, uint64_t n, uint32_t g, uint64_t* line_starts);

int fg_gather_size(const fg_tables* parts, uint32_t g, uint64_t* n_rows, uint64_t* n_entries);
int fg_merge_tables_device(fg_ctx* ctx, const fg_tables* parts, uint32_t g, const uint64_t* const* d_index, const fg_tables* out,
                           uint8_t* d_src_part, void* stream);
int fg_gather_tables(const fg_tables* parts, uint32_t g, fg_tables* out);
int fg_merge_tables(const fg_tables* parts, uint32_t g, const uint64_t* const* index, fg_tables* out, uint8_t* src_part);
int64_t fg_ordered_merge(uint32_t g, const uint64_t* m, const uint64_t* const* index, const uint8_t* const* blobs,
                         const uint64_t* const* offs, uint8_t* out, uint64_t cap, uint64_t* out_offs);

int fg_set_timing(fg_ctx* ctx, int enabled);
int fg_last_kernel_ms(fg_ctx* ctx, float* ms);

int fg_ticket_ring_check(fg_ctx* ctx);

#ifdef __cplusplus
}
#endif
#endif
```

integration/rust/fg-hip-sys/src/lib.rs:

```rust
#![allow(non_camel_case_types, non_upper_case_globals, non_snake_case, dead_code)]
use std::os::raw::{c_char, c_int, c_void};

pub const FG_ABI_VERSION: c_int = 4;
pub type fg_format = c_int;
pub const FG_RFC5424: fg_format = 0;
pub const FG_LTSV: fg_format = 1;
pub const FG_GELF: fg_format = 2;
pub const FG_RFC3164: fg_format = 3;
pub const FG_CAPNP: fg_format = 4;

pub const FG_OK: c_int = 0;
pub const FG_ERR_ARG: c_int = -1;
pub const FG_ERR_HIP: c_int = -2;
pub const FG_ERR_NO_DEVICE: c_int = -3;
pub const FG_ERR_ENT_OVERFLOW: c_int = -4;
pub const FG_ERR_UNSUPPORTED: c_int = -5;
pub const FG_ERR_NOMEM: c_int = -6;

pub const FG_T_STRING: c_int = 0;
pub const FG_T_BOOL: c_int = 1;
pub const FG_T_F64: c_int = 2;
pub const FG_T_I64: c_int = 3;
pub const FG_T_U64: c_int = 4;
pub const FG_T_NULL: c_int = 5;
pub const FG_T_SDID: c_int = 6;

pub const FG_NONE: u32 = 0xFFFFFFFF;
#[repr(C)]
#[derive(Clone, Copy)]
pub struct fg_span {
    pub off: u32,
    pub len: u32,
}

#[inline] pub const fn FG_META_STATUS(m: u32) -> u8 { ((m >> 0) & 0xFF) as u8 }
#[inline] pub const fn FG_META_FACILITY(m: u32) -> u8 { ((m >> 8) & 0xFF) as u8 }
#[inline] pub const fn FG_META_SEVERITY(m: u32) -> u8 { ((m >> 16) & 0xFF) as u8 }
#[inline] pub const fn FG_META_FLAGS(m: u32) -> u8 { ((m >> 24) & 0xFF) as u8 }
pub const FG_F_TS_NOW: c_int = 1;
pub const FG_F_HOST_ESC: c_int = 2;
pub const FG_F_MSG_ESC: c_int = 4;
pub const FG_F_FULLMSG_ESC: c_int = 8;
pub const FG_F_BOM: c_int = 16;
pub const FG_F_GELF_RETRY: c_int = 32;
pub const FG_F_MSG_JOIN: c_int = 64;
pub const FG_F_LTSV_NOVALUE: c_int = 128;

pub const FG_ST_OVERFLOW: u8 = 254;
pub const FG_ST_BAD_UTF8: u8 = 253;
pub type fg_framing = c_int;
pub const FG_FRAME_NONE: fg_framing = 0;
pub const FG_FRAME_LINE: fg_framing = 1;
pub const FG_FRAME_NUL: fg_framing = 2;
pub const FG_FRAME_SYSLEN: fg_framing = 3;
pub const FG_FRAME_CAPNP: fg_framing = 4;

pub type fg_capnp_stop = c_int;
pub const FG_CAPNP_CLEAN: fg_capnp_stop = 0;
pub const FG_CAPNP_TAIL: fg_capnp_stop = 1;
pub const FG_CAPNP_TOO_MANY_SEGMENTS: fg_capnp_stop = 2;
pub const FG_CAPNP_TOO_LARGE: fg_capnp_stop = 3;

pub type fg_syslen_stop = c_int;
pub const FG_SYSLEN_CLEAN: fg_syslen_stop = 0;
pub const FG_SYSLEN_TAIL: fg_syslen_stop = 1;
pub const FG_SYSLEN_BAD_LEN: fg_syslen_stop = 2;
pub const FG_SYSLEN_LONG_PREFIX: fg_syslen_stop = 3;

pub const FG_SYSLEN_MAX_PREFIX: u32 = 24;
pub const FG_EF_VAL_ESC: c_int = 1;
pub const FG_EF_NAME_ESC: c_int = 2;
pub const FG_EF_SUFFIX: c_int = 4;
pub const FG_EF_NAME_VERBATIM: c_int = 8;

#[repr(C)]
#[derive(Clone, Copy)]
pub struct fg_tables {
    pub n: u64,
    pub ent_cap: u64,
    pub meta: *mut u32,
    pub ts: *mut f64,
    pub hostname: *mut fg_span,
    pub appname: *mut fg_span,
    pub procid: *mut fg_span,
    pub msgid: *mut fg_span,
    pub msg: *mut fg_span,
    pub full_msg: *mut fg_span,
    pub ent_first: *mut u32,
    pub ent_count: *mut u32,
    pub ent_name: *mut fg_span,
    pub ent_val: *mut u64,
    pub ent_type: *mut u8,
    pub ent_flags: *mut u8,
    pub ent_used: *mut u64,
}

pub const FG_ROW_BYTES: u32 = 68;
pub const FG_ENT_BYTES: u32 = 18;
#[repr(C)]
#[derive(Clone, Copy)]
pub struct fg_cfg {
    pub n_schema: u32,
    pub schema_names: *const *const c_char,
    pub schema_types: *const u8,
    pub suffix_bool: *const c_char,
    pub suffix_f64: *const c_char,
    pub suffix_i64: *const c_char,
    pub suffix_u64: *const c_char,
}

#[repr(C)]
#[derive(Clone, Copy)]
pub struct fg_tz_table {
    pub n_zones: u32,
    pub names: *const *const c_char,
    pub zone_first: *const u32,
    pub utc_start: *const i64,
    pub utc_offset: *const i32,
}

pub const FG_YEAR_NOW: c_int = -2147483648;
#[repr(C)]
#[derive(Clone, Copy)]
pub struct fg_rfc3164_cfg {
    pub current_year: i32,
    pub tz: *const fg_tz_table,
}

#[repr(C)] pub struct fg_ctx { _private: [u8; 0] }

pub const FG_STREAM_OWN: *mut c_void = usize::MAX as *mut c_void;
#[repr(C)]
#[derive(Clone, Copy)]
pub struct fg_launch_opts {
    pub lines_per_group: u32,
    pub tile_cap: u32,
    pub waves_per_cu: u32,
    pub gelf_lds_budget: u32,
    pub gelf_window_kib: u32,
    pub flags: u32,
    pub chunk_lines: u32,
    pub ent_chunk: u32,
    pub fused_look: u32,
    pub fused_ext: u32,
}

pub const FG_LO_GELF_GENERIC: c_int = 1;
pub const FG_LO_TRANSCODE_ONE_PIECE: c_int = 2;
pub const FG_LO_NO_HEAD: c_int = 4;
pub const FG_LO_FORCE_HEAD: c_int = 8;
pub const FG_LO_SD_WALK: c_int = 16;
pub const FG_LO_SD_PAIRS: c_int = 32;
pub const FG_LO_NO_ZERO_COPY: c_int = 64;
pub const FG_LO_FRAME_KERNEL_UPLOAD: c_int = 128;
pub const FG_LO_FRAME_CLASSIC: c_int = 256;
pub const FG_LO_STATIC_CHUNKS: c_int = 512;
pub const FG_LO_FRAME_SELFTEST_STALL: c_int = 1024;
pub const FG_LO_NO_TAPER: c_int = 2048;
pub const FG_LO_TAPER_1: c_int = 4096;
pub const FG_LO_TAPER_2: c_int = 8192;
pub const FG_LO_NO_FUSED_FRAMING: c_int = 16384;
pub const FG_LO_RFC3164_REGROUP: c_int = 32768;
pub const FG_LO_RFC3164_NO_REGROUP: c_int = 65536;
pub const FG_LO_RESERVED: c_int = 1073741824;

pub const FG_TABLE_ARRAYS: c_int = 15;
pub type fg_slot_kind = c_int;
pub const FG_SLOT_FRAME: fg_slot_kind = 0;
pub const FG_SLOT_BAD_UTF8: fg_slot_kind = 1;
pub const FG_SLOT_CARRY: fg_slot_kind = 2;

pub const FG_CAPNP_FRAME_MAX_BYTES: u32 = 0xFFFF0000;
pub type fg_udp_status = c_int;
pub const FG_UDP_RAW: fg_udp_status = 0;
pub const FG_UDP_ZLIB: fg_udp_status = 1;
pub const FG_UDP_GZIP: fg_udp_status = 2;
pub const FG_UDP_BAD_ZLIB: fg_udp_status = 3;
pub const FG_UDP_BAD_GZIP: fg_udp_status = 4;
pub const FG_UDP_BAD_UTF8: fg_udp_status = 5;
pub const FG_UDP_TOO_LARGE: fg_udp_status = 6;

pub const FG_UDP_DEFAULT_MAX_INFLATED: u32 = 0x4FFD3;
pub const FG_UDP_MAX_MAX_INFLATED: u32 = 0x7FFFFFF0;
pub const FG_PATH_DECODE_ZERO_COPY: c_int = 1;
pub const FG_PATH_DECODE_SLICED: c_int = 2;
pub const FG_PATH_FRAME_FUSED: c_int = 3;
pub const FG_PATH_FRAME_SLICED: c_int = 4;
pub const FG_PATH_FRAME_ONE_PIECE: c_int = 5;
pub const FG_PATH_FRAME_SYSLEN_DEVICE: c_int = 6;
pub const FG_PATH_FRAME_SYSLEN_HOST: c_int = 7;
pub const FG_PATH_FRAME_CAPNP_DEVICE: c_int = 8;
pub const FG_PATH_FRAME_CAPNP_HOST: c_int = 9;
pub const FG_PATH_FRAME_MULTI: c_int = 10;
pub const FG_PATH_FRAME_SYSLEN_MULTI_DEVICE: c_int = 11;
pub const FG_PATH_FRAME_SYSLEN_MULTI_HOST: c_int = 12;
pub const FG_PATH_FRAME_CAPNP_MULTI_DEVICE: c_int = 13;
pub const FG_PATH_FRAME_CAPNP_MULTI_HOST: c_int = 14;

#[repr(C)]
#[derive(Clone, Copy)]
pub struct fg_gelf_extra {
    pub n: u32,
    pub keys: *const *const c_char,
    pub values: *const *const c_char,
}

pub type fg_encoder = c_int;
pub const FG_ENC_GELF: fg_encoder = 0;
pub const FG_ENC_LTSV: fg_encoder = 1;
pub const FG_ENC_RFC5424: fg_encoder = 2;
pub const FG_ENC_RFC3164: fg_encoder = 3;
pub const FG_ENC_PASSTHROUGH: fg_encoder = 4;
pub const FG_ENC_CAPNP: fg_encoder = 5;

pub type fg_merger = c_int;
pub const FG_MERGE_NONE: fg_merger = 0;
pub const FG_MERGE_LINE: fg_merger = 1;
pub const FG_MERGE_NUL: fg_merger = 2;
pub const FG_MERGE_SYSLEN: fg_merger = 3;

#[repr(C)]
#[derive(Clone, Copy)]
pub struct fg_encode_cfg {
    pub encoder: fg_encoder,
    pub merger: fg_merger,
    pub n_extra: u32,
    pub extra_keys: *const *const c_char,
    pub extra_values: *const *const c_char,
    pub prepend: *const c_char,
    pub now_ts: f64,
}

#[repr(C)]
#[derive(Clone, Copy)]
pub struct fg_transcoded {
    pub out: *const u8,
    pub out_bytes: u64,
    pub out_offsets: *const u64,
    pub meta: *const u32,
    pub enc_status: *const u8,
    pub frame_offsets: *const u64,
    pub n: u64,
    pub consumed: u64,
}

pub const FG_CALIB_COPY: c_int = 0;
pub const FG_CALIB_READ: c_int = 1;
pub const FG_CALIB_COPY_NT: c_int = 2;
pub const FG_CALIB_COPY_FLAT: c_int = 3;

#[link(name = "fg_hip")]
extern "C" {
    pub fn fg_abi_version() -> c_int;
    pub fn fg_create(device: c_int, cfg: *const fg_cfg, out: *mut *mut fg_ctx) -> c_int;
    pub fn fg_clone(ctx: *const fg_ctx, out: *mut *mut fg_ctx) -> c_int;
    pub fn fg_destroy(ctx: *mut fg_ctx);
    pub fn fg_last_hip_error(ctx: *const fg_ctx) -> c_int;
    pub fn fg_set_launch_opts(ctx: *mut fg_ctx, opts: *const fg_launch_opts) -> c_int;
    pub fn fg_set_rfc3164(ctx: *mut fg_ctx, cfg: *const fg_rfc3164_cfg) -> c_int;
    pub fn fg_tables_layout(n: u64, ent_cap: u64, sizes: *mut u64) -> c_int;
    pub fn fg_decode_batch_device(
        ctx: *mut fg_ctx,
        fmt: fg_format,
        d_bytes: *const u8,
        nbytes: u64,
        d_offsets: *const u64,
        n: u64,
        tables: *const fg_tables,
        stream: *mut c_void,
    ) -> c_int;
    pub fn fg_frame_device(
        ctx: *mut fg_ctx,
        framing: fg_framing,
        d_bytes: *const u8,
        nbytes: u64,
        d_offsets: *mut u64,
        d_bad_utf8: *mut u8,
        cap_frames: u64,
        n_frames: *mut u64,
        stream: *mut c_void,
    ) -> c_int;
    pub fn fg_frame_multi_device(
        ctx: *mut fg_ctx,
        framing: fg_framing,
        d_bytes: *const u8,
        nbytes: u64,
        d_seg_starts: *const u64,
        d_seg_final: *const u8,
        n_segs: u64,
        d_offsets: *mut u64,
        d_kind: *mut u8,
        cap_slots: u64,
        d_seg_first: *mut u64,
        d_seg_consumed: *mut u64,
        n_slots: *mut u64,
        stream: *mut c_void,
    ) -> c_int;
    pub fn fg_decode_frames_device(
        ctx: *mut fg_ctx,
        fmt: fg_format,
        framing: fg_framing,
        d_bytes: *const u8,
        nbytes: u64,
        d_offsets: *const u64,
        n: u64,
        d_bad_utf8: *const u8,
        tables: *const fg_tables,
        stream: *mut c_void,
    ) -> c_int;
    pub fn fg_frame_syslen_device(
        ctx: *mut fg_ctx,
        d_bytes: *const u8,
        nbytes: u64,
        is_final: c_int,
        d_packed: *mut u8,
        d_offsets: *mut u64,
        d_frame_starts: *mut u64,
        d_bad_utf8: *mut u8,
        cap_frames: u64,
        n_frames: *mut u64,
        consumed: *mut u64,
        stop_reason: *mut c_int,
        stream: *mut c_void,
    ) -> c_int;
    pub fn fg_frame_syslen_multi_device(
        ctx: *mut fg_ctx,
        d_bytes: *const u8,
        nbytes: u64,
        d_seg_starts: *const u64,
        n_segs: u64,
        d_packed: *mut u8,
        d_offsets: *mut u64,
        d_frame_starts: *mut u64,
        d_bad_utf8: *mut u8,
        cap_frames: u64,
        d_seg_first: *mut u64,
        d_seg_consumed: *mut u64,
        d_seg_stop: *mut u8,
        n_frames: *mut u64,
        payload_bytes: *mut u64,
        stream: *mut c_void,
    ) -> c_int;
    pub fn fg_frame_capnp_device(
        ctx: *mut fg_ctx,
        d_bytes: *const u8,
        nbytes: u64,
        is_final: c_int,
        d_offsets: *mut u64,
        cap_frames: u64,
        n_frames: *mut u64,
        consumed: *mut u64,
        stop_reason: *mut c_int,
        stream: *mut c_void,
    ) -> c_int;
    pub fn fg_frame_capnp_multi_device(
        ctx: *mut fg_ctx,
        d_bytes: *const u8,
        nbytes: u64,
        d_seg_starts: *const u64,
        n_segs: u64,
        d_offsets: *mut u64,
        d_kind: *mut u8,
        cap_slots: u64,
        d_seg_first: *mut u64,
        d_seg_consumed: *mut u64,
        d_seg_stop: *mut u8,
        n_slots: *mut u64,
        stream: *mut c_void,
    ) -> c_int;
    pub fn fg_frame_decode_device(
        ctx: *mut fg_ctx,
        fmt: fg_format,
        framing: fg_framing,
        d_bytes: *const u8,
        nbytes: u64,
        is_final: c_int,
        d_offsets: *mut u64,
        cap_frames: u64,
        tables: *const fg_tables,
        avg_line_hint: u64,
        d_result: *mut u64,
        stream: *mut c_void,
    ) -> c_int;
    pub fn fg_udp_error_string(st: u8) -> *const c_char;
    pub fn fg_udp_unpack_device(
        ctx: *mut fg_ctx,
        d_bytes: *const u8,
        nbytes: u64,
        d_offsets: *const u64,
        n: u64,
        max_inflated: u64,
        d_out: *mut u8,
        out_cap: u64,
        d_out_offsets: *mut u64,
        d_drop: *mut u8,
        d_udp_status: *mut u8,
        total: *mut u64,
        stream: *mut c_void,
    ) -> c_int;
    pub fn fg_decode_batch(
        ctx: *mut fg_ctx,
        fmt: fg_format,
        bytes: *const u8,
        nbytes: u64,
        offsets: *const u64,
        n: u64,
        out: *mut fg_tables,
    ) -> c_int;
    pub fn fg_frame_decode_batch(
        ctx: *mut fg_ctx,
        fmt: fg_format,
        framing: fg_framing,
        bytes: *const u8,
        nbytes: u64,
        is_final: c_int,
        out: *mut fg_tables,
        out_offsets: *mut *const u64,
        n_frames: *mut u64,
        consumed: *mut u64,
    ) -> c_int;
    pub fn fg_frame_decode_multi_batch(
        ctx: *mut fg_ctx,
        fmt: fg_format,
        framing: fg_framing,
        bytes: *const u8,
        nbytes: u64,
        seg_starts: *const u64,
        seg_final: *const u8,
        n_segs: u64,
        out: *mut fg_tables,
        out_offsets: *mut *const u64,
        out_kind: *mut *const u8,
        out_seg_first: *mut *const u64,
        out_seg_consumed: *mut *const u64,
        n_slots: *mut u64,
    ) -> c_int;
    pub fn fg_frame_decode_syslen_multi_batch(
        ctx: *mut fg_ctx,
        fmt: fg_format,
        bytes: *const u8,
        nbytes: u64,
        seg_starts: *const u64,
        n_segs: u64,
        out: *mut fg_tables,
        out_frame_starts: *mut *const u64,
        out_seg_first: *mut *const u64,
        out_seg_consumed: *mut *const u64,
        out_seg_stop: *mut *const u8,
        n_frames: *mut u64,
    ) -> c_int;
    pub fn fg_frame_decode_capnp_multi_batch(
        ctx: *mut fg_ctx,
        bytes: *const u8,
        nbytes: u64,
        seg_starts: *const u64,
        n_segs: u64,
        out: *mut fg_tables,
        out_offsets: *mut *const u64,
        out_kind: *mut *const u8,
        out_seg_first: *mut *const u64,
        out_seg_consumed: *mut *const u64,
        out_seg_stop: *mut *const u8,
        n_slots: *mut u64,
    ) -> c_int;
    pub fn fg_udp_decode_batch(
        ctx: *mut fg_ctx,
        fmt: fg_format,
        bytes: *const u8,
        nbytes: u64,
        offsets: *const u64,
        n: u64,
        max_inflated: u64,
        out: *mut fg_tables,
        out_lines: *mut *const u8,
        out_line_offsets: *mut *const u64,
        udp_status: *mut *const u8,
    ) -> c_int;
    pub fn fg_last_host_path(ctx: *const fg_ctx) -> c_int;
    pub fn fg_last_capnp_stop(ctx: *const fg_ctx) -> c_int;
    pub fn fg_last_syslen_stop(ctx: *const fg_ctx) -> c_int;
    pub fn fg_encode_gelf_device(
        ctx: *mut fg_ctx,
        src_fmt: fg_format,
        d_bytes: *const u8,
        nbytes: u64,
        d_offsets: *const u64,
        n: u64,
        tables: *const fg_tables,
        extra: *const fg_gelf_extra,
        d_out: *mut u8,
        out_cap: u64,
        d_out_offsets: *mut u64,
        total: *mut u64,
        stream: *mut c_void,
    ) -> c_int;
    pub fn fg_encode_device(
        ctx: *mut fg_ctx,
        src_fmt: fg_format,
        cfg: *const fg_encode_cfg,
        d_bytes: *const u8,
        nbytes: u64,
        d_offsets: *const u64,
        n: u64,
        tables: *const fg_tables,
        d_out: *mut u8,
        out_cap: u64,
        d_out_offsets: *mut u64,
        d_enc_status: *mut u8,
        total: *mut u64,
        stream: *mut c_void,
    ) -> c_int;
    pub fn fg_encode_device_async(
        ctx: *mut fg_ctx,
        src_fmt: fg_format,
        cfg: *const fg_encode_cfg,
        d_bytes: *const u8,
        nbytes: u64,
        d_offsets: *const u64,
        n: u64,
        tables: *const fg_tables,
        d_out: *mut u8,
        out_cap: u64,
        d_out_offsets: *mut u64,
        d_enc_status: *mut u8,
        ent_hint: u64,
        stream: *mut c_void,
    ) -> c_int;
    pub fn fg_encode_error_string(enc_status: u8) -> *const c_char;
    pub fn fg_transcode_batch(
        ctx: *mut fg_ctx,
        fmt: fg_format,
        framing: fg_framing,
        cfg: *const fg_encode_cfg,
        bytes: *const u8,
        nbytes: u64,
        offsets: *const u64,
        n: u64,
        is_final: c_int,
        out: *mut fg_transcoded,
    ) -> c_int;
    pub fn fg_alloc_pinned(bytes: u64, out: *mut *mut c_void) -> c_int;
    pub fn fg_free_pinned(p: *mut c_void);
    pub fn fg_set_pinned_limits(total_bytes: u64, idle_bytes: u64) -> c_int;
    pub fn fg_pinned_stats(pinned_bytes: *mut u64, idle_bytes: *mut u64, live_blocks: *mut u64) -> c_int;
    pub fn fg_is_pinned(p: *const c_void) -> c_int;
    pub fn fg_measure_link(ctx: *mut fg_ctx, nbytes: u64, gbps: *mut f64) -> c_int;
    pub fn fg_calibrate_device(
        ctx: *mut fg_ctx,
        mode: c_int,
        d_src: *const u8,
        d_dst: *mut u8,
        nbytes: u64,
        stream: *mut c_void,
    ) -> c_int;
    pub fn fg_error_string(fmt: fg_format, status: u8) -> *const c_char;
    pub fn fg_tables_serialize(
        fmt: fg_format,
        cfg: *const fg_cfg,
        bytes: *const u8,
        offsets: *const u64,
        tables: *const fg_tables,
        i0: u64,
        i1: u64,
        out: *mut u8,
        cap: u64,
        out_offsets: *mut u64,
    ) -> i64;
    pub fn fg_tables_stdout(
        fmt: fg_format,
        framing: fg_framing,
        bytes: *const u8,
        offsets: *const u64,
        tables: *const fg_tables,
        i0: u64,
        i1: u64,
        out: *mut u8,
        cap: u64,
    ) -> i64;
    pub fn fg_shard_plan(offsets: *const u64, n: u64, g: u32, line_starts: *mut u64) -> c_int;
    pub fn fg_gather_size(parts: *const fg_tables, g: u32, n_rows: *mut u64, n_entries: *mut u64) -> c_int;
    pub fn fg_merge_tables_device(
        ctx: *mut fg_ctx,
        parts: *const fg_tables,
        g: u32,
        d_index: *const *const u64,
        out: *const fg_tables,
        d_src_part: *mut u8,
        stream: *mut c_void,
    ) -> c_int;
    pub fn fg_gather_tables(parts: *const fg_tables, g: u32, out: *mut fg_tables) -> c_int;
    pub fn fg_merge_tables(
        parts: *const fg_tables,
        g: u32,
        index: *const *const u64,
        out: *mut fg_tables,
        src_part: *mut u8,
    ) -> c_int;
    pub fn fg_ordered_merge(
        g: u32,
        m: *const u64,
        index: *const *const u64,
        blobs: *const *const u8,
        offs: *const *const u64,
        out: *mut u8,
        cap: u64,
        out_offs: *mut u64,
    ) -> i64;
    pub fn fg_set_timing(ctx: *mut fg_ctx, enabled: c_int) -> c_int;
    pub fn fg_last_kernel_ms(ctx: *mut fg_ctx, ms: *mut f32) -> c_int;
    pub fn fg_ticket_ring_check(ctx: *mut fg_ctx) -> c_int;
}
```

Baseline: 16.33 billion lines/s.

## Add sparse-window RFC5424 kernel loading only each line's head and tail chunks

Adds a sparse RFC5424 decode path that builds a per-window need bitmap in LDS, marking only the first 96 bytes and the last few bytes of each line. Buffer loads for unneeded 16-byte chunks are pushed out of range so they return zeros instead of reading HBM. Lines whose parse needs bytes past the head are flagged as handed. When more than a handful of lines in a group are flagged, the next window is loaded densely, and cooperative lines still use the whole-line fallback. The goal is to cut HBM traffic for lines without structured data, at the cost of extra LDS atomics, barriers, a waitcnt, and possible dense reloads for irregular input.

```diff
diff --git a/flowgger_amd/_lib.py b/flowgger_amd/_lib.py
--- a/flowgger_amd/_lib.py
+++ b/flowgger_amd/_lib.py
@@ -85,6 +85,7 @@
 FG_LO_TAPER_2 = 8192
 FG_LO_NO_FUSED_FRAMING = 16384
 FG_LO_RFC3164_REGROUP, FG_LO_RFC3164_NO_REGROUP = 32768, 65536
+FG_LO_NO_SPARSE, FG_LO_FORCE_SPARSE = 131072, 262144
 FG_PATH_DECODE_ZERO_COPY, FG_PATH_DECODE_SLICED, FG_PATH_FRAME_FUSED, FG_PATH_FRAME_SLICED, FG_PATH_FRAME_ONE_PIECE = 1, 2, 3, 4, 5
 FG_PATH_FRAME_SYSLEN_DEVICE, FG_PATH_FRAME_SYSLEN_HOST = 6, 7
 FG_PATH_FRAME_CAPNP_DEVICE, FG_PATH_FRAME_CAPNP_HOST = 8, 9
diff --git a/flowgger_amd/csrc/fg_pipeline.hpp b/flowgger_amd/csrc/fg_pipeline.hpp
--- a/flowgger_amd/csrc/fg_pipeline.hpp
+++ b/flowgger_amd/csrc/fg_pipeline.hpp
@@ -1,6 +1,7 @@
 #pragma once
 #include "fg_device.hpp"
 #include "fg_plan_policy.hpp"
+#include "fg_sparse_need.hpp"
 #include "fg_wave.hpp"
 
 namespace fg {
@@ -128,6 +129,7 @@
     fg_span span[6];
     uint32_t first, count;
     bool skip = false;
+    bool handed = false;
 };
 __device__ __forceinline__ void store_row(const DevTables& t, uint64_t li, const RowOut& o) {
     if (o.skip) return;
@@ -259,11 +261,15 @@
 template <class F>
 struct head_cap<F, decltype((void)F::kHeadBytes)> { static constexpr uint32_t value = F::kHeadBytes; };
 
-template <int NB, bool PROF, class F, bool HEAD = false>
+constexpr uint32_t kSparseHandful = 4;
+
+template <int NB, bool PROF, class F, bool HEAD = false, uint32_t SPARSE = 0>
 __device__ __forceinline__ void persistent_loop(const uint8_t* __restrict__ bytes, const uint64_t* __restrict__ offsets,
                                                 uint64_t n, const DevTables& t, uint32_t tile_cap, uint32_t L, uint64_t chunk_lines,
                                                 unsigned long long* prof, uint64_t* stash_base, F& fmt, FrameArgs fr) {
     static_assert(!HEAD || F::kClasses <= 1, "HEAD staging classifies one stage-A byte class at most");
+    static_assert(SPARSE == 0 || (!HEAD && F::kClasses == 0), "the sparse window builds its need bitmap where a stage-A class bitmap would lie");
+    static_assert(SPARSE % 16u == 0 && SPARSE <= 112u, "a line's run of chunks (at most (H + 4 + 14) / 16 + 1) must fit two bitmap words at any shift");
     const uint64_t kChunkLines = chunk_lines;
     extern __shared__ __attribute__((aligned(16))) uint8_t smem[];
     uint16_t* bm16 = reinterpret_cast<uint16_t*>(smem + tile_cap + 64u);
@@ -315,6 +321,40 @@
 #pragma unroll
         for (int k = 0; k < NB; ++k) v[k] = __builtin_amdgcn_raw_buffer_load_b128(rsrc, (int)(lane * 16u + k * 1024u), 0, FG_STREAM_AUX);
     };
+    const uint32_t sparse_tail = fr.strip != FG_FRAME_NONE ? kSparseTailFramed : kSparseTailPlain;
+    auto sparse_offsets = [&](uint64_t a0_, uint32_t span_, uint32_t nl_, uint64_t lo0, uint64_t lo1, bool dense, uint32_t* vo) {
+        uint32_t* skip = reinterpret_cast<uint32_t*>(bm16);
+        const uint32_t nchunk_ = span_ >> 4;
+        const uint32_t nwin = nchunk_ < (uint32_t)NB * kWave ? nchunk_ : (uint32_t)NB * kWave;
+        const uint32_t nword = 2u * NB + 2u < tile_cap / 32u + 8u ? 2u * NB + 2u : tile_cap / 32u + 8u;
+        if (lane < nword) {
+            const uint32_t c = lane * 32u;
+            skip[lane] = !dense || c >= nchunk_ ? ~0u : nchunk_ - c >= 32u ? 0u : ~0u << (nchunk_ - c);
+        }
+        __syncthreads();
+        if (!dense) {
+            auto mark = [&](const NeedRange& r, bool on) {
+                const bool go = on && r.n != 0u && r.c0 < nwin;
+                const uint64_t m = go ? ((1ull << r.n) - 1ull) << (r.c0 & 31u) : 0ull;
+                const uint32_t w = go ? r.c0 >> 5 : 0u;
+                __hip_atomic_fetch_and(skip + w, ~(uint32_t)m, __ATOMIC_RELAXED, __HIP_MEMORY_SCOPE_WORKGROUP);
+                __hip_atomic_fetch_and(skip + w + 1u, ~(uint32_t)(m >> 32), __ATOMIC_RELAXED, __HIP_MEMORY_SCOPE_WORKGROUP);
+            };
+            const uint32_t t0 = (uint32_t)lo0 - (uint32_t)a0_, t1 = (uint32_t)lo1 - (uint32_t)a0_;
+            mark(need_head(t0, t1 - t0, SPARSE, sparse_tail, lane == 0u), lane < nl_);
+            if (lane + 1u == nl_) mark(need_tail(t1, sparse_tail), true);
+            __syncthreads();
+        }
+        const uint32_t half = lane >> 5, bit = lane & 31u, off = lane * 16u;
+#pragma unroll
+        for (int k = 0; k < NB; ++k) vo[k] = ((skip[2 * k + (int)half] >> bit) << 31) | off;
+    };
+    auto load_window_sparse = [&](uint64_t a0_, uint32_t span_, const uint32_t* vo, u32x4* v) {
+        __amdgpu_buffer_rsrc_t rsrc =
+            __builtin_amdgcn_make_buffer_rsrc(const_cast<uint8_t*>(bytes + a0_), (short)0, (int)span_, 0x00020000);
+#pragma unroll
+        for (int k = 0; k < NB; ++k) v[k] = __builtin_amdgcn_raw_buffer_load_b128(rsrc, (int)vo[k], k * 1024, FG_STREAM_AUX);
+    };
     auto geometry_head = [&](uint64_t q, uint64_t o0, uint64_t o1, uint32_t* nl, uint32_t* span, uint32_t* st_out, uint32_t* tb_out) {
         const uint64_t left = hi_line - q;
         const uint32_t avail = left < (uint64_t)L ? (uint32_t)left : L;
@@ -362,10 +402,16 @@
         geometry_head(p, o0, o1, &nl, &span, &st, &tb);
         load_window_head(o0, st, v);
         last2 = load_last2(o0, o1);
+    } else if constexpr (SPARSE != 0) {
+        geometry(p, o0, o1, &nl, &a0, &span);
+        uint32_t vo[NB];
+        sparse_offsets(a0, span, nl, o0, o1, false, vo);
+        load_window_sparse(a0, span, vo, v);
     } else {
         geometry(p, o0, o1, &nl, &a0, &span);
         load_window(a0, span, v);
     }
+    bool dense = false, dense_next = false, dense_then = false;
     RowOut pend{};
     uint64_t pend_li = 0;
     bool pend_valid = false;
@@ -465,6 +511,7 @@
                     }
                 }
             }
+            if constexpr (SPARSE != 0) __builtin_amdgcn_s_waitcnt(0x0F70);
         }
         __builtin_amdgcn_sched_barrier(0);
         FG_MARK(S);
@@ -477,6 +524,11 @@
         if (more) {
             if constexpr (HEAD) geometry_head(pn, no0, no1, &pnl, &pspan, &pst, &ptb);
             else geometry(pn, no0, no1, &pnl, &pa0, &pspan);
+        }
+        uint32_t pvo[SPARSE != 0 ? NB : 1];
+        if constexpr (SPARSE != 0) {
+            dense_next = dense_then;
+            if (more) sparse_offsets(pa0, pspan, pnl, no0, no1, dense_next, pvo);
         }
         FG_MARK(ST);
         if (pend_valid && !(ablate & 1u)) store_row(t, pend_li, pend);
@@ -485,6 +537,8 @@
             if constexpr (HEAD) {
                 load_window_head(no0, pst, v);
                 plast2 = load_last2(no0, no1);
+            } else if constexpr (SPARSE != 0) {
+                load_window_sparse(pa0, pspan, pvo, v);
             } else {
                 load_window(pa0, pspan, v);
             }
@@ -539,7 +593,22 @@
                 c.tlen = st == 0u ? 0u : (st - al < len ? st - al : len);
                 c.last2 = l2;
             }
+            if constexpr (SPARSE != 0) {
+                const uint32_t len = (uint32_t)(e1 - o0);
+                c.tbase = (uint32_t)(o0 - a0);
+                c.tlen = dense || len < SPARSE ? len : SPARSE;
+                c.last2 = 0u;
+                if (valid && e1 > o0 && (o1 - a0) <= (uint64_t)span) {
+                    const uint32_t q = (uint32_t)(e1 - a0);
+                    c.last2 = smem[q - 1u];
+                    if (len >= 2u) c.last2 |= (uint32_t)smem[q - 2u] << 8;
+                }
+            }
             pend = fmt.decode(c, t);
+            if constexpr (SPARSE != 0) {
+                const uint32_t nh = (uint32_t)__popcll(__ballot(valid && pend.handed));
+                dense_then = dense ? nh != 0u : nh > kSparseHandful;
+            }
             if (fr.line_bad && valid && fr.line_bad[li]) {
                 pend.meta = FG_ST_BAD_UTF8 | (0xFFu << 8) | (0xFFu << 16);
                 pend.ts = 0.0;
@@ -573,6 +642,7 @@
         o1 = no1;
         a0 = pa0;
         span = pspan;
+        if constexpr (SPARSE != 0) dense = dense_next;
         if constexpr (HEAD) {
             st = pst;
             tb = ptb;
diff --git a/flowgger_amd/csrc/fg_plan_policy.hpp b/flowgger_amd/csrc/fg_plan_policy.hpp
--- a/flowgger_amd/csrc/fg_plan_policy.hpp
+++ b/flowgger_amd/csrc/fg_plan_policy.hpp
@@ -2,6 +2,7 @@
 #include <stdint.h>
 
 #include "../../include/fg_hip.h"
+#include "fg_sparse_need.hpp"
 
 #if defined(__HIPCC__)
 #define FG_POLICY_HD __host__ __device__
@@ -116,6 +117,14 @@
     return Variant{(flags & FG_LO_FORCE_HEAD) || (avg_len >= kHeadFromLen && !(flags & FG_LO_NO_HEAD)),
                    (flags & FG_LO_SD_PAIRS) || (avg_len >= kPairsFromLen && !(flags & FG_LO_SD_WALK))};
 }
+#if !defined(FG_SPARSE_DEFAULT)
+#define FG_SPARSE_DEFAULT 1
+#endif
+constexpr bool kSparseDefault = FG_SPARSE_DEFAULT != 0;
+inline bool pick_sparse(uint64_t avg_len, uint32_t flags, const Variant& v) {
+    if (v.head || v.pairs) return false;
+    return (flags & FG_LO_FORCE_SPARSE) || (kSparseDefault && avg_len >= kSparseFromLen && !(flags & FG_LO_NO_SPARSE));
+}
 inline bool gelf_group_fits_3k(uint64_t avg_len) { return 8u * avg_len * 17u / 16u + 256u <= 3072u; }
 inline bool gelf_const_3k(uint64_t avg_len, const fg_launch_opts& lo) {
     return gelf_group_fits_3k(avg_len) && !lo.tile_cap && !(lo.flags & FG_LO_GELF_GENERIC);
diff --git a/flowgger_amd/csrc/fg_rfc5424.hip b/flowgger_amd/csrc/fg_rfc5424.hip
--- a/flowgger_amd/csrc/fg_rfc5424.hip
+++ b/flowgger_amd/csrc/fg_rfc5424.hip
@@ -259,6 +259,7 @@
     uint32_t d0;
     uint32_t c7;
     uint32_t e, s;
+    uint32_t start_ok;
 };
 
 __device__ __forceinline__ uint32_t fast_rfc3339(const Tile& T, uint32_t base, const uint32_t* hdr, uint32_t t0, uint32_t L,
@@ -282,7 +283,7 @@
 }
 
 constexpr uint32_t kNoLastByte = 0xFFFFFFFFu;
-__device__ __forceinline__ Fast parse_line_fast(const Tile& T, uint32_t base, uint32_t len, Row& r, uint32_t last_byte = kNoLastByte) {
+__device__ __forceinline__ Fast parse_line_fast(const Tile& T, uint32_t base, uint32_t len, Row& r, uint32_t last_byte, uint32_t vis) {
     Fast f;
     uint32_t l0 = last_byte, l1;
     if (last_byte == kNoLastByte) load8(T, base + (len ? len - 1u : 0u), &l0, &l1);
@@ -323,8 +324,8 @@
         hi = (uint64_t)(m[4] | (m[5] << 16)) | ((uint64_t)(m[6] | (m[7] << 16)) << 32);
     }
     {
-        const uint64_t lo_keep = len < 64u ? (1ull << (len & 63u)) - 1ull : ~0ull;
-        const uint64_t hi_keep = len < 64u ? 0ull : len < 128u ? (1ull << ((len - 64u) & 63u)) - 1ull : ~0ull;
+        const uint64_t lo_keep = vis < 64u ? (1ull << (vis & 63u)) - 1ull : ~0ull;
+        const uint64_t hi_keep = vis < 64u ? 0ull : vis < 128u ? (1ull << ((vis - 64u) & 63u)) - 1ull : ~0ull;
         lo &= lo_keep & ~((2ull << sp0) - 1ull);
         hi &= hi_keep;
     }
@@ -369,6 +370,7 @@
     const bool one_sp = s + 1u < len && cA == ' ' && cB > 0x20u && cB < 0x80u;
     const bool no_sp = s < len && cA > 0x20u && cA < 0x80u;
     f.s = one_sp ? s + 1u : s;
+    f.start_ok = (one_sp || no_sp) ? 1u : 0u;
     f.route |= (live && c == '-' && !(end_plain && (one_sp || no_sp))) ? R_TRIM : 0u;
     return f;
 }
@@ -613,8 +615,10 @@
 
 constexpr uint32_t kShortSdTail = 64;
 
-template <bool HEAD, bool SDX = false, bool PROF = false>
+template <bool HEAD, bool SDX = false, bool PROF = false, uint32_t HB = 0, bool NESTED = false>
 struct Rfc5424FormatT {
+    static_assert(HB == 0 || (HEAD && !SDX), "the sparse head form is a head form without the pair-parallel walk");
+    static constexpr bool kSparse = HB != 0;
     static constexpr uint32_t kClasses = 0;
     static __device__ __forceinline__ void classify_store(const uint4&, uint16_t*, uint32_t, uint32_t, uint32_t) {}
     unsigned long long* pacc = nullptr;
@@ -635,9 +639,11 @@
         r.len[k] = FG_NONE;
     }
     const uint32_t len = (uint32_t)(o1 - o0);
-    const bool in_tile = HEAD ? c.tlen == len : (o1 - a0) <= (uint64_t)span;
-    const bool head_only = HEAD && !in_tile && c.tlen >= 512u;
+    const bool in_window = !kSparse || (o1 - a0) <= (uint64_t)span;
+    const bool in_tile = HEAD ? c.tlen == len && in_window : (o1 - a0) <= (uint64_t)span;
+    const bool head_only = HEAD && !in_tile && (kSparse ? in_window : c.tlen >= 512u);
     const uint32_t walk_len = HEAD ? c.tlen : len;
+    const uint32_t sd_len = kSparse ? len : walk_len;
     const uint32_t base = HEAD ? c.tbase : (uint32_t)(o0 - a0);
     bool from_global = false;
     uint32_t* tile_w = reinterpret_cast<uint32_t*>(const_cast<uint8_t*>(smem));
@@ -656,8 +662,9 @@
     if (valid) {
         route = R_GENERIC;
         if (in_tile || head_only) {
-            f = parse_line_fast(T, base, len, r, HEAD ? (len ? (c.last2 & 0xFFu) : 0u) : kNoLastByte);
+            f = parse_line_fast(T, base, len, r, HEAD ? (len ? (c.last2 & 0xFFu) : 0u) : kNoLastByte, kSparse ? walk_len : len);
             route = f.route;
+            if (kSparse && head_only && f.d0 + 3u > walk_len) route |= R_GENERIC;
             if (!(route & R_GENERIC)) {
                 if (route & R_TS_SLOW) {
                     LdsReader rd(T.w, base);
@@ -669,11 +676,11 @@
             }
         }
     }
-    const bool sd_any = valid && !(route & R_GENERIC) && (route & R_TAIL) && r.status == E_OK && f.c7 == '[';
+    const bool sd_any = valid && !(route & R_GENERIC) && (route & R_TAIL) && r.status == E_OK && f.c7 == '[' && !(kSparse && head_only);
     const uint64_t sd_ballot = __ballot(sd_any);
     const bool group_has_sd = __any(sd_any && len - f.d0 > kShortSdTail) || __popcll(sd_ballot) > 4;
     const bool sd_lane = sd_any && group_has_sd;
-    FG_MARK(F);
+    if constexpr (!NESTED) FG_MARK(F);
     tick(0);
     sd2::Lds SL{};
     sd2::LineIn sin{false, 0u, 0u, 0u, false};
@@ -699,6 +706,10 @@
         rebuild_bitmap<QuoteClass>(smem, bm16, span >> 4);
         __syncthreads();
     }
+    const uint32_t end_b1 = c.last2 & 0xFFu, end_b2 = (c.last2 >> 8) & 0xFFu;
+    const bool end_is_plain = end_b1 > 0x20u && end_b1 < 0x80u;
+    const bool end_settled = end_is_plain || (len >= 2u && ascii_ws(end_b1) && end_b2 > 0x20u && end_b2 < 0x80u);
+    bool trim_settled = false;
     bool redo = false;
     bool coop = false;
     if (valid) {
@@ -712,11 +723,11 @@
                             r.status = slo.status;
                         } else {
                             r.n_ent = slo.n_ent;
-                            redo = !finish_sd_tail(T, base, len, walk_len, c.last2, slo.msg_at, r, bytes, o0);
+                            redo = !finish_sd_tail(T, base, len, sd_len, c.last2, slo.msg_at, r, bytes, o0);
                         }
                     }
                 } else if (sd_lane) {
-                    redo = !parse_tail_sd_tile(T, base, f.d0, len, walk_len, c.last2, r, t, stash ? tile_w : nullptr, &rec_ok, bytes, o0);
+                    redo = !parse_tail_sd_tile(T, base, f.d0, len, sd_len, c.last2, r, t, stash ? tile_w : nullptr, &rec_ok, bytes, o0);
                 } else if (head_only && (route & R_TAIL)) {
                     redo = true;
                 } else if (route & R_TAIL) {
@@ -726,7 +737,12 @@
                     uint32_t e = f.e, s0 = f.s;
                     if (route & R_TRIM) {
                         LdsReader rd(T.w, base);
-                        if (head_only) {
+                        if (kSparse && head_only) {
+                            e = end_is_plain ? len : len - 1u;
+                            if (!f.start_ok) s0 = trim_start(rd, f.d0 + 1u, walk_len);
+                            trim_settled = end_settled && s0 + 3u <= walk_len;
+                            redo = !trim_settled;
+                        } else if (head_only) {
                             s0 = trim_start(rd, f.d0 + 1u, walk_len - 8u);
                             GlobalReader grd(reinterpret_cast<const uint32_t*>(bytes), o0);
                             e = trim_end(grd, 0u, len);
@@ -734,6 +750,7 @@
                         } else {
                             e = trim_end(rd, 0u, len);
                             s0 = trim_start(rd, f.d0 + 1u, len);
+                            if (kSparse) trim_settled = end_settled && s0 + 3u <= HB;
                         }
                     }
                     r.data0 = f.d0;
@@ -829,7 +846,7 @@
                 sd_walk<true>(rd, r.data0, len, &msg_at, &cnt, t, first);
                 FG_RARE_END();
             } else if (sd_lane) {
-                sd_walk_tile<SD_EMIT>(T, base, r.data0, walk_len, &msg_at, &cnt, t, first);
+                sd_walk_tile<SD_EMIT>(T, base, r.data0, sd_len, &msg_at, &cnt, t, first);
             } else if (in_tile) {
                 LdsReader rd(T.w, base);
                 sd_walk<true>(rd, r.data0, len, &msg_at, &cnt, t, first);
@@ -851,6 +868,10 @@
     for (int k = 0; k < 6; ++k) o.span[k] = ok ? fg_span{r.off[k], r.len[k]} : fg_span{0, FG_NONE};
     o.first = first;
     o.count = r.n_ent;
+    if constexpr (kSparse) {
+        o.handed = valid && in_window && (coop ||
+                             (len > HB && ((route & (R_GENERIC | R_TAIL)) != 0u || ((route & R_TRIM) != 0u && !trim_settled) || f.d0 + 3u > HB)));
+    }
     if constexpr (HEAD) {
         unsigned long long todo = __ballot(coop);
         while (todo) {
@@ -880,7 +901,7 @@
             __syncthreads();
             GroupCtx c2{bytes, smem, bm16, ro0, ro1, ra0, rspan, lane == 0u, rli, c.stash, ablate, c.ent_state, nullptr};
             c2.tile_cap = c.tile_cap;
-            Rfc5424FormatT<false, SDX, false> whole;
+            Rfc5424FormatT<false, SDX, false, 0, true> whole;
             const RowOut w = whole.decode(c2, t);
             auto b32 = [&](uint32_t x) -> uint32_t { return (uint32_t)__builtin_amdgcn_readfirstlane((int)x); };
             const uint32_t g_meta = b32(w.meta), g_first = b32(w.first), g_count = b32(w.count);
@@ -935,6 +956,24 @@
     }
 }
 
+template <int NB, bool PROF, uint32_t H>
+__global__ __launch_bounds__(kWave, 2) void k_rfc5424_sparse(const uint8_t* __restrict__ bytes, const uint64_t* __restrict__ offsets, uint64_t n,
+                                                            DevTables t, uint32_t tile_cap, uint32_t L, uint64_t groups,
+                                                            unsigned long long* prof, uint64_t* stash_base, FrameArgs fr) {
+    Rfc5424FormatT<true, false, PROF, H> fmt;
+    if constexpr (PROF) {
+        __shared__ unsigned long long pacc[10];
+        if (threadIdx.x < 10) pacc[threadIdx.x] = 0ull;
+        fmt.pacc = pacc;
+        __syncthreads();
+        persistent_loop<NB, PROF, Rfc5424FormatT<true, false, PROF, H>, false, H>(bytes, offsets, n, t, tile_cap, L, groups, prof, stash_base, fmt, fr);
+        __syncthreads();
+        if (prof && threadIdx.x < 10) atomicAdd(&prof[6 + threadIdx.x], pacc[threadIdx.x]);
+    } else {
+        persistent_loop<NB, PROF, Rfc5424FormatT<true, false, PROF, H>, false, H>(bytes, offsets, n, t, tile_cap, L, groups, prof, stash_base, fmt, fr);
+    }
+}
+
 template <int NB, bool SDX>
 __global__ __launch_bounds__(kWave, 2) void k_rfc5424_fused(const uint8_t* __restrict__ bytes, DevTables t, uint32_t tile_cap, uint32_t L,
                                                            uint64_t* stash_base, FusedArgs fa, uint32_t strip) {
@@ -967,7 +1006,10 @@
                                  const uint8_t* line_bad, const fg_launch_opts* lo, fg::TicketSlot* tk) {
     if (n == 0) return 0;
     const fg::Variant v = fg::pick_variant(avg_len, lo->flags);
-    const auto ks = v.pairs ? (v.head ? rfc5424_kernels<true, true>("rfc5424 (head, pairs)") : rfc5424_kernels<false, true>("rfc5424 (pairs)"))
+    const bool sparse = fg::pick_sparse(avg_len, lo->flags, v);
+    const auto ks = sparse ? fg::kernels(fg::k_rfc5424_sparse<fg::kWindowKiB, false, fg::kSparseHead>,
+                                         FG_PROF_TWIN(fg::k_rfc5424_sparse<fg::kWindowKiB, true, fg::kSparseHead>), "rfc5424 (sparse)")
+                    : v.pairs ? (v.head ? rfc5424_kernels<true, true>("rfc5424 (head, pairs)") : rfc5424_kernels<false, true>("rfc5424 (pairs)"))
                             : (v.head ? rfc5424_kernels<true, false>("rfc5424 (head)") : rfc5424_kernels<false, false>("rfc5424"));
     const fg::PlanFormat pf = v.pairs ? fg::PlanFormat().classes(2u).lds_tile(fg::sd2::extra_bytes).tile(12288u).chunk(128u).tickets_from(4u)
                               : v.head ? fg::PlanFormat()
diff --git a/flowgger_amd/csrc/fg_sparse_need.hpp b/flowgger_amd/csrc/fg_sparse_need.hpp
--- /dev/null
+++ b/flowgger_amd/csrc/fg_sparse_need.hpp
@@ -0,0 +1,30 @@
+#pragma once
+#include <stdint.h>
+
+#if defined(__HIPCC__)
+#define FG_NEED_HD __host__ __device__
+#else
+#define FG_NEED_HD
+#endif
+
+namespace fg {
+
+constexpr uint32_t kSparseHead = 96;
+constexpr uint32_t kSparseTailPlain = 2, kSparseTailFramed = 4;
+constexpr uint64_t kSparseFromLen = kSparseHead + kSparseTailPlain + 127u;
+
+struct NeedRange {
+    uint32_t c0, n;
+};
+FG_NEED_HD inline NeedRange need_chunks(uint32_t b0, uint32_t b1) {
+    if (b1 <= b0) return NeedRange{0u, 0u};
+    const uint32_t c0 = b0 >> 4, c1 = (b1 - 1u) >> 4;
+    return NeedRange{c0, c1 - c0 + 1u};
+}
+FG_NEED_HD inline NeedRange need_head(uint32_t t0, uint32_t len, uint32_t H, uint32_t tail, bool first) {
+    const uint32_t b0 = first ? t0 : (t0 >= tail ? t0 - tail : 0u);
+    return need_chunks(b0, t0 + (len > H ? H : len));
+}
+FG_NEED_HD inline NeedRange need_tail(uint32_t t1, uint32_t tail) { return need_chunks(t1 >= tail ? t1 - tail : 0u, t1); }
+
+}
diff --git a/flowgger_amd/decoder.py b/flowgger_amd/decoder.py
--- a/flowgger_amd/decoder.py
+++ b/flowgger_amd/decoder.py
@@ -46,11 +46,11 @@
 
     def set_launch_opts(self, lines_per_group: int = 0, tile_cap: int = 0, waves_per_cu: int = 0, gelf_lds_budget: int = 0,
                         gelf_window_kib: int = 0, gelf_generic: bool = False, transcode_one_piece: bool = False, chunk_lines: int = 0,
-                        no_head: bool = False, force_head: bool = False, sd_walk: bool = False, sd_pairs: bool = False, no_zero_copy: bool = False, frame_kernel_upload: bool = False, frame_classic: bool = False, static_chunks: bool = False, frame_selftest_stall: bool = False, ent_chunk: int = 0, no_taper: bool = False, taper_levels: int = 0, no_fused_framing: bool = False, fused_look: int = 0, fused_ext: int = 0, rfc3164_regroup: int = 0) -> None:
+                        no_head: bool = False, force_head: bool = False, sd_walk: bool = False, sd_pairs: bool = False, no_zero_copy: bool = False, frame_kernel_upload: bool = False, frame_classic: bool = False, static_chunks: bool = False, frame_selftest_stall: bool = False, ent_chunk: int = 0, no_taper: bool = False, taper_levels: int = 0, no_fused_framing: bool = False, fused_look: int = 0, fused_ext: int = 0, rfc3164_regroup: int = 0, no_sparse: bool = False, force_sparse: bool = False) -> None:
         lo = L.fg_launch_opts(lines_per_group, tile_cap, waves_per_cu, gelf_lds_budget, gelf_window_kib,
                               (L.FG_LO_GELF_GENERIC if gelf_generic else 0) | (L.FG_LO_TRANSCODE_ONE_PIECE if transcode_one_piece else 0) |
                               (L.FG_LO_NO_HEAD if no_head else 0) | (L.FG_LO_FORCE_HEAD if force_head else 0) |
-                              (L.FG_LO_SD_WALK if sd_walk else 0) | (L.FG_LO_SD_PAIRS if sd_pairs else 0) | (L.FG_LO_NO_ZERO_COPY if no_zero_copy else 0) | (L.FG_LO_FRAME_KERNEL_UPLOAD if frame_kernel_upload else 0) | (L.FG_LO_FRAME_CLASSIC if frame_classic else 0) | (L.FG_LO_STATIC_CHUNKS if static_chunks else 0) | (L.FG_LO_FRAME_SELFTEST_STALL if frame_selftest_stall else 0) | (L.FG_LO_NO_TAPER if no_taper else 0) | (L.FG_LO_TAPER_1 if taper_levels & 1 else 0) | (L.FG_LO_TAPER_2 if taper_levels & 2 else 0) | (L.FG_LO_NO_FUSED_FRAMING if no_fused_framing else 0) | (L.FG_LO_RFC3164_REGROUP if rfc3164_regroup == 1 else L.FG_LO_RFC3164_NO_REGROUP if rfc3164_regroup == 2 else 0),
+                              (L.FG_LO_SD_WALK if sd_walk else 0) | (L.FG_LO_SD_PAIRS if sd_pairs else 0) | (L.FG_LO_NO_ZERO_COPY if no_zero_copy else 0) | (L.FG_LO_FRAME_KERNEL_UPLOAD if frame_kernel_upload else 0) | (L.FG_LO_FRAME_CLASSIC if frame_classic else 0) | (L.FG_LO_STATIC_CHUNKS if static_chunks else 0) | (L.FG_LO_FRAME_SELFTEST_STALL if frame_selftest_stall else 0) | (L.FG_LO_NO_TAPER if no_taper else 0) | (L.FG_LO_TAPER_1 if taper_levels & 1 else 0) | (L.FG_LO_TAPER_2 if taper_levels & 2 else 0) | (L.FG_LO_NO_FUSED_FRAMING if no_fused_framing else 0) | (L.FG_LO_RFC3164_REGROUP if rfc3164_regroup == 1 else L.FG_LO_RFC3164_NO_REGROUP if rfc3164_regroup == 2 else 0) | (L.FG_LO_NO_SPARSE if no_sparse else 0) | (L.FG_LO_FORCE_SPARSE if force_sparse else 0),
                               chunk_lines, ent_chunk, fused_look, fused_ext)
         L.check(L.lib().fg_set_launch_opts(self._ctx, C.byref(lo)), "fg_set_launch_opts")
 
diff --git a/include/fg_hip.h b/include/fg_hip.h
--- a/include/fg_hip.h
+++ b/include/fg_hip.h
@@ -162,6 +162,8 @@
     FG_LO_NO_FUSED_FRAMING = 16384,
     FG_LO_RFC3164_REGROUP = 32768,
     FG_LO_RFC3164_NO_REGROUP = 65536,
+    FG_LO_NO_SPARSE = 131072,
+    FG_LO_FORCE_SPARSE = 262144,
     FG_LO_RESERVED = 0x40000000
 };
 
diff --git a/integration/rust/fg-hip-sys/src/lib.rs b/integration/rust/fg-hip-sys/src/lib.rs
--- a/integration/rust/fg-hip-sys/src/lib.rs
+++ b/integration/rust/fg-hip-sys/src/lib.rs
@@ -162,6 +162,8 @@
 pub const FG_LO_NO_FUSED_FRAMING: c_int = 16384;
 pub const FG_LO_RFC3164_REGROUP: c_int = 32768;
 pub const FG_LO_RFC3164_NO_REGROUP: c_int = 65536;
+pub const FG_LO_NO_SPARSE: c_int = 131072;
+pub const FG_LO_FORCE_SPARSE: c_int = 262144;
 pub const FG_LO_RESERVED: c_int = 1073741824;
 
 pub const FG_TABLE_ARRAYS: c_int = 15;
```

Measured after the change: 17.88 billion lines/s (median of 6 runs). +9.5%, better.
